# Dokumushikun/jittor-clip-fewshot

Hardware: AMD Instinct MI355X
Metric: images/sec ViT-B/32 fwd+LoRA-bwd bs=256 (higher is better)
Workload: dtype f32; 1 GPU; cfg-2: ViT-B/32 + rank-4 LoRA(q,k,v; 12 text + 12 vision blocks; shipped lora_weights.pkl) + 4 text-prompt tokens; run_lora train step = text tower fwd+bwd on 403 captions + image tower fwd+bwd + 100*cos CE + AdamW; global_batch=256, images_per_rank=256, captions=403, tower_streams=2, text_positions=77, parallelism=dp1

## Files before the change

include/clipfs.h:

```cpp
#ifndef CLIPFS_H
#define CLIPFS_H

#include <stddef.h>
#include <stdint.h>

#ifdef __cplusplus
extern "C" {
#endif

#define CLIPFS_OK 0
#define CLIPFS_EINVAL 1
#define CLIPFS_HIPERR_BASE 1000

#define CLIPFS_ABI_VERSION 2
int clipfs_abi_version(void);
const char* clipfs_source_stamp(void);
const char* clipfs_gemm_source_stamp(void);
const char* clipfs_last_error(void);

typedef struct clipfs_gemm_args {
  size_t struct_size;
  const float* A;
  const float* B;
  float* C;
// ... 17 lines not shown
  float* workspace;
  size_t workspace_floats;
  const void* A_f16;
  void* C_f16;
  int aux_f16;
  int* counters;
  size_t counters_ints;
} clipfs_gemm_args;
int clipfs_gemm_nt(const clipfs_gemm_args* args, void* stream);
int clipfs_split_bf16(const float* src, void* planes, size_t n, void* stream);
int clipfs_convert_f16(const float* src, void* dst, size_t n, void* stream);
int clipfs_gemm_splits(int M, int N, int K);
size_t clipfs_gemm_workspace_floats(int M, int N, int K);
size_t clipfs_gemm_counter_ints(int M, int N, int K);
int clipfs_gemm_timing(int enable);
int clipfs_gemm_timing_collect(double* total_ms, double* total_flops, int* launches);
double clipfs_gemm_timing_last_bytes(void);

int clipfs_layernorm_fwd(const float* x, int ldx, const float* gamma, const float* beta, float* y,
                         float* mean, float* rstd, int rows, int width, float eps, void* stream);
int clipfs_layernorm_bwd(const float* dy, const float* x, int ldx, const float* gamma, const float* mean,
                         const float* rstd, const float* dres, float* dx, int lddx, int rows, int width,
                         void* stream);
int clipfs_layernorm_bwd_rows(const float* dy, const float* x, int ldx, const float* gamma, const float* mean,
                              const float* rstd, const int32_t* xmap, const float* dres, float* dx, int lddx, int rows,
                              int width, void* stream);
int clipfs_layernorm_fwd_f16(const float* x, int ldx, const float* gamma, const float* beta, float* y, void* y16,
                             float* mean, float* rstd, int rows, int width, float eps, void* stream);
int clipfs_layernorm_bwd_f16(const float* dy, const float* x, int ldx, const float* gamma, const float* mean,
                             const float* rstd, const float* dres, float* dx, void* dx16, int lddx, int rows, int width,
                             void* stream);
int clipfs_layernorm_fwd_lora_ok(int width, int r, int nseg);
int clipfs_layernorm_fwd_lora(const float* x, int ldx, const float* gamma, const float* beta, float* y, void* y16,
                              float* mean, float* rstd, int rows, int width, float eps, const float* A, float* t, int r,
                              int nseg, unsigned seg_mask, float p, uint64_t seed, uint32_t stream_base, uint32_t drow0,
                              void* keep_bits, void* stream);
int clipfs_layernorm_fwd_lora_map(const float* x, int ldx, const float* gamma, const float* beta, float* y, void* y16,
                                  float* mean, float* rstd, int rows, int width, float eps, const float* A, float* t, int r,
                                  int nseg, unsigned seg_mask, float p, uint64_t seed, uint32_t stream_base, uint32_t drow0,
                                  const int32_t* drow_map, void* keep_bits, void* stream);

int clipfs_attention_fwd(const float* qkv, float* out, float* lse, int batch, int seq, int heads, int causal,
                         void* stream);
int clipfs_attention_bwd(const float* qkv, const float* dout, const float* out, const float* lse, float* dqkv,
                         float* work, int batch, int seq, int heads, int causal, void* stream);
size_t clipfs_attention_lse_floats(int batch, int seq, int heads);
int clipfs_attention_bwd_packed_ok(int seq, int causal);
int clipfs_attention_bwd_packed(const float* qkv, const float* dout, const float* out, const float* lse, float* dqkv,
                                const int32_t* off, int batch, int seq, int heads, void* stream);
int clipfs_attention_fwd_packed(const float* qkv, float* out, float* lse, const int32_t* off, int batch, int seq, int heads,
                                void* stream);
int clipfs_attention_bwd_packed_io(const float* qkv, const float* dout, const float* out, const float* lse, float* dqkv,
                                   const int32_t* off, int batch, int seq, int heads, void* stream);
int clipfs_attention_f16_fwd(const void* qkv, int qkv_f16, float* out, void* out16, float* lse, int batch, int seq,
                             int heads, int causal, void* stream);
int clipfs_attention_f16_bwd(const void* qkv, int qkv_f16, const void* dout, int dout_f16, const float* out,
                             const float* lse, float* dqkv, void* dqkv16, float* work, int batch, int seq, int heads,
                             int causal, void* stream);

int clipfs_lora_down(const float* x, const float* A, float* t, int rows, int width, int r, int nseg,
                     unsigned seg_mask, float p, uint64_t seed, uint32_t stream_base, uint32_t drow0,
                     void* keep_bits, void* stream);
int clipfs_lora_keep_bits_ok(int width, int segw, int r, int nseg);
size_t clipfs_lora_bwd_work_floats(int rows, int width, int r, int nseg);
int clipfs_lora_bwd(const float* dy, const float* x, const float* t, const float* A, const float* B,
                    float* dt, float* dA, float* dB, float* dx, int rows, int width, int segw, int r,
                    int nseg, unsigned seg_mask, float scale, float p, uint64_t seed, uint32_t stream_base,
                    uint32_t drow0, const void* keep_bits, float* work, void* stream);
int clipfs_lora_bwd_f16dy_ok(int width, int segw, int r, int nseg);
int clipfs_lora_bwd_f16dy(const void* dy16, const float* x, const float* t, const float* A, const float* B,
                          float* dt, float* dA, float* dB, float* dx, int rows, int width, int segw, int r,
                          int nseg, unsigned seg_mask, float scale, float p, uint64_t seed, uint32_t stream_base,
                          uint32_t drow0, const void* keep_bits, float* work, void* stream);

int clipfs_vit_fill_special(float* x, const float* class_emb, const float* pos, const float* vpt, int batch,
                            int tokens, int n_patch, int n_vpt, int width, void* stream);
int clipfs_text_embed(const int64_t* ids, const float* table, const float* pos, const float* ctx, int n_ctx,
                      float* x, int n, int seq, int width, void* stream);
int clipfs_token_rows_grad(const float* dx, float* dtok, int n, int seq, int width, int n_tok, int first,
                           void* stream);
int clipfs_matmul_small(const float* A, const float* B, float* C, int M, int N, int K, long sam, long sak,
                        long sbk, long sbn, float alpha, void* stream);
int clipfs_gather_eot(const float* x, const int64_t* ids, float* out, int32_t* idx_out, int n, int seq,
                      int width, void* stream);
int clipfs_scatter_rows(const float* dy, const int32_t* idx, float* dx, int n, int seq, int width, void* stream);
int clipfs_gather_seq_rows(const float* src, size_t ld, const int32_t* idx, float* out, int n, int seq, int width,
                           void* stream);
int clipfs_add_seq_rows(const float* src, const int32_t* idx, float* dx, int n, int seq, int width, void* stream);
int clipfs_put_seq_rows(const float* src, const int32_t* idx, float* dst, size_t ld, int n, int seq, int width,
                        void* stream);
int clipfs_eot_index(const int64_t* ids, int32_t* idx, int n, int seq, void* stream);
int clipfs_gather_rows_map(const float* src, size_t ld, const int32_t* map, float* out, int n, int width, void* stream);
int clipfs_put_rows_map(const float* src, const int32_t* map, float* dst, size_t ld, int n, int width, void* stream);
int clipfs_gather_seq_rows_f16(const void* src_f16, size_t ld, const int32_t* idx, float* out, int n, int seq, int width,
                               void* stream);
int clipfs_put_seq_rows_f16(const float* src, const int32_t* idx, void* dst_f16, size_t ld, int n, int seq, int width,
                            void* stream);

void* clipfs_bpe_create(const char* merges, size_t n_bytes, int n_merges);
void clipfs_bpe_destroy(void* handle);
long clipfs_bpe_encode(const void* handle, const uint8_t* words, const int32_t* offsets, int n_words, int32_t* ids,
                       int32_t* counts, long cap);

int clipfs_nchw_to_nhwc(const float* x, float* y, int N, int C, int H, int W, void* stream);
int clipfs_im2col_nhwc(const float* x, float* col, int N, int H, int W, int C, int kh, int kw, int stride, int pad,
                       int Kp, void* stream);
int clipfs_maxpool3x3s2_nhwc(const float* x, float* y, int N, int H, int W, int C, void* stream);
int clipfs_global_avgpool_nhwc(const float* x, float* y, int N, int HW, int C, void* stream);

int clipfs_l2norm_fwd(const float* x, float* y, float* inv_norm, int rows, int width, void* stream);
int clipfs_l2norm_bwd(const float* dy, const float* y, const float* inv_norm, float* dx, int rows, int width,
                      void* stream);
int clipfs_class_mean_fwd(const float* emb, float* out, int classes, int templates, int width, void* stream);
int clipfs_class_mean_bwd(const float* emb, const float* dout, float* demb, int classes, int templates, int width,
                          void* stream);
int clipfs_cross_entropy(const float* logits, const int64_t* target, float* dlogits, float* loss_rows,
                         float* loss_sum, int32_t* correct, int rows, int classes, float grad_scale,
                         void* stream);
int clipfs_topk(const float* logits, int32_t* labels, int rows, int classes, int k, void* stream);
int clipfs_channel_affine(const float* x, const float* scale1, const float* bias1, float* y, int rows,
                          int width, void* stream);
int clipfs_logit_normalize(const float* z, float* out, float* work, int rows, int classes, void* stream);
int clipfs_logit_normalize_bwd(const float* z, const float* dzn, float* dz, int rows, int classes, void* stream);
int clipfs_colsum(const float* x, const float* y, float* out, int rows, int cols, void* stream);
size_t clipfs_bias_grad_work_floats(int rows, int cols);
int clipfs_bias_grad(const float* x, size_t ldx, int rows, int cols, int seg_width, float* out0, float* out1,
                     float* out2, float* work, void* stream);
int clipfs_l1_loss(const float* a, const float* b, size_t n, float* loss, float* da, float grad_scale, void* stream);
int clipfs_kl_logits(const float* logits, const float* target_logits, float* loss_rows, float* dlogits, int rows,
                     int classes, float grad_scale, void* stream);

int clipfs_adamw(float* p, const float* g, float* m, float* v, size_t n, int step, float lr, float beta1,
                 float beta2, float eps, float weight_decay, float grad_scale, void* stream);

size_t clipfs_mta_work_floats(int n_img, int views, int width, int classes);
// ... 1 lines not shown
               int n_img, int views, int width, int classes, void* stream);

int clipfs_tta_views(const uint8_t* image, int height, int width, const int32_t* recs, int n_views, int out_size,
                     const float* mean, const float* stdv, float* out, void* stream);

int clipfs_crop_batch(const uint8_t* pool, size_t pool_bytes, const int64_t* src, const int64_t* src_dev, int n_src,
                      const int32_t* recs, const int32_t* recs_dev, int n, int out_size, const float* mean,
                      const float* stdv, float* out_norm, float* out_raw, void* stream);

typedef struct clipfs_block {
  const float *ln1_g, *ln1_b, *ln2_g, *ln2_b;
  const float *w_qkv, *b_qkv, *w_qkv_t;
  const float *w_o, *b_o, *w_o_t;
  const float *w_fc, *b_fc, *w_fc_t;
  const float *w_pr, *b_pr, *w_pr_t;
  const float *lora_a_qkv, *lora_b_qkv, *lora_a_o, *lora_b_o;
  float *g_lora_a_qkv, *g_lora_b_qkv, *g_lora_a_o, *g_lora_b_o;
  unsigned lora_mask;
  const void *w_qkv_p, *w_o_p, *w_fc_p, *w_pr_p, *w_qkv_t_p, *w_o_t_p, *w_fc_t_p, *w_pr_t_p;
  float *g_ln1_b, *g_ln2_b, *g_b_q, *g_b_k, *g_b_v, *g_b_o, *g_b_fc, *g_b_pr;
  const float* prompt;
  float* g_prompt;
  int prompt_first, prompt_rows;
} clipfs_block;

typedef struct clipfs_tower {
  size_t struct_size;
  size_t block_size;
  int width, heads, layers, seq, causal;
  int lora_r;
  float lora_scale, lora_dropout;
  uint64_t dropout_seed;
  uint32_t dropout_stream0;
  uint32_t dropout_row0;
  const clipfs_block* blocks;
  int weight_format;
  int* gemm_counters;
  size_t gemm_counters_ints;
  int grad_lo;
} clipfs_tower;

int clipfs_prompt_put(const float* prompt, float* x, const int32_t* off, int batch, int seq, int first, int n, int width,
                      void* stream);
int clipfs_prompt_harvest(float* dx, void* dx16, const int32_t* off, int batch, int seq, int first, int n, int width,
                          float* g, void* stream);

size_t clipfs_tower_saved_floats(const clipfs_tower* t, int batch);
size_t clipfs_tower_scratch_floats(const clipfs_tower* t, int batch);
size_t clipfs_tower_counter_ints(const clipfs_tower* t, int batch);
int clipfs_tower_fwd(const clipfs_tower* t, float* x, int batch, float* saved, float* scratch, void* stream);
int clipfs_tower_fwd_rows(const clipfs_tower* t, float* x, const int32_t* rows, int batch, float* saved, float* scratch,
                          void* stream);
int clipfs_tower_rows_mode(const clipfs_tower* t);
int clipfs_tower_bwd(const clipfs_tower* t, float* dx, int batch, const float* saved, float* scratch,
                     int stop_at_input, void* stream);
int clipfs_tower_bwd_sparse(const clipfs_tower* t, const float* dxs, const int32_t* rows, float* dx, int batch,
                            const float* saved, float* scratch, int stop_at_input, void* stream);
int clipfs_tower_pack_mode(const clipfs_tower* t, int batch, int R);
int clipfs_tower_bwd_packed(const clipfs_tower* t, const float* dxs, const int32_t* rows, const int32_t* plan, int R,
                            float* dx, int batch, const float* saved, float* scratch, int stop_at_input, void* stream);
int clipfs_tower_pack_fwd_mode(const clipfs_tower* t, int batch, int R);
int clipfs_tower_fwd_packed(const clipfs_tower* t, float* x, const int32_t* rows, const int32_t* plan, int R, int batch,
                            float* saved, float* scratch, void* stream);
int clipfs_tower_bwd_packed_saved(const clipfs_tower* t, const float* dxs, const int32_t* rows, const int32_t* plan, int R,
                                  float* dx, int batch, const float* saved, float* scratch, int stop_at_input, void* stream);

#ifdef __cplusplus
}
#endif
#endif
```

jittor-clip-fewshot_amd/clipfs/_lib.py:

```python
from __future__ import annotations

import ctypes as C
import os

ABI_VERSION = 2

_HERE = os.path.dirname(os.path.abspath(__file__))
_TAG = os.environ.get("CLIPFS_LIB_TAG", "")
LIB_PATH = os.path.join(_HERE, f"libclipfs_hip_{_TAG}.so" if _TAG else "libclipfs_hip.so")

c_f32p = C.c_void_p
c_stream = C.c_void_p


class ClipfsError(RuntimeError):
    pass


class GemmArgs(C.Structure):
    _fields_ = [
        ("struct_size", C.c_size_t),
        ("A", C.c_void_p), ("B", C.c_void_p), ("C", C.c_void_p),
        ("M", C.c_int), ("N", C.c_int), ("K", C.c_int),
        ("lda", C.c_int), ("ldb", C.c_int), ("ldc", C.c_int),
# ... 24 lines not shown
                                  "prompt", "g_prompt")] + [("prompt_first", C.c_int), ("prompt_rows", C.c_int)]


class Tower(C.Structure):
    _fields_ = [
        ("struct_size", C.c_size_t), ("block_size", C.c_size_t),
        ("width", C.c_int), ("heads", C.c_int), ("layers", C.c_int), ("seq", C.c_int), ("causal", C.c_int),
        ("lora_r", C.c_int), ("lora_scale", C.c_float), ("lora_dropout", C.c_float),
        ("dropout_seed", C.c_uint64), ("dropout_stream0", C.c_uint32), ("dropout_row0", C.c_uint32),
        ("blocks", C.POINTER(Block)), ("weight_format", C.c_int),
        ("gemm_counters", C.c_void_p), ("gemm_counters_ints", C.c_size_t),
        ("grad_lo", C.c_int),
    ]


_i, _f, _p, _sz = C.c_int, C.c_float, C.c_void_p, C.c_size_t
_u, _u64, _u32 = C.c_uint, C.c_uint64, C.c_uint32

SIGNATURES = {
    "clipfs_abi_version": (_i, []),
    "clipfs_last_error": (C.c_char_p, []),
    "clipfs_source_stamp": (C.c_char_p, []),
    "clipfs_gemm_source_stamp": (C.c_char_p, []),
    "clipfs_gemm_nt": (_i, [C.POINTER(GemmArgs), _p]),
    "clipfs_split_bf16": (_i, [_p, _p, _sz, _p]),
    "clipfs_convert_f16": (_i, [_p, _p, _sz, _p]),
    "clipfs_gemm_splits": (_i, [_i, _i, _i]),
    "clipfs_gemm_workspace_floats": (_sz, [_i, _i, _i]),
    "clipfs_gemm_counter_ints": (_sz, [_i, _i, _i]),
    "clipfs_gemm_timing": (_i, [_i]),
    "clipfs_gemm_timing_collect": (_i, [C.POINTER(C.c_double), C.POINTER(C.c_double), C.POINTER(C.c_int)]),
    "clipfs_gemm_timing_last_bytes": (C.c_double, []),
    "clipfs_layernorm_fwd": (_i, [_p, _i, _p, _p, _p, _p, _p, _i, _i, _f, _p]),
    "clipfs_layernorm_bwd": (_i, [_p, _p, _i, _p, _p, _p, _p, _p, _i, _i, _i, _p]),
    "clipfs_layernorm_fwd_f16": (_i, [_p, _i, _p, _p, _p, _p, _p, _p, _i, _i, _f, _p]),
    "clipfs_layernorm_fwd_lora_ok": (_i, [_i, _i, _i]),
    "clipfs_layernorm_fwd_lora": (_i, [_p, _i, _p, _p, _p, _p, _p, _p, _i, _i, _f, _p, _p, _i, _i, _u, _f, _u64, _u32, _u32, _p, _p]),
    "clipfs_layernorm_bwd_f16": (_i, [_p, _p, _i, _p, _p, _p, _p, _p, _p, _i, _i, _i, _p]),
    "clipfs_attention_fwd": (_i, [_p, _p, _p, _i, _i, _i, _i, _p]),
    "clipfs_attention_bwd": (_i, [_p, _p, _p, _p, _p, _p, _i, _i, _i, _i, _p]),
    "clipfs_attention_lse_floats": (_sz, [_i, _i, _i]),
    "clipfs_attention_f16_fwd": (_i, [_p, _i, _p, _p, _p, _i, _i, _i, _i, _p]),
    "clipfs_attention_f16_bwd": (_i, [_p, _i, _p, _i, _p, _p, _p, _p, _p, _i, _i, _i, _i, _p]),
    "clipfs_lora_keep_bits_ok": (_i, [_i, _i, _i, _i]),
    "clipfs_lora_down": (_i, [_p, _p, _p, _i, _i, _i, _i, _u, _f, _u64, _u32, _u32, _p, _p]),
    "clipfs_lora_bwd_work_floats": (_sz, [_i, _i, _i, _i]),
    "clipfs_lora_bwd": (_i, [_p, _p, _p, _p, _p, _p, _p, _p, _p, _i, _i, _i, _i, _i, _u, _f, _f, _u64, _u32, _u32, _p, _p, _p]),
    "clipfs_lora_bwd_f16dy_ok": (_i, [_i, _i, _i, _i]),
    "clipfs_lora_bwd_f16dy": (_i, [_p, _p, _p, _p, _p, _p, _p, _p, _p, _i, _i, _i, _i, _i, _u, _f, _f, _u64, _u32, _u32, _p, _p, _p]),
    "clipfs_vit_fill_special": (_i, [_p, _p, _p, _p, _i, _i, _i, _i, _i, _p]),
    "clipfs_text_embed": (_i, [_p, _p, _p, _p, _i, _p, _i, _i, _i, _p]),
    "clipfs_token_rows_grad": (_i, [_p, _p, _i, _i, _i, _i, _i, _p]),
    "clipfs_matmul_small": (_i, [_p, _p, _p, _i, _i, _i, C.c_long, C.c_long, C.c_long, C.c_long, _f, _p]),
    "clipfs_gather_eot": (_i, [_p, _p, _p, _p, _i, _i, _i, _p]),
    "clipfs_scatter_rows": (_i, [_p, _p, _p, _i, _i, _i, _p]),
    "clipfs_gather_seq_rows": (_i, [_p, _sz, _p, _p, _i, _i, _i, _p]),
    "clipfs_add_seq_rows": (_i, [_p, _p, _p, _i, _i, _i, _p]),
    "clipfs_put_seq_rows": (_i, [_p, _p, _p, _sz, _i, _i, _i, _p]),
    "clipfs_eot_index": (_i, [_p, _p, _i, _i, _p]),
    "clipfs_gather_seq_rows_f16": (_i, [_p, _sz, _p, _p, _i, _i, _i, _p]),
    "clipfs_put_seq_rows_f16": (_i, [_p, _p, _p, _sz, _i, _i, _i, _p]),
    "clipfs_l2norm_fwd": (_i, [_p, _p, _p, _i, _i, _p]),
    "clipfs_l2norm_bwd": (_i, [_p, _p, _p, _p, _i, _i, _p]),
    "clipfs_class_mean_fwd": (_i, [_p, _p, _i, _i, _i, _p]),
    "clipfs_class_mean_bwd": (_i, [_p, _p, _p, _i, _i, _i, _p]),
    "clipfs_cross_entropy": (_i, [_p, _p, _p, _p, _p, _p, _i, _i, _f, _p]),
    "clipfs_topk": (_i, [_p, _p, _i, _i, _i, _p]),
    "clipfs_channel_affine": (_i, [_p, _p, _p, _p, _i, _i, _p]),
    "clipfs_logit_normalize": (_i, [_p, _p, _p, _i, _i, _p]),
    "clipfs_logit_normalize_bwd": (_i, [_p, _p, _p, _i, _i, _p]),
    "clipfs_colsum": (_i, [_p, _p, _p, _i, _i, _p]),
    "clipfs_bias_grad_work_floats": (_sz, [_i, _i]),
    "clipfs_bias_grad": (_i, [_p, _sz, _i, _i, _i, _p, _p, _p, _p, _p]),
    "clipfs_l1_loss": (_i, [_p, _p, _sz, _p, _p, _f, _p]),
    "clipfs_kl_logits": (_i, [_p, _p, _p, _p, _i, _i, _f, _p]),
    "clipfs_adamw": (_i, [_p, _p, _p, _p, _sz, _i, _f, _f, _f, _f, _f, _f, _p]),
    "clipfs_mta_work_floats": (_sz, [_i, _i, _i, _i]),
    "clipfs_mta": (_i, [_p, _p, _p, _p, _p, _i, _i, _i, _i, _p]),
    "clipfs_tta_views": (_i, [_p, _i, _i, _p, _i, _i, _p, _p, _p, _p]),
    "clipfs_crop_batch": (_i, [_p, _sz, _p, _p, _i, _p, _p, _i, _i, _p, _p, _p, _p, _p]),
    "clipfs_bpe_create": (C.c_void_p, [C.c_char_p, _sz, _i]),
    "clipfs_bpe_destroy": (None, [C.c_void_p]),
    "clipfs_bpe_encode": (C.c_long, [C.c_void_p, _p, _p, _i, _p, _p, C.c_long]),
    "clipfs_nchw_to_nhwc": (_i, [_p, _p, _i, _i, _i, _i, _p]),
    "clipfs_im2col_nhwc": (_i, [_p, _p, _i, _i, _i, _i, _i, _i, _i, _i, _i, _p]),
    "clipfs_maxpool3x3s2_nhwc": (_i, [_p, _p, _i, _i, _i, _i, _p]),
    "clipfs_global_avgpool_nhwc": (_i, [_p, _p, _i, _i, _i, _p]),
    "clipfs_prompt_put": (_i, [_p, _p, _p, _i, _i, _i, _i, _i, _p]),
    "clipfs_prompt_harvest": (_i, [_p, _p, _p, _i, _i, _i, _i, _i, _p, _p]),
    "clipfs_tower_saved_floats": (_sz, [C.POINTER(Tower), _i]),
    "clipfs_tower_scratch_floats": (_sz, [C.POINTER(Tower), _i]),
    "clipfs_tower_counter_ints": (_sz, [C.POINTER(Tower), _i]),
    "clipfs_tower_fwd": (_i, [C.POINTER(Tower), _p, _i, _p, _p, _p]),
    "clipfs_tower_fwd_rows": (_i, [C.POINTER(Tower), _p, _p, _i, _p, _p, _p]),
    "clipfs_tower_rows_mode": (_i, [C.POINTER(Tower)]),
    "clipfs_tower_bwd": (_i, [C.POINTER(Tower), _p, _i, _p, _p, _i, _p]),
    "clipfs_tower_bwd_sparse": (_i, [C.POINTER(Tower), _p, _p, _p, _i, _p, _p, _i, _p]),
    "clipfs_attention_bwd_packed_ok": (_i, [_i, _i]),
    "clipfs_attention_bwd_packed": (_i, [_p, _p, _p, _p, _p, _p, _i, _i, _i, _p]),
    "clipfs_gather_rows_map": (_i, [_p, _sz, _p, _p, _i, _i, _p]),
    "clipfs_put_rows_map": (_i, [_p, _p, _p, _sz, _i, _i, _p]),
    "clipfs_layernorm_bwd_rows": (_i, [_p, _p, _i, _p, _p, _p, _p, _p, _p, _i, _i, _i, _p]),
    "clipfs_tower_pack_mode": (_i, [C.POINTER(Tower), _i, _i]),
    "clipfs_tower_bwd_packed": (_i, [C.POINTER(Tower), _p, _p, _p, _i, _p, _i, _p, _p, _i, _p]),
    "clipfs_layernorm_fwd_lora_map": (_i, [_p, _i, _p, _p, _p, _p, _p, _p, _i, _i, _f, _p, _p, _i, _i, _u, _f, _u64, _u32, _u32, _p,
                                           _p, _p]),
    "clipfs_attention_fwd_packed": (_i, [_p, _p, _p, _p, _i, _i, _i, _p]),
    "clipfs_attention_bwd_packed_io": (_i, [_p, _p, _p, _p, _p, _p, _i, _i, _i, _p]),
    "clipfs_tower_pack_fwd_mode": (_i, [C.POINTER(Tower), _i, _i]),
    "clipfs_tower_fwd_packed": (_i, [C.POINTER(Tower), _p, _p, _p, _i, _i, _p, _p, _p]),
    "clipfs_tower_bwd_packed_saved": (_i, [C.POINTER(Tower), _p, _p, _p, _i, _p, _i, _p, _p, _i, _p]),
}

def new_gemm_args() -> GemmArgs:
    g = GemmArgs()
    g.struct_size = C.sizeof(GemmArgs)
    return g


def new_tower() -> Tower:
    t = Tower()
    t.struct_size = C.sizeof(Tower)
    t.block_size = C.sizeof(Block)
    return t


_lib = None


def load() -> C.CDLL:
    global _lib
    if _lib is not None:
        return _lib
    if not os.path.isfile(LIB_PATH):
        raise ClipfsError(
            f"{LIB_PATH} not found: the HIP engine is not built.  Run "
            "`python jittor-clip-fewshot_amd/build.py` (needs hipcc).  There is no CPU fallback.")
    try:
        import torch
    except Exception:
        pass
    lib = C.CDLL(LIB_PATH, mode=C.RTLD_GLOBAL if hasattr(C, "RTLD_GLOBAL") else 0)
    for name, (res, args) in SIGNATURES.items():
        fn = getattr(lib, name)
        fn.restype = res
        fn.argtypes = args
    if lib.clipfs_abi_version() != ABI_VERSION:
        raise ClipfsError(f"libclipfs_hip.so ABI version {lib.clipfs_abi_version()} != {ABI_VERSION} of this binding: "
                          "rebuild with `python jittor-clip-fewshot_amd/build.py --force`")
    _lib = lib
    return lib


def check(rc: int, what: str = "") -> None:
    if rc != 0:
        msg = load().clipfs_last_error().decode("utf-8", "replace")
        raise ClipfsError(f"{what or 'clipfs call'} failed (rc={rc}): {msg}")
```

jittor-clip-fewshot_amd/clipfs/engine.py:

```python
from __future__ import annotations

import ctypes as C
from typing import Dict, List, Optional, Tuple

import torch

from . import _lib, ops
from ._lib import Block, Tower, check


def _ptr(t: Optional[torch.Tensor]) -> Optional[int]:
    return None if t is None else t.data_ptr()


def _bias_slot(p: Optional[torch.nn.Parameter]) -> Optional[torch.Tensor]:
    if p is None or not p.requires_grad:
        return None
    return getattr(p, "grad_slot", None)


def _lora_trains(a, where: str) -> bool:
    flags = {p.requires_grad for p, _ in a.trainable_pairs()}
    if len(flags) > 1:
        raise ValueError(f"{where}: some of its LoRA adapters are frozen and others trainable; freeze or train the "
                         "q / k / v / o adapters of a block together")
    return flags == {True}


def _blk_biases(blk) -> List[torch.nn.Parameter]:
    a = blk.attn
    if getattr(a, "is_lora_mha", False):
        out = [a.q_proj.bias, a.k_proj.bias, a.v_proj.bias, a.proj.bias]
    else:
        out = [a.in_proj_bias, a.out_proj.bias]
    return out + [blk.ln_1.bias, blk.ln_2.bias, blk.mlp.c_fc.bias, blk.mlp.c_proj.bias]


def _mix_seed(base: int, step: int) -> int:
    z = (base * 0x9E3779B97F4A7C15 + step * 0xBF58476D1CE4E5B9 + 0x94D049BB133111EB) & 0xFFFFFFFFFFFFFFFF
    z ^= z >> 30
    z = (z * 0xBF58476D1CE4E5B9) & 0xFFFFFFFFFFFFFFFF
    z ^= z >> 27
    z = (z * 0x94D049BB133111EB) & 0xFFFFFFFFFFFFFFFF
    z ^= z >> 31
    return z or 1


class _TowerRT:

    def __init__(self, transformer, seq: int, stream0: int, name: str = "tower"):
        self.mod = transformer
        self.name = name
        self.seq = seq
        self.width = transformer.width
        self.heads = transformer.heads
        self.layers = transformer.layers
        self.causal = bool(transformer.causal)
        self.stream0 = stream0
        self._bufs: Dict[Tuple[str, int], torch.Tensor] = {}
        self._wt: Dict[int, Dict[str, torch.Tensor]] = {}
        self._planes: Dict[Tuple[int, str, str], torch.Tensor] = {}
        self.precision = "fp32"
        self.lora_r = 0
        self.lora_scale = 0.0
        self.lora_dropout = 0.0

    def _transposed(self, i: int, blk) -> Dict[str, torch.Tensor]:
        wt = self._wt.get(i)
        if wt is None:
            a = blk.attn
            w_qkv = a.qkv_weight if getattr(a, "is_lora_mha", False) else a.in_proj_weight
            w_o = a.proj.weight if getattr(a, "is_lora_mha", False) else a.out_proj.weight
            wt = {"qkv": w_qkv.data.t().contiguous(), "o": w_o.data.t().contiguous(),
                  "fc": blk.mlp.c_fc.weight.data.t().contiguous(), "pr": blk.mlp.c_proj.weight.data.t().contiguous()}
            self._wt[i] = wt
        return wt

    def _plane(self, i: int, name: str, w: torch.Tensor) -> torch.Tensor:
        key = (i, name, self.precision)
        pl = self._planes.get(key)
        if pl is None:
            pl = ops.split_bf16(w.contiguous()) if self.precision == "bf16x3" else ops.to_f16(w.contiguous())
            self._planes[key] = pl
        return pl

    def _block_trains(self, i: int, blk) -> bool:
        a = blk.attn
        if getattr(a, "is_lora_mha", False) and a.r > 0 and _lora_trains(a, f"{self.name} block {i}"):
            return True
        if _bias_slot(getattr(blk, "VPT_shallow", None)) is not None:
            return True
        return any(_bias_slot(p) is not None for p in _blk_biases(blk))

    def grad_floor(self, needs_input_grad: bool, head_trains: bool = False) -> Optional[int]:
        if needs_input_grad:
            return 0
        for i, blk in enumerate(self.mod.resblocks):
            if self._block_trains(i, blk):
                return i
        return self.layers - 1 if head_trains else None

    def descriptor(self, train: bool, seed: int, seq: Optional[int] = None, row0: int = 0, grad_lo: int = 0) -> Tower:
        blocks = (Block * self.layers)()
        r, scale, p = 0, 0.0, 0.0
        n_pr = getattr(self.mod, "prompt_rows", 0)
        first = (seq or self.seq) - n_pr if getattr(self.mod, "prompt_tail", False) else 1
        for i, blk in enumerate(self.mod.resblocks):
            a = blk.attn
            b = blocks[i]
            vp = getattr(blk, "VPT_shallow", None)
            if vp is not None:
                g = _bias_slot(vp)
                ok = (vp.dim() == 2 and tuple(vp.shape) == (n_pr, self.width) and vp.dtype == torch.float32
                      and vp.is_contiguous() and vp.device == self.mod.resblocks[0].ln_1.weight.device and first >= 1)
                if g is not None:
                    ok = ok and g.shape == vp.shape and g.dtype == torch.float32 and g.is_contiguous() and g.device == vp.device
                if not ok:
                    raise ValueError(f"{self.name} block {i}: deep prompt {tuple(vp.shape)} (slot "
# ... 21 lines not shown
                gq, gk, gv = (None, None, None) if g is None else (g[:d], g[d:2 * d], g[2 * d:])
                go = _bias_slot(a.out_proj.bias)
            b.g_b_q, b.g_b_k, b.g_b_v, b.g_b_o = _ptr(gq), _ptr(gk), _ptr(gv), _ptr(go)
            b.g_ln1_b, b.g_ln2_b = _ptr(_bias_slot(blk.ln_1.bias)), _ptr(_bias_slot(blk.ln_2.bias))
            b.g_b_fc, b.g_b_pr = _ptr(_bias_slot(blk.mlp.c_fc.bias)), _ptr(_bias_slot(blk.mlp.c_proj.bias))
            if train:
                wt = self._transposed(i, blk)
                b.w_qkv_t, b.w_o_t, b.w_fc_t, b.w_pr_t = _ptr(wt["qkv"]), _ptr(wt["o"]), _ptr(wt["fc"]), _ptr(wt["pr"])
            if self.precision != "fp32":
                b.w_qkv_p = _ptr(self._plane(i, "qkv", w_qkv.data))
                b.w_o_p = _ptr(self._plane(i, "o", w_o.data))
                b.w_fc_p = _ptr(self._plane(i, "fc", blk.mlp.c_fc.weight.data))
                b.w_pr_p = _ptr(self._plane(i, "pr", blk.mlp.c_proj.weight.data))
                if train:
                    b.w_qkv_t_p = _ptr(self._plane(i, "qkv_t", wt["qkv"]))
                    b.w_o_t_p = _ptr(self._plane(i, "o_t", wt["o"]))
                    b.w_fc_t_p = _ptr(self._plane(i, "fc_t", wt["fc"]))
                    b.w_pr_t_p = _ptr(self._plane(i, "pr_t", wt["pr"]))
            b.lora_mask = 0
            if lora and a.r > 0:
                if r and (a.r != r or abs(a.scaling - scale) > 0 or abs(a.dropout_rate - p) > 0):
                    raise ValueError("all LoRA layers of one tower must share r / alpha / dropout")
                r, scale, p = a.r, float(a.scaling), float(a.dropout_rate)
                b.lora_mask = a.lora_mask
                trains = _lora_trains(a, f"{self.name} block {i}")
                b.lora_a_qkv, b.lora_b_qkv = _ptr(a.lora_A_qkv), _ptr(a.lora_B_qkv)
                if trains:
                    b.g_lora_a_qkv, b.g_lora_b_qkv = _ptr(a.grad_A_qkv), _ptr(a.grad_B_qkv)
                if a.lora_mask & 8:
                    b.lora_a_o, b.lora_b_o = _ptr(a.lora_A_o), _ptr(a.lora_B_o)
                    if trains:
                        b.g_lora_a_o, b.g_lora_b_o = _ptr(a.grad_A_o), _ptr(a.grad_B_o)
        t = _lib.new_tower()
        t.width, t.heads, t.layers, t.seq, t.causal = (self.width, self.heads, self.layers, seq or self.seq,
                                                       int(self.causal))
        t.lora_r, t.lora_scale, t.lora_dropout = r, scale, p
        t.dropout_seed = seed if p > 0 else 0
        t.dropout_stream0 = self.stream0
        t.dropout_row0 = row0 * (seq or self.seq)
        t.weight_format = {"fp32": 0, "bf16x3": 1, "fp16": 2}[self.precision]
        t.grad_lo = grad_lo
        t.blocks = C.cast(blocks, C.POINTER(Block))
        t._blocks_keepalive = blocks
        self.lora_r, self.lora_scale, self.lora_dropout = r, scale, p
        return t

    def lora_dropout_rate(self) -> float:
        return max((float(b.attn.dropout_rate) for b in self.mod.resblocks
                    if getattr(b.attn, "is_lora_mha", False) and b.attn.r > 0), default=0.0)

    def has_lora(self) -> bool:
        return any(getattr(b.attn, "is_lora_mha", False) and b.attn.r > 0 for b in self.mod.resblocks)

    def buffer(self, kind: str, n_floats: int, device) -> torch.Tensor:
        key = (kind, n_floats)
        buf = self._bufs.get(key)
        if buf is None:
            for k in [k for k in self._bufs if k[0] == kind]:
                del self._bufs[k]
            buf = torch.empty(max(n_floats, 4), device=device, dtype=torch.float32)
            self._bufs[key] = buf
        return buf

    def _attach_counters(self, t: Tower, batch: int, device) -> None:
        n = _lib.load().clipfs_tower_counter_ints(C.byref(t), batch)
        if n == 0:
            return
        buf = self._bufs.get(("counters", 0))
        if buf is None or buf.numel() < n:
            buf = torch.zeros(n, device=device, dtype=torch.int32)
            self._bufs[("counters", 0)] = buf
        t.gemm_counters, t.gemm_counters_ints = buf.data_ptr(), buf.numel()

    def forward(self, x: torch.Tensor, batch: int, train: bool, seed: int, seq: Optional[int] = None,
                own_saved: bool = False, row0: int = 0, rows: Optional[torch.Tensor] = None, grad_lo: int = 0,
                pack: Optional[Tuple[torch.Tensor, int]] = None, desc: Optional[Tower] = None):
        lib = _lib.load()
        t = desc if desc is not None else self.descriptor(train, seed, seq, row0, grad_lo if train else 0)
        self._attach_counters(t, batch, x.device)
        scratch = self.buffer("scratch", lib.clipfs_tower_scratch_floats(C.byref(t), batch), x.device)
        saved = None
        if train:
            n = lib.clipfs_tower_saved_floats(C.byref(t), batch)
            saved = torch.empty(max(n, 4), device=x.device, dtype=torch.float32) if own_saved else \
                self.buffer("saved", n, x.device)
        if rows is not None:
            assert rows.dtype == torch.int32 and rows.is_cuda and rows.numel() >= batch
        if pack is not None:
            assert rows is not None
            plan, R = pack
            check(lib.clipfs_tower_fwd_packed(C.byref(t), x.data_ptr(), rows.data_ptr(), plan.data_ptr(), R, batch, _ptr(saved),
                                              scratch.data_ptr(), torch.cuda.current_stream().cuda_stream), "tower_fwd_packed")
        elif rows is not None:
            check(lib.clipfs_tower_fwd_rows(C.byref(t), x.data_ptr(), rows.data_ptr(), batch, _ptr(saved), scratch.data_ptr(),
                                            torch.cuda.current_stream().cuda_stream), "tower_fwd_rows")
        else:
            check(lib.clipfs_tower_fwd(C.byref(t), x.data_ptr(), batch, _ptr(saved), scratch.data_ptr(),
                                       torch.cuda.current_stream().cuda_stream), "tower_fwd")
        return saved

    def backward(self, dx: torch.Tensor, batch: int, saved: torch.Tensor, seed: int, stop_at_input: bool,
                 seq: Optional[int] = None, row0: int = 0, grad_lo: int = 0):
        lib = _lib.load()
        t = self.descriptor(True, seed, seq, row0, grad_lo)
        self._attach_counters(t, batch, dx.device)
        scratch = self.buffer("scratch", lib.clipfs_tower_scratch_floats(C.byref(t), batch), dx.device)
        check(lib.clipfs_tower_bwd(C.byref(t), dx.data_ptr(), batch, saved.data_ptr(), scratch.data_ptr(),
                                   int(stop_at_input), torch.cuda.current_stream().cuda_stream), "tower_bwd")


    def backward_sparse(self, dxs: torch.Tensor, rows: torch.Tensor, batch: int, saved: torch.Tensor, seed: int,
                        stop_at_input: bool, seq: Optional[int] = None, row0: int = 0, grad_lo: int = 0) -> torch.Tensor:
        lib = _lib.load()
        t = self.descriptor(True, seed, seq, row0, grad_lo)
        self._attach_counters(t, batch, dxs.device)
        scratch = self.buffer("scratch", lib.clipfs_tower_scratch_floats(C.byref(t), batch), dxs.device)
        dx = torch.empty(batch * (seq or self.seq), self.width, device=dxs.device, dtype=torch.float32)
        check(lib.clipfs_tower_bwd_sparse(C.byref(t), dxs.data_ptr(), rows.data_ptr(), dx.data_ptr(), batch, saved.data_ptr(),
                                          scratch.data_ptr(), int(stop_at_input), torch.cuda.current_stream().cuda_stream),
              "tower_bwd_sparse")
        return dx

    def backward_packed(self, dxs: torch.Tensor, rows: torch.Tensor, plan: torch.Tensor, R: int, batch: int,
                        saved: torch.Tensor, seed: int, stop_at_input: bool, seq: Optional[int] = None, row0: int = 0,
                        grad_lo: int = 0, saved_packed: bool = False) -> torch.Tensor:
        lib = _lib.load()
        t = self.descriptor(True, seed, seq, row0, grad_lo)
        self._attach_counters(t, batch, dxs.device)
        scratch = self.buffer("scratch", lib.clipfs_tower_scratch_floats(C.byref(t), batch), dxs.device)
        dx = torch.empty(batch * (seq or self.seq), self.width, device=dxs.device, dtype=torch.float32)
        fn = lib.clipfs_tower_bwd_packed_saved if saved_packed else lib.clipfs_tower_bwd_packed
        check(fn(C.byref(t), dxs.data_ptr(), rows.data_ptr(), plan.data_ptr(), R, dx.data_ptr(), batch, saved.data_ptr(),
                 scratch.data_ptr(), int(stop_at_input), torch.cuda.current_stream().cuda_stream),
              "tower_bwd_packed_saved" if saved_packed else "tower_bwd_packed")
        return dx

    def pack_mode(self, batch: int, R: int, seed: int, seq: Optional[int] = None, grad_lo: int = 0,
                  train: bool = True) -> bool:
        t = self.descriptor(train, seed, seq, 0, grad_lo)
        return bool(_lib.load().clipfs_tower_pack_mode(C.byref(t), batch, R))

    @staticmethod
    def pack_modes(desc: Tower, batch: int, R: int) -> Tuple[bool, bool]:
        lib = _lib.load()
        return bool(lib.clipfs_tower_pack_mode(C.byref(desc), batch, R)), bool(lib.clipfs_tower_pack_fwd_mode(C.byref(desc), batch, R))

    def pack_fwd_mode(self, batch: int, R: int, seed: int, seq: Optional[int] = None, grad_lo: int = 0,
                      train: bool = True) -> bool:
        t = self.descriptor(train, seed, seq, 0, grad_lo)
        return bool(_lib.load().clipfs_tower_pack_fwd_mode(C.byref(t), batch, R))


class Engine:
    def __init__(self, model):
        self.model = model
        v = model.visual
        self.vis = _TowerRT(v.transformer, v.tokens, stream0=1000, name="vision")
        self.txt = _TowerRT(model.transformer, model.context_length, stream0=0, name="text")
        self.vproj_t = v.proj.data.t().contiguous()
        self.tproj_t = model.text_projection.data.t().contiguous()
        self.seed_base = 0x5EED
        self.step = 0
        self.trim_text = False
        self._trim_cache = {}
        self.sparse_backward = True
        self.prune_backward = True
        self.pack_text_backward = True
        self.pack_text_forward = True
        self._pack_cache = {}

    @property
    def precision(self) -> str:
        return self.vis.precision

    @precision.setter
    def precision(self, mode: str) -> None:
        if mode not in ("fp32", "bf16x3", "fp16"):
            raise ValueError("precision must be 'fp32', 'bf16x3' or 'fp16'")
        self.vis.precision = mode
        self.txt.precision = mode

    def image_plan(self) -> Optional[int]:
        if not self.prune_backward:
            return 0
        v = self.model.visual
        return self.vis.grad_floor(v.VPT is not None or _bias_slot(v.ln_pre.bias) is not None,
                                   _bias_slot(v.ln_post.bias) is not None)

    def text_plan(self, has_ctx: bool) -> Optional[int]:
        if not self.prune_backward:
            return 0
        return self.txt.grad_floor(has_ctx, _bias_slot(self.model.ln_final.bias) is not None)

    def next_seed(self) -> int:
        self.step += 1
        return _mix_seed(self.seed_base, self.step)

    def vit_forward(self, images: torch.Tensor, train: bool, seed: int = 0, own_saved: bool = False, row0: int = 0):
        lo = self.image_plan() if train else 0
        if lo is None:
            train = False
        m = self.model
        v = m.visual
        assert images.is_cuda and images.dtype == torch.float32, "images: fp32 device tensor [B,3,R,R]"
        images = images.contiguous()
        B = images.shape[0]
        if images.shape[1] != 3 or images.shape[2] != v.input_resolution or images.shape[3] != v.input_resolution:
            raise ValueError(f"expected images [B,3,{v.input_resolution},{v.input_resolution}], got {tuple(images.shape)}")
        L, d = v.tokens, v.width
        P = (v.input_resolution // v.patch_size) ** 2
        x0 = torch.empty(B * L, d, device=images.device, dtype=torch.float32)
        ops.patch_embed(images, v.conv1.weight.data, v.positional_embedding.data, x0, L)
        ops.vit_fill_special(x0, v.class_embedding.data, v.positional_embedding.data,
                             None if v.VPT is None else v.VPT.data, B, L, P)
        need_pre = train and v.VPT is not None
        if need_pre:
            x, mean0, rstd0 = ops.layernorm_fwd(x0, v.ln_pre.weight.data, v.ln_pre.bias.data, save_stats=True)
        else:
            x = ops.layernorm_fwd(x0, v.ln_pre.weight.data, v.ln_pre.bias.data)
            mean0 = rstd0 = None
        one_row = bool(self.sparse_backward)
        saved = self.vis.forward(x, B, train, seed, own_saved=own_saved, row0=row0,
# ... 354 lines not shown
```

jittor-clip-fewshot_amd/clipfs/ops.py:

```python
from __future__ import annotations

import ctypes as C
from typing import Optional

import torch

from . import _lib
from ._lib import GemmArgs, check


def _stream() -> int:
    return torch.cuda.current_stream().cuda_stream


def _p(t: Optional[torch.Tensor]) -> Optional[int]:
    if t is None:
        return None
    assert t.is_cuda, "clipfs ops need device tensors (there is no CPU path)"
    return t.data_ptr()


def _f32(t: torch.Tensor) -> torch.Tensor:
    assert t.dtype == torch.float32 and t.is_contiguous(), (t.dtype, t.is_contiguous())
    return t
# ... 201 lines not shown
def lora_bwd(dy, x, t, A, B, dA, dB, *, dx=None, scale, p=0.0, seed=0, stream_base=0, seg_mask=None, row0=0, keep_bits=None):
    rows, width = x.shape
    nseg = dy.shape[1] // width
    r = B.shape[1]
    if seg_mask is None:
        seg_mask = (1 << nseg) - 1
    lib = _lib.load()
    nwork = lib.clipfs_lora_bwd_work_floats(rows, width, r, nseg)
    work = torch.empty(nwork, device=x.device, dtype=torch.float32)
    dt = torch.empty(rows, nseg * r, device=x.device, dtype=torch.float32)
    if dy.dtype == torch.float16:
        assert dy.is_contiguous()
        check(lib.clipfs_lora_bwd_f16dy(_p(dy), _p(_f32(x)), _p(_f32(t)), _p(_f32(A)), _p(_f32(B)), _p(dt), _p(dA),
                                        _p(dB), _p(dx), rows, width, width, r, nseg, seg_mask, scale, p, seed, stream_base,
                                        row0, _p(keep_bits), _p(work), _stream()), "lora_bwd_f16dy")
        return dt
    check(lib.clipfs_lora_bwd(_p(_f32(dy)), _p(_f32(x)), _p(_f32(t)), _p(_f32(A)), _p(_f32(B)), _p(dt), _p(dA),
                              _p(dB), _p(dx), rows, width, width, r, nseg, seg_mask, scale, p, seed, stream_base,
                              row0, _p(keep_bits), _p(work), _stream()), "lora_bwd")
    return dt


def vit_fill_special(x, class_emb, pos, vpt, batch, tokens, n_patch):
    n_vpt = 0 if vpt is None else vpt.shape[0]
    check(_lib.load().clipfs_vit_fill_special(_p(x), _p(class_emb), _p(pos), _p(vpt), batch, tokens, n_patch, n_vpt,
                                              class_emb.numel(), _stream()), "vit_fill_special")


def text_embed(ids, table, pos, ctx=None):
    n, seq = ids.shape
    width = table.shape[1]
    assert ids.dtype == torch.int64 and ids.is_contiguous()
    x = torch.empty(n * seq, width, device=table.device, dtype=torch.float32)
    n_ctx = 0 if ctx is None else ctx.shape[0]
    check(_lib.load().clipfs_text_embed(_p(ids), _p(table), _p(pos), _p(ctx), n_ctx, _p(x), n, seq, width, _stream()),
          "text_embed")
    return x


def token_rows_grad(dx, dtok, n, seq, first):
    n_tok, width = dtok.shape
    check(_lib.load().clipfs_token_rows_grad(_p(dx), _p(dtok), n, seq, width, n_tok, first, _stream()),
          "token_rows_grad")


def matmul_small(a, b, M, N, K, sam, sak, sbk, sbn, alpha=1.0, out=None):
    if out is None:
        out = torch.empty(M, N, device=a.device, dtype=torch.float32)
    check(_lib.load().clipfs_matmul_small(_p(a), _p(b), _p(out), M, N, K, sam, sak, sbk, sbn, alpha, _stream()),
          "matmul_small")
    return out


def eot_index(ids: torch.Tensor) -> torch.Tensor:
    assert ids.is_cuda and ids.dtype == torch.int64 and ids.is_contiguous()
    n, seq = ids.shape
    idx = torch.empty(n, device=ids.device, dtype=torch.int32)
    check(_lib.load().clipfs_eot_index(_p(ids), _p(idx), n, seq, _stream()), "eot_index")
    return idx


def gather_eot(x, ids):
    n, seq = ids.shape
    width = x.shape[-1]
    out = torch.empty(n, width, device=x.device, dtype=torch.float32)
    idx = torch.empty(n, device=x.device, dtype=torch.int32)
    check(_lib.load().clipfs_gather_eot(_p(x), _p(ids), _p(out), _p(idx), n, seq, width, _stream()), "gather_eot")
    return out, idx


def scatter_rows(dy, idx, seq, out=None):
    n, width = dy.shape
    dx = out if out is not None else torch.empty(n * seq, width, device=dy.device, dtype=torch.float32)
    check(_lib.load().clipfs_scatter_rows(_p(_f32(dy)), _p(idx), _p(dx), n, seq, width, _stream()), "scatter_rows")
    return dx


def l2norm_fwd(x, save_inv=False):
    rows, width = x.shape
    y = torch.empty_like(x)
    inv = torch.empty(rows, device=x.device, dtype=torch.float32) if save_inv else None
    check(_lib.load().clipfs_l2norm_fwd(_p(_f32(x)), _p(y), _p(inv), rows, width, _stream()), "l2norm_fwd")
    return (y, inv) if save_inv else y


def l2norm_bwd(dy, y, inv):
    rows, width = y.shape
    dx = torch.empty_like(y)
    check(_lib.load().clipfs_l2norm_bwd(_p(_f32(dy)), _p(y), _p(inv), _p(dx), rows, width, _stream()), "l2norm_bwd")
    return dx


def class_mean_fwd(emb, classes, templates, out=None):
    width = emb.shape[1]
    if out is None:
        out = torch.empty(classes, width, device=emb.device, dtype=torch.float32)
    assert out.is_contiguous() and tuple(out.shape) == (classes, width)
    check(_lib.load().clipfs_class_mean_fwd(_p(_f32(emb)), _p(out), classes, templates, width, _stream()),
          "class_mean_fwd")
    return out


def class_mean_bwd(emb, dout, classes, templates):
    demb = torch.empty_like(emb)
    check(_lib.load().clipfs_class_mean_bwd(_p(_f32(emb)), _p(_f32(dout)), _p(demb), classes, templates, emb.shape[1],
                                            _stream()), "class_mean_bwd")
# ... 102 lines not shown
```

jittor-clip-fewshot_amd/csrc/attention.hip:

```cpp
#include "common.h"

#include <stdlib.h>

namespace clipfs {

constexpr int HD = 64;
constexpr int KSTRIDE = 68;

typedef float f32x4 __attribute__((ext_vector_type(4)));

__device__ __forceinline__ void stage_rows(const float* __restrict__ base, size_t ld, float* __restrict__ dst, int L,
                                           int tid) {
  for (int idx = tid; idx < L * (HD / 4); idx += (int)blockDim.x) {
    const int r = idx >> 4, c = idx & 15;
    *reinterpret_cast<f32x4*>(dst + r * KSTRIDE + 4 * c) = *reinterpret_cast<const f32x4*>(base + (size_t)r * ld + 4 * c);
  }
}

template <int KPL>
__device__ __forceinline__ void rows_to_regs(const float* __restrict__ s, int lane, int L, float (&reg)[KPL][HD]) {
#pragma unroll
  for (int kk = 0; kk < KPL; ++kk) {
    const int j = lane + 64 * kk;
    const bool ok = j < L;
// ... 525 lines not shown
  float* sP = sG + L * KSTRIDE;
  const int lane = threadIdx.x & 63;
  const int wave = __builtin_amdgcn_readfirstlane(threadIdx.x >> 6);
  const int b = blockIdx.x / H, h = blockIdx.x % H;
  const int d = H * HD;
  const size_t ld = (size_t)3 * d;
  const float* q0 = qkv + (size_t)b * L * ld + (size_t)h * HD;
  stage_rows_n(q0, ld, sQ, L);
  stage_rows_n(dout + (size_t)b * L * d + (size_t)h * HD, (size_t)d, sG, L);
  __syncthreads();
  float* myP = sP + wave * 64;
  float* myS = sP + 8 * 64 + wave * 64;
  const float* lse0 = lse + ((size_t)b * H + h) * L;
  const float* D0 = Dbuf + ((size_t)b * H + h) * L;
  for (int j = wave; j < L; j += 8) {
    f32x4 k[HD / 4], v[HD / 4];
#pragma unroll
    for (int c = 0; c < HD / 4; ++c) {
      k[c] = *reinterpret_cast<const f32x4*>(q0 + d + (size_t)j * ld + 4 * c);
      v[c] = *reinterpret_cast<const f32x4*>(q0 + 2 * d + (size_t)j * ld + 4 * c);
    }
    float av = 0.f, ak = 0.f;
    const int ibeg = causal ? j : 0;
    for (int i0 = ibeg & ~63; i0 < L; i0 += 64) {
      const int i = i0 + lane;
      float pj = 0.f, ds = 0.f;
      if (i < L && i >= ibeg) {
        pj = __expf(dot64_row(k, sQ + i * KSTRIDE) * 0.125f - lse0[i]);
        ds = pj * (dot64_row(v, sG + i * KSTRIDE) - D0[i]) * 0.125f;
      }
      myP[lane] = pj;
      myS[lane] = ds;
      __builtin_amdgcn_wave_barrier();
      const int n = min(64, L - i0);
      av = axpy_block_lds(myP, sG + i0 * KSTRIDE, lane, n, av);
      ak = axpy_block_lds(myS, sQ + i0 * KSTRIDE, lane, n, ak);
      __builtin_amdgcn_wave_barrier();
    }
    dqkv[((size_t)b * L + j) * ld + 2 * d + h * HD + lane] = av;
    dqkv[((size_t)b * L + j) * ld + d + h * HD + lane] = ak;
  }
}

bool attention_mfma_enabled();
int attention_mfma_fwd(const float* qkv, float* out, float* lse, int batch, int seq, int heads, int causal, hipStream_t st);
int attention_mfma_bwd(const float* qkv, const float* dout, const float* out, const float* lse, float* dqkv, float* work,
                       int batch, int seq, int heads, int causal, hipStream_t st);
constexpr int ATTN_MFMA_MAX = 288;
bool attention16_enabled(int seq);
int attention16_bwd_packed(const float* qkv, const float* dout, const float* out, const float* lse, float* dqkv,
                           const int32_t* off, int batch, int seq, int heads, bool pin, hipStream_t st);
int attention16_fwd_packed(const float* qkv, float* out, float* lse, const int32_t* off, int batch, int seq, int heads,
                           hipStream_t st);

static int check_attn(const char* what, int batch, int seq, int heads, int max_seq) {
  CLIPFS_REQUIRE(batch > 0 && heads > 0 && seq > 0 && seq <= max_seq, "%s: batch %d seq %d heads %d unsupported (seq <= %d)",
                 what, batch, seq, heads, max_seq);
  return CLIPFS_OK;
}

static int padded_lp(int seq) {
  int lp = (seq + 3) & ~3;
  if (((lp >> 2) & 1) == 0) lp += 4;
  return lp;
}

}

using namespace clipfs;

constexpr int ATTN_FAST_MAX = 96;
constexpr int ATTN_MAX_SEQ = 4096;
constexpr int ATTN_LDS_MAX = 288;

extern "C" int clipfs_attention_fwd(const float* qkv, float* out, float* lse, int batch, int seq, int heads, int causal,
                                    void* stream) {
  CLIPFS_CHECK(check_attn("attention_fwd", batch, seq, heads, ATTN_MAX_SEQ));
  CLIPFS_REQUIRE(qkv && out && aligned16(qkv), "attention_fwd: null or misaligned pointer");
  hipStream_t st = (hipStream_t)stream;
  if (attention_mfma_enabled() && seq <= ATTN_MFMA_MAX && aligned16(out))
    return attention_mfma_fwd(qkv, out, lse, batch, seq, heads, causal, st);
  if ((seq > 128 || (seq > ATTN_FAST_MAX && lse)) && seq <= ATTN_LDS_MAX) {
    const size_t lds = ((size_t)2 * seq * KSTRIDE + 8 * 64) * sizeof(float);
    static bool attr = false;
    if (!attr) {
      (void)hipFuncSetAttribute(reinterpret_cast<const void*>(&attention_lds_fwd_kernel),
                                hipFuncAttributeMaxDynamicSharedMemorySize, 160 * 1024);
      attr = true;
    }
    hipLaunchKernelGGL(attention_lds_fwd_kernel, dim3(batch * heads), dim3(512), lds, st, qkv, out, lse, seq, heads, causal);
    return launch_status();
  }
  if (seq > 128 || (seq > ATTN_FAST_MAX && lse)) {
    hipLaunchKernelGGL(attention_generic_fwd_kernel, dim3(batch * heads, (seq + 3) / 4), dim3(256), 0, st, qkv, out, lse,
                       seq, heads, causal);
    return launch_status();
  }
  static const int thr_cfg = getenv("CLIPFS_ATTN_FWD_THREADS") ? atoi(getenv("CLIPFS_ATTN_FWD_THREADS")) : 0;
  const dim3 grid(batch * heads), block(thr_cfg ? thr_cfg : 256);
  const size_t lds1 = ((size_t)seq * KSTRIDE + 16 * 64) * sizeof(float);
  const size_t lds2 = ((size_t)seq * KSTRIDE + 16 * 128) * sizeof(float);
  if (seq <= 64)
    hipLaunchKernelGGL((attention_fwd_kernel<64>), grid, block, lds1, st, qkv, out, seq, heads, causal);
  else if (seq <= 80)
    hipLaunchKernelGGL((attention_fwd_kernel<80>), grid, block, lds2, st, qkv, out, seq, heads, causal);
  else if (seq <= 96)
// ... 46 lines not shown
  const dim3 grid(batch * heads), block(thr_cfg ? thr_cfg : (seq > 64 ? 512 : 256));
  static bool attr = false;
  if (!attr) {
    (void)hipFuncSetAttribute(reinterpret_cast<const void*>(&attention_bwd_kernel<64>),
                              hipFuncAttributeMaxDynamicSharedMemorySize, 160 * 1024);
    (void)hipFuncSetAttribute(reinterpret_cast<const void*>(&attention_bwd_kernel<80>),
                              hipFuncAttributeMaxDynamicSharedMemorySize, 160 * 1024);
    (void)hipFuncSetAttribute(reinterpret_cast<const void*>(&attention_bwd_kernel<96>),
                              hipFuncAttributeMaxDynamicSharedMemorySize, 160 * 1024);
    attr = true;
  }
  if (seq <= 64)
    hipLaunchKernelGGL((attention_bwd_kernel<64>), grid, block, lds, st, qkv, dout, dqkv, seq, heads, causal, lp);
  else if (seq <= 80)
    hipLaunchKernelGGL((attention_bwd_kernel<80>), grid, block, lds, st, qkv, dout, dqkv, seq, heads, causal, lp);
  else
    hipLaunchKernelGGL((attention_bwd_kernel<96>), grid, block, lds, st, qkv, dout, dqkv, seq, heads, causal, lp);
  return launch_status();
}

extern "C" int clipfs_attention_bwd_packed_ok(int seq, int causal) {
  return (causal && seq > 0 && seq <= ATTN_MFMA_MAX && attention_mfma_enabled() && attention16_enabled(seq)) ? 1 : 0;
}

extern "C" int clipfs_attention_bwd_packed(const float* qkv, const float* dout, const float* out, const float* lse,
                                           float* dqkv, const int32_t* off, int batch, int seq, int heads, void* stream) {
  CLIPFS_CHECK(check_attn("attention_bwd_packed", batch, seq, heads, ATTN_MAX_SEQ));
  CLIPFS_REQUIRE(clipfs_attention_bwd_packed_ok(seq, 1), "attention_bwd_packed: seq %d has no packed kernel", seq);
  CLIPFS_REQUIRE(qkv && dout && out && lse && dqkv && off, "attention_bwd_packed: null pointer");
  CLIPFS_REQUIRE(aligned16(qkv) && aligned16(dout) && aligned16(out) && aligned16(dqkv),
                 "attention_bwd_packed: misaligned pointer");
  return attention16_bwd_packed(qkv, dout, out, lse, dqkv, off, batch, seq, heads, false, (hipStream_t)stream);
}

extern "C" int clipfs_attention_fwd_packed(const float* qkv, float* out, float* lse, const int32_t* off, int batch, int seq,
                                           int heads, void* stream) {
  CLIPFS_CHECK(check_attn("attention_fwd_packed", batch, seq, heads, ATTN_MAX_SEQ));
  CLIPFS_REQUIRE(clipfs_attention_bwd_packed_ok(seq, 1), "attention_fwd_packed: seq %d has no packed kernel", seq);
  CLIPFS_REQUIRE(qkv && out && off, "attention_fwd_packed: null pointer");
  CLIPFS_REQUIRE(aligned16(qkv) && aligned16(out), "attention_fwd_packed: misaligned pointer");
  return attention16_fwd_packed(qkv, out, lse, off, batch, seq, heads, (hipStream_t)stream);
}

extern "C" int clipfs_attention_bwd_packed_io(const float* qkv, const float* dout, const float* out, const float* lse,
                                              float* dqkv, const int32_t* off, int batch, int seq, int heads, void* stream) {
  CLIPFS_CHECK(check_attn("attention_bwd_packed_io", batch, seq, heads, ATTN_MAX_SEQ));
  CLIPFS_REQUIRE(clipfs_attention_bwd_packed_ok(seq, 1), "attention_bwd_packed_io: seq %d has no packed kernel", seq);
  CLIPFS_REQUIRE(qkv && dout && out && lse && dqkv && off, "attention_bwd_packed_io: null pointer");
  CLIPFS_REQUIRE(aligned16(qkv) && aligned16(dout) && aligned16(out) && aligned16(dqkv),
                 "attention_bwd_packed_io: misaligned pointer");
  return attention16_bwd_packed(qkv, dout, out, lse, dqkv, off, batch, seq, heads, true, (hipStream_t)stream);
}

extern "C" size_t clipfs_attention_lse_floats(int batch, int seq, int heads) {
  if (attention_mfma_enabled() && seq <= ATTN_MFMA_MAX) return (size_t)batch * heads * seq;
  return seq > ATTN_FAST_MAX ? (size_t)batch * heads * seq : 0;
}
```

jittor-clip-fewshot_amd/csrc/attention_mfma16.hip:

```cpp
#include "common.h"

#include <stdlib.h>

namespace clipfs {

typedef float f32x4 __attribute__((ext_vector_type(4)));

constexpr int A16_HD = 64;
constexpr float A16_LOG2E = 1.4426950408889634f;
constexpr int A16_MAX_TILES = 6;

__device__ __forceinline__ f32x4 mfma16(float a, float b, f32x4 c) {
  return __builtin_amdgcn_mfma_f32_16x16x4f32(a, b, c, 0, 0, 0);
}

template <int NT>
__device__ __forceinline__ void a16_fetch(const float* __restrict__ src, size_t ld, int L, f32x4 (&v)[4]) {
  constexpr int Lp = 16 * NT;
#pragma unroll
  for (int k = 0; k < 4; ++k) {
    const int idx = (int)threadIdx.x + k * 64 * NT;
    const int c = idx / Lp, tok = idx - c * Lp;
    v[k] = *reinterpret_cast<const f32x4*>(src + (size_t)min(tok, L - 1) * ld + 4 * c);
  }
// ... 18 lines not shown
#pragma unroll
    for (int e = 0; e < 4; ++e) w[4 * j + e] = v[e];
  }
}

template <int NA, int TP>
__device__ __forceinline__ void a16_scores(const float* tr, int lane, const float (&own)[16], f32x4 (&acc)[A16_MAX_TILES]) {
  const float* p = tr + (16 * (lane >> 4)) * TP + (lane & 15);
#pragma unroll
  for (int t = 0; t < NA; ++t) acc[t] = f32x4{0.f, 0.f, 0.f, 0.f};
#pragma unroll
  for (int s = 0; s < 16; ++s)
#pragma unroll
    for (int t = 0; t < NA; ++t) acc[t] = mfma16(p[s * TP + 16 * t], own[s], acc[t]);
}

template <int TP>
__device__ __forceinline__ void a16_accum(const float* tr, int lane, int t, const f32x4& w, f32x4 (&o)[4]) {
  const float* p = tr + (lane & 15) * TP + 16 * t + 4 * (lane >> 4);
  f32x4 a[4];
#pragma unroll
  for (int ft = 0; ft < 4; ++ft) a[ft] = *reinterpret_cast<const f32x4*>(p + 16 * ft * TP);
#pragma unroll
  for (int r = 0; r < 4; ++r)
#pragma unroll
    for (int ft = 0; ft < 4; ++ft) o[ft] = mfma16(a[ft][r], w[r], o[ft]);
}

__device__ __forceinline__ void a16_store(float* __restrict__ dst, const f32x4 (&o)[4], float scale, int lane) {
  float* p = dst + 4 * (lane >> 4);
#pragma unroll
  for (int ft = 0; ft < 4; ++ft) *reinterpret_cast<f32x4*>(p + 16 * ft) = o[ft] * scale;
}

__device__ __forceinline__ float a16_allreduce_max(float v) {
  v = fmaxf(v, __shfl_xor(v, 16, 64));
  return fmaxf(v, __shfl_xor(v, 32, 64));
}
__device__ __forceinline__ float a16_allreduce_sum(float v) {
  v += __shfl_xor(v, 16, 64);
  return v + __shfl_xor(v, 32, 64);
}

#define A16_SWITCH_SCORES(na, IMG, OWN, ACC)                                   \
  switch (na) {                                                                \
    case 1: a16_scores<1, TP>(IMG, lane, OWN, ACC); break;               \
    case 2: a16_scores<(NT >= 2 ? 2 : 1), TP>(IMG, lane, OWN, ACC); break; \
    case 3: a16_scores<(NT >= 3 ? 3 : 1), TP>(IMG, lane, OWN, ACC); break; \
    case 4: a16_scores<(NT >= 4 ? 4 : 1), TP>(IMG, lane, OWN, ACC); break; \
    case 5: a16_scores<(NT >= 5 ? 5 : 1), TP>(IMG, lane, OWN, ACC); break; \
    default: a16_scores<(NT >= 6 ? 6 : 1), TP>(IMG, lane, OWN, ACC); break; \
  }

template <int NT, bool PACKED = false>
__global__ __launch_bounds__(64 * NT) void attention16_fwd_kernel(const float* __restrict__ qkv, float* __restrict__ out,
                                                                  float* __restrict__ lse, int L, int H, int causal,
                                                                  const int32_t* __restrict__ off) {
  extern __shared__ __attribute__((aligned(16))) float a16_smem[];
  constexpr int TP = 16 * NT + 8;
  float* sKt = a16_smem;
  float* sVt = sKt + 64 * TP;
  const int lane = threadIdx.x & 63;
  const int qt = __builtin_amdgcn_readfirstlane(threadIdx.x >> 6);
  const int d = H * A16_HD;
  const size_t ld = (size_t)3 * d;
  const int g = lane >> 4;
  const int q_tok = 16 * qt + (lane & 15);
  const float c = 0.125f * A16_LOG2E;
  const int item = blockIdx.x;
  const int b = item / H, h = item % H;
  const size_t prow = PACKED ? (size_t)off[b] : (size_t)b * L;
  const int Lb = PACKED ? (int)(off[b + 1] - prow) : L;
  if (PACKED && (Lb <= 0 || Lb > L)) return;
  const int klim = causal ? q_tok : Lb - 1;
  const int na = causal ? qt + 1 : NT;
  const float* hq = qkv + prow * ld + (size_t)h * A16_HD;
  f32x4 kst[4], vst[4];
  a16_fetch<NT>(hq + d, ld, Lb, kst);
  a16_fetch<NT>(hq + 2 * d, ld, Lb, vst);
  float qf[16];
  a16_load_own(hq, ld, min(q_tok, Lb - 1), lane, qf);
  a16_put<NT>(sKt, kst, Lb);
  a16_put<NT>(sVt, vst, Lb);
  __syncthreads();
  if (PACKED && 16 * qt >= Lb) return;
  f32x4 s[A16_MAX_TILES];
  A16_SWITCH_SCORES(na, sKt, qf, s)
  float m = -INFINITY;
#pragma unroll
  for (int t = 0; t < NT; ++t)
    if (t < na) {
#pragma unroll
      for (int r = 0; r < 4; ++r) {
        const int key = 16 * t + 4 * g + r;
        s[t][r] = (key < Lb && key <= klim) ? s[t][r] * c : -INFINITY;
        m = fmaxf(m, s[t][r]);
      }
    }
  m = a16_allreduce_max(m);
  float l = 0.f;
#pragma unroll
  for (int t = 0; t < NT; ++t)
    if (t < na) {
#pragma unroll
      for (int r = 0; r < 4; ++r) {
        s[t][r] = __builtin_amdgcn_exp2f(s[t][r] - m);
        l += s[t][r];
      }
    }
  l = a16_allreduce_sum(l);
  f32x4 o[4];
#pragma unroll
  for (int ft = 0; ft < 4; ++ft) o[ft] = f32x4{0.f, 0.f, 0.f, 0.f};
#pragma unroll
  for (int t = 0; t < NT; ++t)
    if (t < na) a16_accum<TP>(sVt, lane, t, s[t], o);
  if (q_tok < Lb) {
    a16_store(out + (prow + q_tok) * d + h * A16_HD, o, 1.f / l, lane);
    if (lse && g == 0) lse[((size_t)b * H + h) * L + q_tok] = (m + log2f(l)) * (1.f / A16_LOG2E);
  }
}

template <int NT, bool PACKED, bool PIN>
__device__ __forceinline__ void attention16_bwd_q_body(const float* __restrict__ qkv, const float* __restrict__ dout,
                                                       const float* __restrict__ out, const float* __restrict__ lse,
                                                       float* __restrict__ dqkv, int L, int H, int causal, int item,
                                                       const int32_t* __restrict__ off, float* a16_smem) {
  constexpr int TP = 16 * NT + 8;
  float* sKt = a16_smem;
  float* sVt = sKt + 64 * TP;
  const int lane = threadIdx.x & 63;
  const int qt = __builtin_amdgcn_readfirstlane(threadIdx.x >> 6);
  const int d = H * A16_HD;
  const size_t ld = (size_t)3 * d;
  const int g = lane >> 4;
  const int b = item / H, h = item % H;
  const size_t prow = PACKED ? (size_t)off[b] : (size_t)b * L;
  const size_t irow = PIN ? prow : (size_t)b * L;
  const int Lb = PACKED ? (int)(off[b + 1] - prow) : L;
  const int q_tok = 16 * qt + (lane & 15), q_cl = min(q_tok, Lb - 1);
  const float c = 0.125f * A16_LOG2E;
  const int klim = causal ? q_tok : Lb - 1;
  const int na = causal ? qt + 1 : (Lb + 15) / 16;
  const float* hq = qkv + irow * ld + (size_t)h * A16_HD;
  f32x4 kst[4], vst[4];
  a16_fetch<NT>(hq + d, ld, Lb, kst);
  a16_fetch<NT>(hq + 2 * d, ld, Lb, vst);
  float qf[16], gf[16];
  a16_load_own(hq, ld, q_cl, lane, qf);
  a16_load_own(dout + prow * d + (size_t)h * A16_HD, (size_t)d, q_cl, lane, gf);
  float Di = 0.f;
  {
    const float* op = out + (irow + q_cl) * d + h * A16_HD + 16 * g;
#pragma unroll
    for (int j = 0; j < 4; ++j) {
      const f32x4 ov = *reinterpret_cast<const f32x4*>(op + 4 * j);
#pragma unroll
      for (int e = 0; e < 4; ++e) Di = fmaf(gf[4 * j + e], ov[e], Di);
    }
  }
  const float lse2 = lse[((size_t)b * H + h) * L + q_cl] * A16_LOG2E;
  a16_put<NT>(sKt, kst, Lb);
  a16_put<NT>(sVt, vst, Lb);
  Di = a16_allreduce_sum(Di);
  __syncthreads();
  if (PACKED && 16 * qt >= Lb) return;
  f32x4 s[A16_MAX_TILES], dp[A16_MAX_TILES];
  A16_SWITCH_SCORES(na, sKt, qf, s)
  A16_SWITCH_SCORES(na, sVt, gf, dp)
  f32x4 acc[4];
#pragma unroll
  for (int ft = 0; ft < 4; ++ft) acc[ft] = f32x4{0.f, 0.f, 0.f, 0.f};
#pragma unroll
  for (int t = 0; t < NT; ++t)
    if (t < na) {
      f32x4 ds;
#pragma unroll
      for (int r = 0; r < 4; ++r) {
        const int key = 16 * t + 4 * g + r;
        const float p = (key < Lb && key <= klim) ? __builtin_amdgcn_exp2f(s[t][r] * c - lse2) : 0.f;
        ds[r] = p * (dp[t][r] - Di) * 0.125f;
      }
      a16_accum<TP>(sKt, lane, t, ds, acc);
    }
  if (q_tok < Lb) a16_store(dqkv + (prow + q_tok) * ld + h * A16_HD, acc, 1.f, lane);
}

template <int NT, bool PACKED, bool PIN>
__device__ __forceinline__ void attention16_bwd_kv_body(const float* __restrict__ qkv, const float* __restrict__ dout,
                                                        const float* __restrict__ out, const float* __restrict__ lse,
                                                        float* __restrict__ dqkv, int L, int H, int causal, int item,
                                                        const int32_t* __restrict__ off, float* a16_smem) {
  constexpr int Lp = 16 * NT, TP = Lp + 8;
  float* sQt = a16_smem;
  float* sGt = sQt + 64 * TP;
  float* sLse = sGt + 64 * TP;
  float* sD = sLse + Lp;
  float* sPart = sD + Lp;
  const int lane = threadIdx.x & 63;
  const int kt = __builtin_amdgcn_readfirstlane(threadIdx.x >> 6);
  const int d = H * A16_HD;
  const size_t ld = (size_t)3 * d;
  const int g = lane >> 4;
  const int b = item / H, h = item % H;
  const size_t prow = PACKED ? (size_t)off[b] : (size_t)b * L;
  const size_t irow = PIN ? prow : (size_t)b * L;
  const int Lb = PACKED ? (int)(off[b + 1] - prow) : L;
  const int k_tok = 16 * kt + (lane & 15), k_cl = min(k_tok, Lb - 1);
  const float c = 0.125f * A16_LOG2E;
  const int t_first = causal ? kt : 0;
  const int na = (PACKED ? (Lb + 15) / 16 : NT) - t_first;
  const float* sQ1 = sQt + 16 * t_first;
  const float* sG1 = sGt + 16 * t_first;
  const float* hq = qkv + irow * ld + (size_t)h * A16_HD;
  const int vtok = min((int)threadIdx.x, Lb - 1);
  f32x4 qst[4], gst[4], ost[4];
  a16_fetch<NT>(hq, ld, Lb, qst);
  a16_fetch<NT>(dout + prow * d + (size_t)h * A16_HD, (size_t)d, Lb, gst);
  a16_fetch<NT>(out + irow * d + (size_t)h * A16_HD, (size_t)d, Lb, ost);
  float kf[16], vf[16];
  a16_load_own(hq + d, ld, k_cl, lane, kf);
  a16_load_own(hq + 2 * d, ld, k_cl, lane, vf);
  const float lse_i = lse[(size_t)item * L + vtok];
  a16_put<NT>(sQt, qst, Lb);
  a16_put<NT>(sGt, gst, Lb);
#pragma unroll
  for (int k = 0; k < 4; ++k) {
    const int idx = (int)threadIdx.x + k * 64 * NT;
    const int c = idx / Lp, tok = idx - c * Lp;
    sPart[c * Lp + tok] = fmaf(gst[k][3], ost[k][3], fmaf(gst[k][2], ost[k][2], fmaf(gst[k][1], ost[k][1], gst[k][0] * ost[k][0])));
  }
  __syncthreads();
  if ((int)threadIdx.x < Lp) {
    float d_i = 0.f;
#pragma unroll
    for (int c = 0; c < 16; ++c) d_i += sPart[c * Lp + threadIdx.x];
    sLse[threadIdx.x] = (int)threadIdx.x < Lb ? lse_i * A16_LOG2E : 0.f;
    sD[threadIdx.x] = (int)threadIdx.x < Lb ? d_i : 0.f;
  }
  __syncthreads();
  if (PACKED && na <= 0) return;
  f32x4 s[A16_MAX_TILES], dp[A16_MAX_TILES];
  A16_SWITCH_SCORES(na, sQ1, kf, s)
  A16_SWITCH_SCORES(na, sG1, vf, dp)
  f32x4 av[4], ak[4];
#pragma unroll
  for (int ft = 0; ft < 4; ++ft) {
    av[ft] = f32x4{0.f, 0.f, 0.f, 0.f};
    ak[ft] = f32x4{0.f, 0.f, 0.f, 0.f};
  }
#pragma unroll
  for (int u = 0; u < NT; ++u)
    if (u < na) {
      const int t = t_first + u;
      const f32x4 l4 = *reinterpret_cast<const f32x4*>(sLse + 16 * t + 4 * g);
      const f32x4 d4 = *reinterpret_cast<const f32x4*>(sD + 16 * t + 4 * g);
      f32x4 p, ds;
#pragma unroll
      for (int r = 0; r < 4; ++r) {
        const int qi = 16 * t + 4 * g + r;
        p[r] = (qi < Lb && (!causal || qi >= k_tok)) ? __builtin_amdgcn_exp2f(s[u][r] * c - l4[r]) : 0.f;
        ds[r] = p[r] * (dp[u][r] - d4[r]) * 0.125f;
      }
      a16_accum<TP>(sGt, lane, t, p, av);
      a16_accum<TP>(sQt, lane, t, ds, ak);
    }
  if (k_tok < Lb) {
    float* kp = dqkv + (prow + k_tok) * ld + d + h * A16_HD;
    a16_store(kp, ak, 1.f, lane);
    a16_store(kp + d, av, 1.f, lane);
  }
}

template <int NT, bool PACKED = false, bool PIN = false>
__global__ __launch_bounds__(64 * NT) void attention16_bwd_kernel(const float* __restrict__ qkv, const float* __restrict__ dout,
                                                                  const float* __restrict__ out, const float* __restrict__ lse,
                                                                  float* __restrict__ dqkv, int L, int H, int causal,
                                                                  const int32_t* __restrict__ off) {
  extern __shared__ __attribute__((aligned(16))) float a16_smem[];
  const int item = blockIdx.x >> 1;
  if (blockIdx.x & 1)
    attention16_bwd_kv_body<NT, PACKED, PIN>(qkv, dout, out, lse, dqkv, L, H, causal, item, off, a16_smem);
  else
    attention16_bwd_q_body<NT, PACKED, PIN>(qkv, dout, out, lse, dqkv, L, H, causal, item, off, a16_smem);
}


bool attention16_enabled(int seq) {
  static const int cfg = getenv("CLIPFS_ATTN16") ? atoi(getenv("CLIPFS_ATTN16")) : 1;
  return cfg != 0 && seq <= 16 * A16_MAX_TILES;
}

static size_t a16_lds(int nt, bool vectors) {
  return ((size_t)2 * 64 * (16 * nt + 8) + (vectors ? 18 * (size_t)16 * nt : 0)) * sizeof(float);
}

template <int NT, bool PACKED = false>
static int a16_fwd(const float* qkv, float* out, float* lse, int batch, int seq, int heads, int causal, hipStream_t st,
                   const int32_t* off = nullptr) {
  static bool attr = false;
  if (!attr && a16_lds(NT, false) > 48 * 1024) {
    (void)hipFuncSetAttribute(reinterpret_cast<const void*>(&attention16_fwd_kernel<NT, PACKED>),
                              hipFuncAttributeMaxDynamicSharedMemorySize, (int)a16_lds(NT, false));
    attr = true;
  }
  hipLaunchKernelGGL((attention16_fwd_kernel<NT, PACKED>), dim3(batch * heads), dim3(64 * NT), a16_lds(NT, false), st, qkv, out,
                     lse, seq, heads, causal, off);
  return launch_status();
}

template <int NT, bool PACKED = false, bool PIN = false>
static int a16_bwd(const float* qkv, const float* dout, const float* out, const float* lse, float* dqkv, float* work,
                   int batch, int seq, int heads, int causal, hipStream_t st, const int32_t* off = nullptr) {
  (void)work;
  static bool attr = false;
  if (!attr && a16_lds(NT, true) > 48 * 1024) {
    (void)hipFuncSetAttribute(reinterpret_cast<const void*>(&attention16_bwd_kernel<NT, PACKED, PIN>),
                              hipFuncAttributeMaxDynamicSharedMemorySize, (int)a16_lds(NT, true));
    attr = true;
  }
  hipLaunchKernelGGL((attention16_bwd_kernel<NT, PACKED, PIN>), dim3(2 * batch * heads), dim3(64 * NT), a16_lds(NT, true), st,
                     qkv, dout, out, lse, dqkv, seq, heads, causal, off);
  return launch_status();
}

int attention16_fwd(const float* qkv, float* out, float* lse, int batch, int seq, int heads, int causal, hipStream_t st) {
  switch ((seq + 15) / 16) {
    case 1: return a16_fwd<1>(qkv, out, lse, batch, seq, heads, causal, st);
    case 2: return a16_fwd<2>(qkv, out, lse, batch, seq, heads, causal, st);
    case 3: return a16_fwd<3>(qkv, out, lse, batch, seq, heads, causal, st);
    case 4: return a16_fwd<4>(qkv, out, lse, batch, seq, heads, causal, st);
    case 5: return a16_fwd<5>(qkv, out, lse, batch, seq, heads, causal, st);
    default: return a16_fwd<6>(qkv, out, lse, batch, seq, heads, causal, st);
  }
}

int attention16_bwd(const float* qkv, const float* dout, const float* out, const float* lse, float* dqkv, float* work,
                    int batch, int seq, int heads, int causal, hipStream_t st) {
  switch ((seq + 15) / 16) {
    case 1: return a16_bwd<1>(qkv, dout, out, lse, dqkv, work, batch, seq, heads, causal, st);
    case 2: return a16_bwd<2>(qkv, dout, out, lse, dqkv, work, batch, seq, heads, causal, st);
    case 3: return a16_bwd<3>(qkv, dout, out, lse, dqkv, work, batch, seq, heads, causal, st);
    case 4: return a16_bwd<4>(qkv, dout, out, lse, dqkv, work, batch, seq, heads, causal, st);
    case 5: return a16_bwd<5>(qkv, dout, out, lse, dqkv, work, batch, seq, heads, causal, st);
    default: return a16_bwd<6>(qkv, dout, out, lse, dqkv, work, batch, seq, heads, causal, st);
  }
}

int attention16_bwd_packed(const float* qkv, const float* dout, const float* out, const float* lse, float* dqkv,
                           const int32_t* off, int batch, int seq, int heads, bool pin, hipStream_t st) {
#define A16_BWD_PACKED(nt)                                                                              \
  return pin ? a16_bwd<nt, true, true>(qkv, dout, out, lse, dqkv, nullptr, batch, seq, heads, 1, st, off) \
             : a16_bwd<nt, true, false>(qkv, dout, out, lse, dqkv, nullptr, batch, seq, heads, 1, st, off)
  switch ((seq + 15) / 16) {
    case 1: A16_BWD_PACKED(1);
    case 2: A16_BWD_PACKED(2);
    case 3: A16_BWD_PACKED(3);
    case 4: A16_BWD_PACKED(4);
    case 5: A16_BWD_PACKED(5);
    default: A16_BWD_PACKED(6);
  }
#undef A16_BWD_PACKED
}

int attention16_fwd_packed(const float* qkv, float* out, float* lse, const int32_t* off, int batch, int seq, int heads,
                           hipStream_t st) {
  switch ((seq + 15) / 16) {
    case 1: return a16_fwd<1, true>(qkv, out, lse, batch, seq, heads, 1, st, off);
    case 2: return a16_fwd<2, true>(qkv, out, lse, batch, seq, heads, 1, st, off);
    case 3: return a16_fwd<3, true>(qkv, out, lse, batch, seq, heads, 1, st, off);
    case 4: return a16_fwd<4, true>(qkv, out, lse, batch, seq, heads, 1, st, off);
    case 5: return a16_fwd<5, true>(qkv, out, lse, batch, seq, heads, 1, st, off);
    default: return a16_fwd<6, true>(qkv, out, lse, batch, seq, heads, 1, st, off);
  }
}

}
```

jittor-clip-fewshot_amd/csrc/elem.hip:

```cpp
#include "common.h"

namespace clipfs {

__global__ __launch_bounds__(256) void vit_fill_special_kernel(float* __restrict__ x, const float* __restrict__ cls,
                                                               const float* __restrict__ pos,
                                                               const float* __restrict__ vpt, int batch, int tokens,
                                                               int n_patch, int n_vpt, int width) {
  const int per_img = (1 + n_vpt) * width;
  const size_t total = (size_t)batch * per_img;
  for (size_t i = (size_t)blockIdx.x * 256 + threadIdx.x; i < total; i += (size_t)gridDim.x * 256) {
    const int b = (int)(i / per_img), rem = (int)(i % per_img);
    const int r = rem / width, c = rem % width;
    if (r == 0)
      x[((size_t)b * tokens) * width + c] = cls[c] + pos[c];
    else
      x[((size_t)b * tokens + n_patch + r) * width + c] = vpt[(size_t)(r - 1) * width + c];
  }
}

__global__ __launch_bounds__(256) void text_embed_kernel(const int64_t* __restrict__ ids, const float* __restrict__ table,
                                                         const float* __restrict__ pos, const float* __restrict__ ctx,
                                                         int n_ctx, float* __restrict__ x, int n, int seq, int width) {
  const int nch = width >> 2;
  const size_t total = (size_t)n * seq * nch;
// ... 426 lines not shown
  }
  const float var = block_total(q) / (float)(n - 1);
  const bool clamped = var < 1e-6f;
  const float sd = sqrtf(fmaxf(var, 1e-6f));
  float g = 0.f;
  for (int r = wave; r < rows; r += 16) {
    float rs = 0.f;
    for (int c = lane; c < classes; c += 64) rs += z[(size_t)r * classes + c];
    const float rm = wave_sum(rs) / (float)classes;
    for (int c = lane; c < classes; c += 64) g = fmaf(dzn[(size_t)r * classes + c], z[(size_t)r * classes + c] - rm, g);
  }
  g = block_total(g);
  const float coef = clamped ? 0.f : g / (sd * sd * sd * (float)(n - 1));
  for (int r = wave; r < rows; r += 16) {
    float ds = 0.f;
    for (int c = lane; c < classes; c += 64) ds += dzn[(size_t)r * classes + c];
    const float dm = wave_sum(ds) / (float)classes;
    for (int c = lane; c < classes; c += 64) {
      const size_t i = (size_t)r * classes + c;
      dz[i] = (dzn[i] - dm) / sd - coef * (z[i] - mean);
    }
  }
}

__global__ __launch_bounds__(256) void colsum_kernel(const float* __restrict__ x, const float* __restrict__ y,
                                                     float* __restrict__ out, int rows, int cols) {
  const int c = blockIdx.x * 256 + threadIdx.x;
  if (c >= cols) return;
  float acc = 0.f;
  for (int r = 0; r < rows; ++r) {
    const float v = x[(size_t)r * cols + c];
    acc = y ? fmaf(v, y[(size_t)r * cols + c], acc) : acc + v;
  }
  out[c] = acc;
}

__global__ __launch_bounds__(256) void adamw_kernel(float* __restrict__ p, const float* __restrict__ g,
                                                    float* __restrict__ m, float* __restrict__ v, size_t n, float lr,
                                                    float b1, float b2, float eps, float wd, float inv_sqrt_bc2,
                                                    float step_size, float grad_scale) {
  const size_t i = (size_t)blockIdx.x * 256 + threadIdx.x;
  if (i >= n) return;
  const float gi = g[i] * grad_scale;
  float pi = p[i] * (1.f - lr * wd);
  const float mi = b1 * m[i] + (1.f - b1) * gi;
  const float vi = b2 * v[i] + (1.f - b2) * gi * gi;
  const float denom = sqrtf(vi) * inv_sqrt_bc2 + eps;
  pi -= step_size * mi / denom;
  p[i] = pi;
  m[i] = mi;
  v[i] = vi;
}

__global__ __launch_bounds__(256) void matmul_small_kernel(const float* __restrict__ A, const float* __restrict__ B,
                                                           float* __restrict__ C, int M, int N, int K, long sam, long sak,
                                                           long sbk, long sbn, float alpha) {
  const size_t i = (size_t)blockIdx.x * 256 + threadIdx.x;
  if (i >= (size_t)M * N) return;
  const int m = (int)(i / N), n = (int)(i % N);
  float acc = 0.f;
  for (int k = 0; k < K; ++k) acc = fmaf(A[m * sam + k * sak], B[k * sbk + n * sbn], acc);
  C[i] = alpha * acc;
}

static inline unsigned grid_for(size_t total) {
  size_t b = (total + 255) / 256;
  return (unsigned)(b < 1 ? 1 : (b > 8192 ? 8192 : b));
}


__global__ __launch_bounds__(1024) void l1_loss_kernel(const float* __restrict__ a, const float* __restrict__ b, size_t n,
                                                       float* __restrict__ loss, float* __restrict__ da, float gscale) {
  __shared__ float red[16];
  const int lane = threadIdx.x & 63, wave = threadIdx.x >> 6;
  const float g = gscale / (float)n;
  float acc = 0.f;
  for (size_t i = threadIdx.x; i < n; i += 1024) {
    const float d = a[i] - b[i];
    acc += fabsf(d);
    if (da) da[i] = d > 0.f ? g : (d < 0.f ? -g : 0.f);
  }
  acc = wave_sum(acc);
  if (lane == 0) red[wave] = acc;
  __syncthreads();
  if (threadIdx.x == 0) {
    float t = 0.f;
#pragma unroll
    for (int w = 0; w < 16; ++w) t += red[w];
    loss[0] = t / (float)n;
  }
}

__global__ __launch_bounds__(256) void kl_logits_kernel(const float* __restrict__ x, const float* __restrict__ t,
                                                        float* __restrict__ loss_rows, float* __restrict__ dx, int rows,
                                                        int cols, float gscale) {
  const int lane = threadIdx.x & 63;
  const int row = blockIdx.x * 4 + (threadIdx.x >> 6);
  if (row >= rows) return;
  const float* xr = x + (size_t)row * cols;
  const float* tr = t + (size_t)row * cols;
  float mx = -INFINITY, mt = -INFINITY;
  for (int j = lane; j < cols; j += 64) {
    mx = fmaxf(mx, xr[j]);
    mt = fmaxf(mt, tr[j]);
  }
  mx = wave_max(mx);
  mt = wave_max(mt);
  float sx = 0.f, st = 0.f;
  for (int j = lane; j < cols; j += 64) {
    sx += __expf(xr[j] - mx);
    st += __expf(tr[j] - mt);
  }
  sx = wave_sum(sx);
  st = wave_sum(st);
  const float lx = mx + __logf(sx), lt = mt + __logf(st);
  float acc = 0.f;
  for (int j = lane; j < cols; j += 64) {
    const float a = xr[j] - lx, b = tr[j] - lt;
    const float q = __expf(b);
    acc += q * (b - a);
    if (dx) dx[(size_t)row * cols + j] = (__expf(a) - q) * gscale;
  }
  acc = wave_sum(acc);
  if (lane == 0) loss_rows[row] = acc;
}

}

using namespace clipfs;

extern "C" int clipfs_vit_fill_special(float* x, const float* class_emb, const float* pos, const float* vpt, int batch,
                                       int tokens, int n_patch, int n_vpt, int width, void* stream) {
  CLIPFS_REQUIRE(x && class_emb && pos && (n_vpt == 0 || vpt), "vit_fill_special: null pointer");
  CLIPFS_REQUIRE(batch > 0 && width > 0 && n_vpt >= 0 && tokens == 1 + n_patch + n_vpt, "vit_fill_special: tokens %d != 1 + %d + %d", tokens, n_patch, n_vpt);
  const size_t total = (size_t)batch * (1 + n_vpt) * width;
  hipLaunchKernelGGL(vit_fill_special_kernel, dim3(grid_for(total)), dim3(256), 0, (hipStream_t)stream, x, class_emb, pos,
                     vpt, batch, tokens, n_patch, n_vpt, width);
  return launch_status();
}

extern "C" int clipfs_text_embed(const int64_t* ids, const float* table, const float* pos, const float* ctx, int n_ctx,
                                 float* x, int n, int seq, int width, void* stream) {
  CLIPFS_REQUIRE(ids && table && pos && x, "text_embed: null pointer");
  CLIPFS_REQUIRE(n > 0 && seq > 0 && width > 0 && (width & 3) == 0 && (!ctx || (n_ctx > 0 && n_ctx < seq)), "text_embed: bad dims");
  CLIPFS_REQUIRE(aligned16(table) && aligned16(pos) && aligned16(x) && (!ctx || aligned16(ctx)), "text_embed: misaligned pointer");
  const size_t total = (size_t)n * seq * (width / 4);
  hipLaunchKernelGGL(text_embed_kernel, dim3(grid_for(total)), dim3(256), 0, (hipStream_t)stream, ids, table, pos, ctx,
                     n_ctx, x, n, seq, width);
  return launch_status();
}

extern "C" int clipfs_token_rows_grad(const float* dx, float* dctx, int n, int seq, int width, int n_ctx, int first,
                                      void* stream) {
  CLIPFS_REQUIRE(dx && dctx && n > 0 && n_ctx > 0 && first >= 0 && first + n_ctx <= seq && width > 0, "token_rows_grad: bad args");
  hipLaunchKernelGGL(text_ctx_grad_kernel, dim3((n_ctx * width + 255) / 256), dim3(256), 0, (hipStream_t)stream, dx, dctx,
                     n, seq, width, n_ctx, first);
  return launch_status();
}

extern "C" int clipfs_matmul_small(const float* A, const float* B, float* C, int M, int N, int K, long sam, long sak,
                                   long sbk, long sbn, float alpha, void* stream) {
  CLIPFS_REQUIRE(A && B && C && M > 0 && N > 0 && K > 0, "matmul_small: bad args");
  const size_t total = (size_t)M * N;
  hipLaunchKernelGGL(matmul_small_kernel, dim3((unsigned)((total + 255) / 256)), dim3(256), 0, (hipStream_t)stream, A, B, C,
                     M, N, K, sam, sak, sbk, sbn, alpha);
  return launch_status();
}

extern "C" int clipfs_gather_eot(const float* x, const int64_t* ids, float* out, int32_t* idx_out, int n, int seq,
                                 int width, void* stream) {
  CLIPFS_REQUIRE(x && ids && out && n > 0 && seq > 0 && width > 0, "gather_eot: bad args");
  hipLaunchKernelGGL(gather_eot_kernel, dim3(n), dim3(64), 0, (hipStream_t)stream, x, ids, out, idx_out, seq, width);
  return launch_status();
}

extern "C" int clipfs_scatter_rows(const float* dy, const int32_t* idx, float* dx, int n, int seq, int width,
                                   void* stream) {
  CLIPFS_REQUIRE(dy && idx && dx && n > 0 && seq > 0 && width > 0, "scatter_rows: bad args");
  const size_t total = (size_t)n * seq * width;
  hipLaunchKernelGGL(scatter_rows_kernel, dim3(grid_for(total)), dim3(256), 0, (hipStream_t)stream, dy, idx, dx, n, seq,
                     width);
  return launch_status();
}

extern "C" int clipfs_gather_seq_rows(const float* src, size_t ld, const int32_t* idx, float* out, int n, int seq, int width,
                                      void* stream) {
  CLIPFS_REQUIRE(src && idx && out && n > 0 && seq > 0 && width > 0 && ld >= (size_t)width, "gather_seq_rows: bad args");
  hipLaunchKernelGGL(gather_seq_rows_kernel, dim3(grid_for((size_t)n * width)), dim3(256), 0, (hipStream_t)stream, src, ld,
                     idx, out, n, seq, width);
  return launch_status();
}

extern "C" int clipfs_add_seq_rows(const float* src, const int32_t* idx, float* dx, int n, int seq, int width, void* stream) {
  CLIPFS_REQUIRE(src && idx && dx && n > 0 && seq > 0 && width > 0, "add_seq_rows: bad args");
  hipLaunchKernelGGL(add_seq_rows_kernel, dim3(grid_for((size_t)n * width)), dim3(256), 0, (hipStream_t)stream, src, idx, dx,
                     n, seq, width);
  return launch_status();
}

extern "C" int clipfs_put_seq_rows(const float* src, const int32_t* idx, float* dst, size_t ld, int n, int seq, int width,
                                   void* stream) {
  CLIPFS_REQUIRE(src && idx && dst && n > 0 && seq > 0 && width > 0 && ld >= (size_t)width, "put_seq_rows: bad args");
  hipLaunchKernelGGL(put_seq_rows_kernel, dim3(grid_for((size_t)n * width)), dim3(256), 0, (hipStream_t)stream, src, idx, dst,
                     ld, n, seq, width);
  return launch_status();
}

static inline bool rows_map_vec(const void* a, const void* b, size_t ld, int width) {
  return (width % 4) == 0 && (ld % 4) == 0 && aligned16(a) && aligned16(b);
}

extern "C" int clipfs_gather_rows_map(const float* src, size_t ld, const int32_t* map, float* out, int n, int width,
                                      void* stream) {
  CLIPFS_REQUIRE(src && map && out && n > 0 && width > 0 && ld >= (size_t)width, "gather_rows_map: bad args");
  if (rows_map_vec(src, out, ld, width))
    hipLaunchKernelGGL(gather_rows_map_kernel<4>, dim3(grid_for((size_t)n * width / 4)), dim3(256), 0, (hipStream_t)stream,
                       src, ld, map, out, n, width);
  else
// ... 125 lines not shown
```

jittor-clip-fewshot_amd/csrc/tower.hip:

```cpp
#include "common.h"

#include <stdlib.h>

namespace clipfs {

static inline size_t al4(size_t n) { return (n + 3) & ~(size_t)3; }

static inline bool f16_attention(const clipfs_tower* t) { return t->weight_format == 2 && t->seq <= 288; }
static inline bool qkv_f16(const clipfs_tower* t) {
  return f16_attention(t) && (t->width % 128) == 0 && t->lora_r <= 64;
}

struct SavedLayout {
  size_t x_in, stat1, h1, t_qkv, qkv, att, lse, t_o, x_mid, stat2, u, keep, total;
};

static inline bool keep_bits_slot(const clipfs_tower* t) {
  return t->lora_r > 0 && t->lora_dropout > 0.f && clipfs_lora_keep_bits_ok(t->width, t->width, t->lora_r, 3);
}
static inline bool keep_bits_saved(const clipfs_tower* t) { return keep_bits_slot(t) && t->dropout_seed != 0; }

static SavedLayout saved_layout_rows(const clipfs_tower* t, size_t M, size_t batch) {
  const size_t d = t->width, r = t->lora_r > 0 ? t->lora_r : 0;
  SavedLayout L;
// ... 143 lines not shown
  clipfs_gemm_args a = {};
  a.struct_size = sizeof(a);
  a.B_planes = Bp;
  a.b_format = cx.b_format;
  a.workspace = cx.ws;
  a.workspace_floats = cx.ws_floats;
  a.counters = cx.counters;
  a.counters_ints = cx.counters_ints;
  a.A = A; a.B = B; a.C = C; a.M = M; a.N = N; a.K = K;
  a.lda = K; a.ldb = K; a.ldc = N; a.alpha = 1.f;
  a.bias = bias; a.residual = res; a.ldres = N;
  a.act = act; a.aux_out = aux_out; a.aux_in = aux_in;
  a.lora_t = lt; a.lora_b = lb; a.lora_r = r; a.lora_nseg = nseg; a.lora_seg_width = segw; a.lora_scale = lscale;
  if (cx.b_format == 2 && Bp && cx.a16 && (K % 32) == 0 && (!lt || (segw % 128 == 0 && r <= 64))) {
    if (chain & CHAIN_IN16) {
      a.A_f16 = cx.c16;
    } else if (a16_ready) {
      a.A_f16 = a16_ready;
    } else {
      CLIPFS_CHECK(clipfs_convert_f16(A, cx.a16, (size_t)M * K, st));
      a.A_f16 = cx.a16;
    }
    if (chain & CHAIN_OUT16) {
      a.C_f16 = cx.c16;
      a.C = nullptr;
    }
    a.aux_f16 = 1;
    if (c16_only) {
      a.C_f16 = c16_only;
      a.C = nullptr;
    }
  } else {
    CLIPFS_REQUIRE(!c16_only, "tower: the f16 x f16 GEMM is required for an f16-only result");
  }
  return clipfs_gemm_nt(&a, st);
}

static int put_prompt(const clipfs_block& b, float* x, const int32_t* off, int batch, int seq, int d, hipStream_t st) {
  if (!b.prompt) return CLIPFS_OK;
  return clipfs_prompt_put(b.prompt, x, off, batch, seq, b.prompt_first, b.prompt_rows, d, st);
}
static int harvest_prompt(const clipfs_block& b, float* dx, void* dx16, const int32_t* off, int batch, int seq, int d,
                          hipStream_t st) {
  if (!b.prompt) return CLIPFS_OK;
  return clipfs_prompt_harvest(dx, dx16, off, batch, seq, b.prompt_first, b.prompt_rows, d, b.g_prompt, st);
}

static int bias_sum(const float* x, int rows, int cols, int segw, float* o0, float* o1, float* o2, float* work,
                    hipStream_t st) {
  if (!o0 && !o1 && !o2) return CLIPFS_OK;
  return clipfs_bias_grad(x, (size_t)cols, rows, cols, segw, o0, o1, o2, work, st);
}

}

using namespace clipfs;

extern "C" size_t clipfs_tower_saved_floats(const clipfs_tower* t, int batch) {
  if (!t || batch <= 0 || t->struct_size != sizeof(clipfs_tower)) return 0;
  if (t->grad_lo < 0 || t->grad_lo >= t->layers) return 0;
  return saved_layout(t, (size_t)batch * t->seq).total * (size_t)(t->layers - t->grad_lo);
}

extern "C" size_t clipfs_tower_scratch_floats(const clipfs_tower* t, int batch) {
  if (!t || batch <= 0 || t->struct_size != sizeof(clipfs_tower)) return 0;
  return scratch_layout(t, (size_t)batch * t->seq).total;
}

extern "C" size_t clipfs_tower_counter_ints(const clipfs_tower* t, int batch) {
  if (!t || batch <= 0 || t->struct_size != sizeof(clipfs_tower)) return 0;
  return scratch_layout(t, (size_t)batch * t->seq).counter_ints;
}

static bool last_block_rows_ok(const clipfs_tower* t) {
  static const bool force_dense = getenv("CLIPFS_DENSE_BWD") && atoi(getenv("CLIPFS_DENSE_BWD")) != 0;
  const clipfs_block& b = t->blocks[t->layers - 1];
  const bool lora_o = b.lora_a_o && (b.lora_mask & 8u);
  return !(force_dense || lora_o || t->seq < 8);
}

static int tower_fwd_impl(const clipfs_tower* t, float* x, const int32_t* rows, int batch, float* saved, float* scratch,
                          void* stream) {
  CLIPFS_CHECK(check_tower(t, batch));
  CLIPFS_REQUIRE(x && scratch, "tower_fwd: null buffer");
  hipStream_t st = (hipStream_t)stream;
  const int M = batch * t->seq, d = t->width, r = t->lora_r;
  const SavedLayout SL = saved_layout(t, (size_t)M);
  const ScratchLayout SC = scratch_layout(t, (size_t)M);
  const bool train = saved != nullptr;
  const TowerCtx cx = make_ctx(t, scratch, SC);
  CLIPFS_REQUIRE(!t->gemm_counters || t->gemm_counters_ints >= SC.counter_ints,
                 "tower: gemm_counters holds %zu ints, %zu needed", t->gemm_counters_ints, SC.counter_ints);
  const uint64_t seed = t->dropout_seed;
  const int lo = t->grad_lo;
  for (int l = 0; l < t->layers; ++l) {
    const clipfs_block& b = t->blocks[l];
    const bool keep_l = train && l >= lo;
    if (train && l == lo) {
      hipError_t e = hipMemcpyAsync(saved + SL.x_in, x, (size_t)M * d * sizeof(float), hipMemcpyDeviceToDevice, st);
      CLIPFS_REQUIRE(e == hipSuccess, "tower_fwd: memcpy failed: %s", hipGetErrorString(e));
    }
    float* sv = keep_l ? saved + (size_t)(l - lo) * SL.total : nullptr;
    const float* x_in = keep_l ? sv + SL.x_in : x;
    float* h1 = keep_l ? sv + SL.h1 : scratch + SC.h;
    float* qkv = keep_l ? sv + SL.qkv : scratch + SC.b3;
    float* att = keep_l ? sv + SL.att : scratch + SC.b1;
    float* x_mid = keep_l ? sv + SL.x_mid : x;
    float* t_qkv = keep_l ? sv + SL.t_qkv : scratch + SC.dt;
    float* t_o = keep_l ? sv + SL.t_o : scratch + SC.dt + al4((size_t)M * 3 * r);
    float* x_next = keep_l ? (l + 1 < t->layers ? saved + (size_t)(l + 1 - lo) * SL.total + SL.x_in : x) : x;
    float* lse = keep_l ? sv + SL.lse : (train ? scratch + SC.big : nullptr);
    const unsigned qkv_mask = b.lora_a_qkv ? (b.lora_mask & 7u) : 0u;
    const bool lora_o = b.lora_a_o && (b.lora_mask & 8u);
    const uint32_t ds = t->dropout_stream0 + 4u * (uint32_t)l;
    CLIPFS_CHECK(put_prompt(b, const_cast<float*>(x_in), nullptr, batch, t->seq, d, st));

    void* h16 = cx.a16;
    void* dqkv16 = cx.a16 ? (void*)((char*)cx.a16 + (size_t)M * d * 2) : nullptr;
    (void)dqkv16;
    void* keep = (keep_l && qkv_mask && keep_bits_saved(t)) ? (void*)(sv + SL.keep) : nullptr;
    if (qkv_mask && clipfs_layernorm_fwd_lora_ok(d, r, 3)) {
      CLIPFS_CHECK(clipfs_layernorm_fwd_lora(x_in, d, b.ln1_g, b.ln1_b, h1, h16, keep_l ? sv + SL.stat1 : nullptr,
                                             keep_l ? sv + SL.stat1 + M : nullptr, M, d, 1e-5f, b.lora_a_qkv, t_qkv, r, 3, qkv_mask,
                                             t->lora_dropout, seed, ds, t->dropout_row0, keep, st));
    } else {
      if (h16)
        CLIPFS_CHECK(clipfs_layernorm_fwd_f16(x_in, d, b.ln1_g, b.ln1_b, h1, h16, keep_l ? sv + SL.stat1 : nullptr,
                                              keep_l ? sv + SL.stat1 + M : nullptr, M, d, 1e-5f, st));
      else
        CLIPFS_CHECK(clipfs_layernorm_fwd(x_in, d, b.ln1_g, b.ln1_b, h1, keep_l ? sv + SL.stat1 : nullptr,
                                          keep_l ? sv + SL.stat1 + M : nullptr, M, d, 1e-5f, st));
      if (qkv_mask)
        CLIPFS_CHECK(clipfs_lora_down(h1, b.lora_a_qkv, t_qkv, M, d, r, 3, qkv_mask, t->lora_dropout, seed, ds, t->dropout_row0,
                                      keep, st));
    }
    const bool q16 = qkv_f16(t);
    CLIPFS_CHECK(gemm(cx, h1, b.w_qkv, b.w_qkv_p, qkv, M, 3 * d, d, b.b_qkv, nullptr, 0, nullptr, nullptr, qkv_mask ? t_qkv : nullptr,
                      b.lora_b_qkv, r, 3, d, t->lora_scale, st, CHAIN_NONE, h16, q16 ? (void*)qkv : nullptr));
    const void* att16 = nullptr;
    if (f16_attention(t)) {
      CLIPFS_CHECK(clipfs_attention_f16_fwd(qkv, q16, att, h16, lse, batch, t->seq, t->heads, t->causal, st));
      att16 = h16;
    } else
      CLIPFS_CHECK(clipfs_attention_fwd(qkv, att, lse, batch, t->seq, t->heads, t->causal, st));
    if (rows && l == t->layers - 1) {
      const int seq = t->seq, Ms = batch;
      float* att_s = scratch + SC.big;
      float* xin_s = att_s + (size_t)Ms * d;
      float* xmid_s = xin_s + (size_t)Ms * d;
      float* h2_s = xmid_s + (size_t)Ms * d;
      float* xout_s = h2_s + (size_t)Ms * d;
      float* g_s = xout_s + (size_t)Ms * d;
      float* u_s = g_s + (size_t)Ms * 4 * d;
      float* mean_s = u_s + (size_t)Ms * 4 * d;
      float* rstd_s = mean_s + al4((size_t)Ms);
      CLIPFS_CHECK(clipfs_gather_seq_rows(att, (size_t)d, rows, att_s, Ms, seq, d, st));
      CLIPFS_CHECK(clipfs_gather_seq_rows(x_in, (size_t)d, rows, xin_s, Ms, seq, d, st));
      const bool f16m = t->weight_format == 2;
      CLIPFS_CHECK(gemm(cx, att_s, b.w_o, f16m ? nullptr : b.w_o_p, xmid_s, Ms, d, d, b.b_o, xin_s, 0, nullptr, nullptr, nullptr, nullptr,
                        0, 0, 0, 0.f, st));
      CLIPFS_CHECK(clipfs_layernorm_fwd(xmid_s, d, b.ln2_g, b.ln2_b, h2_s, keep_l ? mean_s : nullptr, keep_l ? rstd_s : nullptr, Ms,
                                        d, 1e-5f, st));
      CLIPFS_CHECK(gemm(cx, h2_s, b.w_fc, f16m ? nullptr : b.w_fc_p, g_s, Ms, 4 * d, d, b.b_fc, nullptr, 1, keep_l ? u_s : nullptr,
                        nullptr, nullptr, nullptr, 0, 0, 0, 0.f, st));
      CLIPFS_CHECK(gemm(cx, g_s, b.w_pr, f16m ? nullptr : b.w_pr_p, xout_s, Ms, d, 4 * d, b.b_pr, xmid_s, 0, nullptr, nullptr, nullptr,
                        nullptr, 0, 0, 0, 0.f, st));
      CLIPFS_CHECK(clipfs_put_seq_rows(xout_s, rows, x, (size_t)d, Ms, seq, d, st));
      if (keep_l) {
        CLIPFS_CHECK(clipfs_put_seq_rows(xmid_s, rows, sv + SL.x_mid, (size_t)d, Ms, seq, d, st));
        if (f16m)
          CLIPFS_CHECK(clipfs_put_seq_rows_f16(u_s, rows, sv + SL.u, (size_t)4 * d, Ms, seq, 4 * d, st));
        else
          CLIPFS_CHECK(clipfs_put_seq_rows(u_s, rows, sv + SL.u, (size_t)4 * d, Ms, seq, 4 * d, st));
        CLIPFS_CHECK(clipfs_put_seq_rows(mean_s, rows, sv + SL.stat2, 1, Ms, seq, 1, st));
        CLIPFS_CHECK(clipfs_put_seq_rows(rstd_s, rows, sv + SL.stat2 + M, 1, Ms, seq, 1, st));
      }
      break;
    }
    if (lora_o)
      CLIPFS_CHECK(clipfs_lora_down(att, b.lora_a_o, t_o, M, d, r, 1, 1u, t->lora_dropout, seed, ds + 3, t->dropout_row0, nullptr, st));
    CLIPFS_CHECK(gemm(cx, att, b.w_o, b.w_o_p, x_mid, M, d, d, b.b_o, x_in, 0, nullptr, nullptr, lora_o ? t_o : nullptr, b.lora_b_o, r,
                      1, d, t->lora_scale, st, CHAIN_NONE, att16));
    float* h2 = scratch + SC.h;
    if (h16)
      CLIPFS_CHECK(clipfs_layernorm_fwd_f16(x_mid, d, b.ln2_g, b.ln2_b, nullptr, h16, keep_l ? sv + SL.stat2 : nullptr,
                                            keep_l ? sv + SL.stat2 + M : nullptr, M, d, 1e-5f, st));
    else
      CLIPFS_CHECK(clipfs_layernorm_fwd(x_mid, d, b.ln2_g, b.ln2_b, h2, keep_l ? sv + SL.stat2 : nullptr,
                                        keep_l ? sv + SL.stat2 + M : nullptr, M, d, 1e-5f, st));
    float* gbuf = scratch + SC.big;
    CLIPFS_CHECK(gemm(cx, h2, b.w_fc, b.w_fc_p, gbuf, M, 4 * d, d, b.b_fc, nullptr, 1, keep_l ? sv + SL.u : nullptr, nullptr, nullptr,
                      nullptr, 0, 0, 0, 0.f, st, CHAIN_OUT16, h16));
    CLIPFS_CHECK(gemm(cx, gbuf, b.w_pr, b.w_pr_p, x_next, M, d, 4 * d, b.b_pr, x_mid, 0, nullptr, nullptr, nullptr, nullptr, 0, 0, 0,
                      0.f, st, CHAIN_IN16));
  }
  return CLIPFS_OK;
}

extern "C" int clipfs_tower_fwd(const clipfs_tower* t, float* x, int batch, float* saved, float* scratch, void* stream) {
  return tower_fwd_impl(t, x, nullptr, batch, saved, scratch, stream);
}

extern "C" int clipfs_tower_fwd_rows(const clipfs_tower* t, float* x, const int32_t* rows, int batch, float* saved,
                                     float* scratch, void* stream) {
  CLIPFS_REQUIRE(t && rows, "tower_fwd_rows: null argument");
  CLIPFS_CHECK(check_tower(t, batch));
  return tower_fwd_impl(t, x, last_block_rows_ok(t) ? rows : nullptr, batch, saved, scratch, stream);
}

extern "C" int clipfs_tower_rows_mode(const clipfs_tower* t) {
  return (t && t->blocks && t->layers > 0 && last_block_rows_ok(t)) ? 1 : 0;
}

static int lora_bwd_block(const clipfs_tower* t, bool dy16, const float* dy, const void* dy16p, const float* x,
                          const float* tt, const float* A, const float* B, float* dt, float* gA, float* gB, float* dx,
                          int M, int nseg, unsigned mask, uint32_t ds, const void* keep, float* work, hipStream_t st, int l) {
  CLIPFS_REQUIRE((gA == nullptr) == (gB == nullptr), "tower_bwd: block %d has only one of the LoRA gradient slots", l);
  if (!gA && !dx) return CLIPFS_OK;
  const int d = t->width, r = t->lora_r;
  if (dy16)
    return clipfs_lora_bwd_f16dy(dy16p, x, tt, A, B, dt, gA, gB, dx, M, d, d, r, nseg, mask, t->lora_scale, t->lora_dropout,
                                 t->dropout_seed, ds, t->dropout_row0, keep, work, st);
  return clipfs_lora_bwd(dy, x, tt, A, B, dt, gA, gB, dx, M, d, d, r, nseg, mask, t->lora_scale, t->lora_dropout,
                         t->dropout_seed, ds, t->dropout_row0, keep, work, st);
}

static int tower_bwd_range(const clipfs_tower* t, float* dx, int batch, const float* saved, float* scratch,
                           int stop_at_input, hipStream_t st, int l_hi) {
  const int M = batch * t->seq, d = t->width, r = t->lora_r;
  const SavedLayout SL = saved_layout(t, (size_t)M);
  const ScratchLayout SC = scratch_layout(t, (size_t)M);
  const TowerCtx cx = make_ctx(t, scratch, SC);
  void* h16 = cx.a16;
  void* dqkv16 = cx.a16 ? (void*)((char*)cx.a16 + (size_t)M * d * 2) : nullptr;
  if (h16) CLIPFS_CHECK(clipfs_convert_f16(dx, h16, (size_t)M * d, st));
  const int lo = t->grad_lo;
  for (int l = l_hi; l >= lo; --l) {
    const clipfs_block& b = t->blocks[l];
    const float* sv = saved + (size_t)(l - lo) * SL.total;
    CLIPFS_REQUIRE(b.w_pr_t && b.w_fc_t && b.w_o_t && b.w_qkv_t, "tower_bwd: block %d lacks transposed weights", l);
    CLIPFS_REQUIRE(t->weight_format != 2 || (b.w_pr_t_p && b.w_fc_t_p && b.w_o_t_p && b.w_qkv_t_p),
                   "tower_bwd: block %d lacks f16 copies of the transposed weights", l);
    const unsigned qkv_mask = b.lora_a_qkv ? (b.lora_mask & 7u) : 0u;
    const bool lora_o = b.lora_a_o && (b.lora_mask & 8u);
    const uint32_t ds = t->dropout_stream0 + 4u * (uint32_t)l;
    float* du = scratch + SC.big;
    float* dh = scratch + SC.h;
    float* datt = scratch + SC.b1;
    float* dqkv = scratch + SC.b3;
    float* dt = scratch + SC.dt;
    float* work = scratch + SC.work;
    float* bwork = scratch + SC.bwork;
    CLIPFS_CHECK(bias_sum(dx, M, d, d, b.g_b_pr, nullptr, nullptr, bwork, st));
    CLIPFS_CHECK(gemm(cx, dx, b.w_pr_t, b.w_pr_t_p, du, M, 4 * d, d, nullptr, nullptr, 2, nullptr, sv + SL.u, nullptr, nullptr, 0, 0, 0,
                      0.f, st, CHAIN_OUT16, h16));
    CLIPFS_CHECK(bias_sum(du, M, 4 * d, 4 * d, b.g_b_fc, nullptr, nullptr, bwork, st));
    CLIPFS_CHECK(gemm(cx, du, b.w_fc_t, b.w_fc_t_p, dh, M, d, 4 * d, nullptr, nullptr, 0, nullptr, nullptr, nullptr, nullptr, 0, 0, 0, 0.f,
                      st, CHAIN_IN16));
    CLIPFS_CHECK(bias_sum(dh, M, d, d, b.g_ln2_b, nullptr, nullptr, bwork, st));
    if (h16)
      CLIPFS_CHECK(clipfs_layernorm_bwd_f16(dh, sv + SL.x_mid, d, b.ln2_g, sv + SL.stat2, sv + SL.stat2 + M, dx, dx, h16, d,
                                            M, d, st));
    else
      CLIPFS_CHECK(clipfs_layernorm_bwd(dh, sv + SL.x_mid, d, b.ln2_g, sv + SL.stat2, sv + SL.stat2 + M, dx, dx, d, M, d,
// ... 43 lines not shown
                                int stop_at_input, void* stream) {
  CLIPFS_CHECK(check_tower(t, batch));
  CLIPFS_REQUIRE(t->grad_lo == 0 || stop_at_input,
                 "tower_bwd: grad_lo %d > 0 needs stop_at_input (the input gradient runs through every block)", t->grad_lo);
  CLIPFS_REQUIRE(dx && saved && scratch, "tower_bwd: null buffer");
  const ScratchLayout SC = scratch_layout(t, (size_t)batch * t->seq);
  CLIPFS_REQUIRE(!t->gemm_counters || t->gemm_counters_ints >= SC.counter_ints,
                 "tower: gemm_counters holds %zu ints, %zu needed", t->gemm_counters_ints, SC.counter_ints);
  return tower_bwd_range(t, dx, batch, saved, scratch, stop_at_input, (hipStream_t)stream, t->layers - 1);
}

struct PackPlan {
  const int32_t* off;
  const int32_t* eotp;
  const int32_t* map;
  int R;
};

static bool pack_dropout_ok(const clipfs_tower* t) {
  const bool drop = t->lora_r > 0 && t->lora_dropout > 0.f && t->dropout_seed != 0;
  if (!drop) return true;
  for (int l = t->grad_lo; l < t->layers; ++l) {
    const clipfs_block& b = t->blocks[l];
    if (b.lora_a_o && (b.lora_mask & 8u)) return false;
    if (b.lora_a_qkv && (b.lora_mask & 7u) && !keep_bits_saved(t)) return false;
  }
  return true;
}

constexpr int kPackMinRows = 2048;

static bool pack_ok(const clipfs_tower* t, int batch, int R) {
  const int M = batch * t->seq, d = t->width, r = t->lora_r;
  if (M < kPackMinRows) return false;
  if (!t->causal || t->weight_format == 2 || !last_block_rows_ok(t)) return false;
  if (!clipfs_attention_bwd_packed_ok(t->seq, 1)) return false;
  if (R < batch || 2 * (size_t)R > (size_t)M || (d % 8) != 0) return false;
  if (!pack_dropout_ok(t)) return false;
  const ScratchLayout SC = scratch_layout(t, (size_t)M);
  if (r > 0) {
    const size_t need = al4(clipfs_lora_bwd_work_floats(R, d, r, 3));
    if (need > SC.gemm_ws - SC.work) return false;
  }
  if (tower_has_bias_slots(t)) {
    const int widths[3] = {d, 3 * d, 4 * d};
    for (int i = 0; i < 3; ++i)
      if (clipfs_bias_grad_work_floats(R, widths[i]) > SC.total - SC.bwork) return false;
  }
  return true;
}

static int tower_bwd_packed_range(const clipfs_tower* t, float* dx, int batch, const PackPlan& P, const float* saved,
                                  float* scratch, int stop_at_input, hipStream_t st, int l_hi, bool attn_only_top,
                                  bool saved_packed) {
  const int M = batch * t->seq, d = t->width, r = t->lora_r, R = P.R;
  const SavedLayout SL = saved_packed ? saved_layout_packed(t, (size_t)R, (size_t)batch) : saved_layout(t, (size_t)M);
  const int srows = saved_packed ? R : M;
  const ScratchLayout SC = scratch_layout(t, (size_t)M);
  const TowerCtx cx = make_ctx(t, scratch, SC);
  const size_t Rd = (size_t)R * d;
  float* datt_p = scratch + SC.b1;
  float* dx_p = datt_p + al4(Rd);
  float* dh_p = scratch + SC.h;
  float* du_p = scratch + SC.big;
  float* u_p = du_p + 4 * Rd;
  float* dqkv_p = scratch + SC.b3;
  float* h1_p = scratch + SC.big;
  float* tq_p = h1_p + al4(Rd);
  float* keep_p = tq_p + al4((size_t)R * 3 * r);
  float* att_p = keep_p + al4((size_t)R * d / 8);
  float* to_p = att_p + al4(Rd);
  float* dt = scratch + SC.dt;
  float* work = scratch + SC.work;
  float* bwork = scratch + SC.bwork;
  const int lo = t->grad_lo;
  for (int l = l_hi; l >= lo; --l) {
    const clipfs_block& b = t->blocks[l];
    const float* sv = saved + (size_t)(l - lo) * SL.total;
    CLIPFS_REQUIRE(b.w_pr_t && b.w_fc_t && b.w_o_t && b.w_qkv_t, "tower_bwd: block %d lacks transposed weights", l);
    const unsigned qkv_mask = b.lora_a_qkv ? (b.lora_mask & 7u) : 0u;
    const bool lora_o = b.lora_a_o && (b.lora_mask & 8u);
    const uint32_t ds = t->dropout_stream0 + 4u * (uint32_t)l;
    if (!(attn_only_top && l == l_hi)) {
      CLIPFS_CHECK(bias_sum(dx_p, R, d, d, b.g_b_pr, nullptr, nullptr, bwork, st));
      if (!saved_packed) CLIPFS_CHECK(clipfs_gather_rows_map(sv + SL.u, (size_t)4 * d, P.map, u_p, R, 4 * d, st));
      CLIPFS_CHECK(gemm(cx, dx_p, b.w_pr_t, b.w_pr_t_p, du_p, R, 4 * d, d, nullptr, nullptr, 2, nullptr,
                        saved_packed ? sv + SL.u : u_p, nullptr, nullptr, 0, 0, 0, 0.f, st));
      CLIPFS_CHECK(bias_sum(du_p, R, 4 * d, 4 * d, b.g_b_fc, nullptr, nullptr, bwork, st));
      CLIPFS_CHECK(gemm(cx, du_p, b.w_fc_t, b.w_fc_t_p, dh_p, R, d, 4 * d, nullptr, nullptr, 0, nullptr, nullptr, nullptr, nullptr, 0,
                        0, 0, 0.f, st));
      CLIPFS_CHECK(bias_sum(dh_p, R, d, d, b.g_ln2_b, nullptr, nullptr, bwork, st));
      if (saved_packed)
        CLIPFS_CHECK(clipfs_layernorm_bwd(dh_p, sv + SL.x_mid, d, b.ln2_g, sv + SL.stat2, sv + SL.stat2 + srows, dx_p, dx_p, d,
                                          R, d, st));
      else
        CLIPFS_CHECK(clipfs_layernorm_bwd_rows(dh_p, sv + SL.x_mid, d, b.ln2_g, sv + SL.stat2, sv + SL.stat2 + srows, P.map,
                                               dx_p, dx_p, d, R, d, st));
      CLIPFS_CHECK(bias_sum(dx_p, R, d, d, b.g_b_o, nullptr, nullptr, bwork, st));
      CLIPFS_CHECK(gemm(cx, dx_p, b.w_o_t, b.w_o_t_p, datt_p, R, d, d, nullptr, nullptr, 0, nullptr, nullptr, nullptr, nullptr, 0, 0,
                        0, 0.f, st));
      if (lora_o) {
        if (!saved_packed) {
          CLIPFS_CHECK(clipfs_gather_rows_map(sv + SL.att, (size_t)d, P.map, att_p, R, d, st));
          CLIPFS_CHECK(clipfs_gather_rows_map(sv + SL.t_o, (size_t)r, P.map, to_p, R, r, st));
        }
        CLIPFS_CHECK(lora_bwd_block(t, false, dx_p, nullptr, saved_packed ? sv + SL.att : att_p, saved_packed ? sv + SL.t_o : to_p,
                                    b.lora_a_o, b.lora_b_o, dt, b.g_lora_a_o, b.g_lora_b_o, datt_p, R, 1, 1u, ds + 3, nullptr,
                                    work, st, l));
      }
    }
    if (saved_packed)
      CLIPFS_CHECK(clipfs_attention_bwd_packed_io(sv + SL.qkv, datt_p, sv + SL.att, sv + SL.lse, dqkv_p, P.off, batch, t->seq,
                                                  t->heads, st));
    else
      CLIPFS_CHECK(clipfs_attention_bwd_packed(sv + SL.qkv, datt_p, sv + SL.att, sv + SL.lse, dqkv_p, P.off, batch, t->seq,
                                               t->heads, st));
    CLIPFS_CHECK(bias_sum(dqkv_p, R, 3 * d, d, b.g_b_q, b.g_b_k, b.g_b_v, bwork, st));
    const bool need_dx = !(l == lo && stop_at_input) || b.g_prompt;
    const bool need_dh = need_dx || b.g_ln1_b;
    if (need_dh)
      CLIPFS_CHECK(gemm(cx, dqkv_p, b.w_qkv_t, b.w_qkv_t_p, dh_p, R, d, 3 * d, nullptr, nullptr, 0, nullptr, nullptr, nullptr, nullptr,
                        0, 0, 0, 0.f, st));
    if (qkv_mask && (b.g_lora_a_qkv || need_dh)) {
      const bool keep = keep_bits_saved(t);
      if (!saved_packed) {
        CLIPFS_CHECK(clipfs_gather_rows_map(sv + SL.h1, (size_t)d, P.map, h1_p, R, d, st));
        CLIPFS_CHECK(clipfs_gather_rows_map(sv + SL.t_qkv, (size_t)3 * r, P.map, tq_p, R, 3 * r, st));
        if (keep)
          CLIPFS_CHECK(clipfs_gather_rows_map(sv + SL.keep, (size_t)d / 8, P.map, keep_p, R, d / 8, st));
      }
      CLIPFS_CHECK(lora_bwd_block(t, false, dqkv_p, nullptr, saved_packed ? sv + SL.h1 : h1_p, saved_packed ? sv + SL.t_qkv : tq_p,
                                  b.lora_a_qkv, b.lora_b_qkv, dt, b.g_lora_a_qkv, b.g_lora_b_qkv, need_dh ? dh_p : nullptr, R, 3,
                                  qkv_mask, ds, keep ? (saved_packed ? (const void*)(sv + SL.keep) : (const void*)keep_p) : nullptr,
                                  work, st, l));
    }
    CLIPFS_CHECK(bias_sum(dh_p, R, d, d, b.g_ln1_b, nullptr, nullptr, bwork, st));
    if (need_dx) {
      if (saved_packed)
        CLIPFS_CHECK(clipfs_layernorm_bwd(dh_p, sv + SL.x_in, d, b.ln1_g, sv + SL.stat1, sv + SL.stat1 + srows, dx_p, dx_p, d, R,
                                          d, st));
      else
        CLIPFS_CHECK(clipfs_layernorm_bwd_rows(dh_p, sv + SL.x_in, d, b.ln1_g, sv + SL.stat1, sv + SL.stat1 + srows, P.map,
                                               dx_p, dx_p, d, R, d, st));
      CLIPFS_CHECK(harvest_prompt(b, dx_p, nullptr, P.off, batch, t->seq, d, st));
    }
  }
  if (stop_at_input) return CLIPFS_OK;
  hipError_t e = hipMemsetAsync(dx, 0, (size_t)M * d * sizeof(float), st);
  CLIPFS_REQUIRE(e == hipSuccess, "tower_bwd_packed: memset failed: %s", hipGetErrorString(e));
  return clipfs_put_rows_map(dx_p, P.map, dx, (size_t)d, R, d, st);
}

static int tower_bwd_sparse_impl(const clipfs_tower* t, const float* dxs, const int32_t* rows, float* dx, int batch,
                                 const float* saved, float* scratch, int stop_at_input, hipStream_t st, const PackPlan* P,
                                 bool saved_packed = false) {
  const int seq = t->seq, M = batch * seq, d = t->width, r = t->lora_r, Ms = batch;
  const SavedLayout SL = saved_packed ? saved_layout_packed(t, (size_t)P->R, (size_t)batch) : saved_layout(t, (size_t)M);
  const ScratchLayout SC = scratch_layout(t, (size_t)M);
  CLIPFS_REQUIRE(!t->gemm_counters || t->gemm_counters_ints >= SC.counter_ints,
                 "tower: gemm_counters holds %zu ints, %zu needed", t->gemm_counters_ints, SC.counter_ints);
  const int l = t->layers - 1;
  const clipfs_block& b = t->blocks[l];
  if (!last_block_rows_ok(t)) {
    CLIPFS_CHECK(clipfs_scatter_rows(dxs, rows, dx, batch, seq, d, st));
    return tower_bwd_range(t, dx, batch, saved, scratch, stop_at_input, st, l);
  }
  CLIPFS_REQUIRE(b.w_pr_t && b.w_fc_t && b.w_o_t && b.w_qkv_t, "tower_bwd: block %d lacks transposed weights", l);
  const TowerCtx cx = make_ctx(t, scratch, SC);
  const float* sv = saved + (size_t)(l - t->grad_lo) * SL.total;
  float* u_s = scratch + SC.big;
  float* du_s = u_s + (size_t)Ms * 4 * d;
  float* xmid_s = du_s + (size_t)Ms * 4 * d;
  float* dh_s = xmid_s + (size_t)Ms * d;
  float* dxm_s = dh_s + (size_t)Ms * d;
  float* datt_s = dxm_s + (size_t)Ms * d;
  float* mean_s = datt_s + (size_t)Ms * d;
  float* rstd_s = mean_s + al4((size_t)Ms);
  float* bwork = scratch + SC.bwork;
  CLIPFS_CHECK(bias_sum(dxs, Ms, d, d, b.g_b_pr, nullptr, nullptr, bwork, st));
  const bool f16m = t->weight_format == 2;
  if (saved_packed) {
    CLIPFS_CHECK(clipfs_gather_rows_map(sv + SL.u, (size_t)4 * d, P->eotp, u_s, Ms, 4 * d, st));
    CLIPFS_CHECK(clipfs_gather_rows_map(sv + SL.x_mid, (size_t)d, P->eotp, xmid_s, Ms, d, st));
    CLIPFS_CHECK(clipfs_gather_rows_map(sv + SL.stat2, 1, P->eotp, mean_s, Ms, 1, st));
    CLIPFS_CHECK(clipfs_gather_rows_map(sv + SL.stat2 + P->R, 1, P->eotp, rstd_s, Ms, 1, st));
  } else {
    if (f16m)
      CLIPFS_CHECK(clipfs_gather_seq_rows_f16(sv + SL.u, (size_t)4 * d, rows, u_s, Ms, seq, 4 * d, st));
    else
      CLIPFS_CHECK(clipfs_gather_seq_rows(sv + SL.u, (size_t)4 * d, rows, u_s, Ms, seq, 4 * d, st));
    CLIPFS_CHECK(clipfs_gather_seq_rows(sv + SL.x_mid, (size_t)d, rows, xmid_s, Ms, seq, d, st));
    CLIPFS_CHECK(clipfs_gather_seq_rows(sv + SL.stat2, 1, rows, mean_s, Ms, seq, 1, st));
    CLIPFS_CHECK(clipfs_gather_seq_rows(sv + SL.stat2 + M, 1, rows, rstd_s, Ms, seq, 1, st));
  }
  CLIPFS_CHECK(gemm(cx, dxs, b.w_pr_t, f16m ? nullptr : b.w_pr_t_p, du_s, Ms, 4 * d, d, nullptr, nullptr, 2, nullptr, u_s, nullptr, nullptr,
                    0, 0, 0, 0.f, st));
  CLIPFS_CHECK(bias_sum(du_s, Ms, 4 * d, 4 * d, b.g_b_fc, nullptr, nullptr, bwork, st));
  CLIPFS_CHECK(gemm(cx, du_s, b.w_fc_t, f16m ? nullptr : b.w_fc_t_p, dh_s, Ms, d, 4 * d, nullptr, nullptr, 0, nullptr, nullptr, nullptr,
                    nullptr, 0, 0, 0, 0.f, st));
  CLIPFS_CHECK(bias_sum(dh_s, Ms, d, d, b.g_ln2_b, nullptr, nullptr, bwork, st));
  CLIPFS_CHECK(clipfs_layernorm_bwd(dh_s, xmid_s, d, b.ln2_g, mean_s, rstd_s, dxs, dxm_s, d, Ms, d, st));
  CLIPFS_CHECK(bias_sum(dxm_s, Ms, d, d, b.g_b_o, nullptr, nullptr, bwork, st));
  CLIPFS_CHECK(gemm(cx, dxm_s, b.w_o_t, f16m ? nullptr : b.w_o_t_p, datt_s, Ms, d, d, nullptr, nullptr, 0, nullptr, nullptr, nullptr,
                    nullptr, 0, 0, 0, 0.f, st));
  if (P) {
    float* datt_p = scratch + SC.b1;
    const size_t Rd = (size_t)P->R * d;
    hipError_t e = hipMemsetAsync(datt_p, 0, (al4(Rd) + Rd) * sizeof(float), st);
    CLIPFS_REQUIRE(e == hipSuccess, "tower_bwd_packed: memset failed: %s", hipGetErrorString(e));
    CLIPFS_CHECK(clipfs_put_rows_map(datt_s, P->eotp, datt_p, (size_t)d, Ms, d, st));
    CLIPFS_CHECK(clipfs_put_rows_map(dxm_s, P->eotp, datt_p + al4(Rd), (size_t)d, Ms, d, st));
    return tower_bwd_packed_range(t, dx, batch, *P, saved, scratch, stop_at_input, st, l, true, saved_packed);
  }
  float* dh = scratch + SC.h;
  float* datt = scratch + SC.b1;
  float* dqkv = scratch + SC.b3;
  float* dt = scratch + SC.dt;
  float* work = scratch + SC.work;
  CLIPFS_CHECK(clipfs_scatter_rows(datt_s, rows, datt, batch, seq, d, st));
  const unsigned qkv_mask = b.lora_a_qkv ? (b.lora_mask & 7u) : 0u;
  const void* dqkv16_ready = nullptr;
  void* dqkv16 = (f16_attention(t) && cx.a16) ? (void*)((char*)cx.a16 + (size_t)M * d * 2) : nullptr;
  const bool dy16 = dqkv16 && (!qkv_mask || clipfs_lora_bwd_f16dy_ok(d, d, r, 3));
  if (f16_attention(t)) {
    CLIPFS_CHECK(clipfs_attention_f16_bwd(sv + SL.qkv, qkv_f16(t), datt, 0, sv + SL.att, sv + SL.lse, dy16 ? nullptr : dqkv, dqkv16,
                                          dh, batch, seq, t->heads, t->causal, st));
    dqkv16_ready = dqkv16;
  } else
    CLIPFS_CHECK(clipfs_attention_bwd(sv + SL.qkv, datt, sv + SL.att, sv + SL.lse, dqkv, dh, batch, seq, t->heads, t->causal, st));
  CLIPFS_CHECK(bias_sum(dqkv, M, 3 * d, d, b.g_b_q, b.g_b_k, b.g_b_v, bwork, st));
  const uint32_t ds = t->dropout_stream0 + 4u * (uint32_t)l;
  const bool need_dx = !(l == t->grad_lo && stop_at_input) || b.g_prompt;
  const bool need_dh = need_dx || b.g_ln1_b;
  if (need_dh)
    CLIPFS_CHECK(gemm(cx, dqkv, b.w_qkv_t, b.w_qkv_t_p, dh, M, d, 3 * d, nullptr, nullptr, 0, nullptr, nullptr, nullptr, nullptr, 0, 0,
                      0, 0.f, st, CHAIN_NONE, dqkv16_ready));
  if (qkv_mask)
    CLIPFS_CHECK(lora_bwd_block(t, dy16, dqkv, dqkv16, sv + SL.h1, sv + SL.t_qkv, b.lora_a_qkv, b.lora_b_qkv, dt,
                                b.g_lora_a_qkv, b.g_lora_b_qkv, need_dh ? dh : nullptr, M, 3, qkv_mask, ds,
                                keep_bits_saved(t) ? (const void*)(sv + SL.keep) : nullptr, work, st, l));
  CLIPFS_CHECK(bias_sum(dh, M, d, d, b.g_ln1_b, nullptr, nullptr, bwork, st));
  if (!need_dx) return CLIPFS_OK;
  CLIPFS_CHECK(clipfs_layernorm_bwd(dh, sv + SL.x_in, d, b.ln1_g, sv + SL.stat1, sv + SL.stat1 + M, nullptr, dx, d, M, d, st));
  CLIPFS_CHECK(clipfs_add_seq_rows(dxm_s, rows, dx, batch, seq, d, st));
  CLIPFS_CHECK(harvest_prompt(b, dx, nullptr, nullptr, batch, seq, d, st));
  return tower_bwd_range(t, dx, batch, saved, scratch, stop_at_input, st, l - 1);
}

extern "C" int clipfs_tower_bwd_sparse(const clipfs_tower* t, const float* dxs, const int32_t* rows, float* dx, int batch,
                                       const float* saved, float* scratch, int stop_at_input, void* stream) {
  CLIPFS_CHECK(check_tower(t, batch));
  CLIPFS_REQUIRE(t->grad_lo == 0 || stop_at_input,
                 "tower_bwd_sparse: grad_lo %d > 0 needs stop_at_input (the input gradient runs through every block)",
                 t->grad_lo);
  CLIPFS_REQUIRE(dxs && rows && dx && saved && scratch, "tower_bwd_sparse: null buffer");
  return tower_bwd_sparse_impl(t, dxs, rows, dx, batch, saved, scratch, stop_at_input, (hipStream_t)stream, nullptr);
}

extern "C" int clipfs_tower_pack_mode(const clipfs_tower* t, int batch, int R) {
  if (!t || !t->blocks || t->struct_size != sizeof(clipfs_tower) || t->block_size != sizeof(clipfs_block)) return 0;
  if (batch <= 0 || t->layers <= 0 || t->seq <= 0 || t->grad_lo < 0 || t->grad_lo >= t->layers) return 0;
  return pack_ok(t, batch, R) ? 1 : 0;
}

extern "C" int clipfs_tower_bwd_packed(const clipfs_tower* t, const float* dxs, const int32_t* rows, const int32_t* plan,
                                       int R, float* dx, int batch, const float* saved, float* scratch, int stop_at_input,
                                       void* stream) {
  CLIPFS_CHECK(check_tower(t, batch));
  CLIPFS_REQUIRE(t->grad_lo == 0 || stop_at_input,
                 "tower_bwd_packed: grad_lo %d > 0 needs stop_at_input (the input gradient runs through every block)",
                 t->grad_lo);
  CLIPFS_REQUIRE(dxs && rows && plan && dx && saved && scratch, "tower_bwd_packed: null buffer");
  CLIPFS_REQUIRE(R >= batch && (size_t)R <= (size_t)batch * t->seq, "tower_bwd_packed: R %d outside [batch %d, batch*seq %zu]",
                 R, batch, (size_t)batch * t->seq);
  hipStream_t st = (hipStream_t)stream;
  if (!pack_ok(t, batch, R))
    return tower_bwd_sparse_impl(t, dxs, rows, dx, batch, saved, scratch, stop_at_input, st, nullptr);
  const PackPlan P = {plan, plan + batch + 1, plan + 2 * (size_t)batch + 1, R};
  return tower_bwd_sparse_impl(t, dxs, rows, dx, batch, saved, scratch, stop_at_input, st, &P);
}

static bool pack_fwd_ok(const clipfs_tower* t, int batch, int R) {
  if (!pack_ok(t, batch, R) || t->weight_format != 0) return false;
  const int M = batch * t->seq, d = t->width, r = t->lora_r;
  const int shapes[4][2] = {{3 * d, d}, {d, d}, {4 * d, d}, {d, 4 * d}};
  for (int i = 0; i < 4; ++i)
    if (clipfs_gemm_workspace_floats(M, shapes[i][0], shapes[i][1]) != 0) return false;
// ... 9 lines not shown
static int tower_fwd_packed_impl(const clipfs_tower* t, float* x, const int32_t* rows, const PackPlan& P, int batch,
                                 float* saved, float* scratch, hipStream_t st) {
  const int seq = t->seq, M = batch * seq, d = t->width, r = t->lora_r, R = P.R;
  const size_t Rd = (size_t)R * d;
  const SavedLayout SL = saved_layout_packed(t, (size_t)R, (size_t)batch);
  const ScratchLayout SC = scratch_layout(t, (size_t)M);
  CLIPFS_REQUIRE(!t->gemm_counters || t->gemm_counters_ints >= SC.counter_ints,
                 "tower: gemm_counters holds %zu ints, %zu needed", t->gemm_counters_ints, SC.counter_ints);
  const TowerCtx cx = make_ctx(t, scratch, SC);
  TowerCtx cxp = cx;
  cxp.ws = nullptr;
  cxp.ws_floats = 0;
  cxp.counters = nullptr;
  cxp.counters_ints = 0;
  const bool train = saved != nullptr;
  const uint64_t seed = t->dropout_seed;
  const int lo = t->grad_lo;
  float* x_p = scratch + SC.b1 + al4(Rd);
  CLIPFS_CHECK(clipfs_gather_rows_map(x, (size_t)d, P.map, train && lo == 0 ? saved + SL.x_in : x_p, R, d, st));
  for (int l = 0; l < t->layers; ++l) {
    const clipfs_block& b = t->blocks[l];
    const bool keep_l = train && l >= lo;
    if (train && l == lo && lo > 0) {
      hipError_t e = hipMemcpyAsync(saved + SL.x_in, x_p, Rd * sizeof(float), hipMemcpyDeviceToDevice, st);
      CLIPFS_REQUIRE(e == hipSuccess, "tower_fwd_packed: memcpy failed: %s", hipGetErrorString(e));
    }
    float* sv = keep_l ? saved + (size_t)(l - lo) * SL.total : nullptr;
    const float* x_in = keep_l ? sv + SL.x_in : x_p;
    float* h1 = keep_l ? sv + SL.h1 : scratch + SC.h;
    float* qkv = keep_l ? sv + SL.qkv : scratch + SC.b3;
    float* att = keep_l ? sv + SL.att : scratch + SC.b1;
    float* x_mid = keep_l ? sv + SL.x_mid : x_p;
    float* t_qkv = keep_l ? sv + SL.t_qkv : scratch + SC.dt;
    float* t_o = keep_l ? sv + SL.t_o : scratch + SC.dt + al4((size_t)R * 3 * r);
    float* x_next = keep_l && l + 1 < t->layers ? saved + (size_t)(l + 1 - lo) * SL.total + SL.x_in : x_p;
    float* lse = keep_l ? sv + SL.lse : nullptr;
    const unsigned qkv_mask = b.lora_a_qkv ? (b.lora_mask & 7u) : 0u;
    const bool lora_o = b.lora_a_o && (b.lora_mask & 8u);
    const uint32_t ds = t->dropout_stream0 + 4u * (uint32_t)l;
    float* mean1 = keep_l ? sv + SL.stat1 : nullptr;
    float* rstd1 = keep_l ? sv + SL.stat1 + R : nullptr;
    CLIPFS_CHECK(put_prompt(b, const_cast<float*>(x_in), P.off, batch, seq, d, st));
    void* keep = (keep_l && qkv_mask && keep_bits_saved(t)) ? (void*)(sv + SL.keep) : nullptr;
    if (qkv_mask && clipfs_layernorm_fwd_lora_ok(d, r, 3)) {
      CLIPFS_CHECK(clipfs_layernorm_fwd_lora_map(x_in, d, b.ln1_g, b.ln1_b, h1, nullptr, mean1, rstd1, R, d, 1e-5f, b.lora_a_qkv,
                                                 t_qkv, r, 3, qkv_mask, t->lora_dropout, seed, ds, t->dropout_row0, P.map, keep,
                                                 st));
    } else {
      CLIPFS_CHECK(clipfs_layernorm_fwd(x_in, d, b.ln1_g, b.ln1_b, h1, mean1, rstd1, R, d, 1e-5f, st));
      if (qkv_mask)
        CLIPFS_CHECK(clipfs_lora_down(h1, b.lora_a_qkv, t_qkv, R, d, r, 3, qkv_mask, t->lora_dropout, seed, ds, t->dropout_row0,
                                      keep, st));
    }
    CLIPFS_CHECK(gemm(cxp, h1, b.w_qkv, b.w_qkv_p, qkv, R, 3 * d, d, b.b_qkv, nullptr, 0, nullptr, nullptr,
                      qkv_mask ? t_qkv : nullptr, b.lora_b_qkv, r, 3, d, t->lora_scale, st));
    CLIPFS_CHECK(clipfs_attention_fwd_packed(qkv, att, lse, P.off, batch, seq, t->heads, st));
    if (l == t->layers - 1) {
      const int Ms = batch;
      float* att_s = scratch + SC.big;
      float* xin_s = att_s + (size_t)Ms * d;
      float* xmid_s = xin_s + (size_t)Ms * d;
      float* h2_s = xmid_s + (size_t)Ms * d;
      float* xout_s = h2_s + (size_t)Ms * d;
      float* g_s = xout_s + (size_t)Ms * d;
      float* u_s = g_s + (size_t)Ms * 4 * d;
      float* mean_s = u_s + (size_t)Ms * 4 * d;
      float* rstd_s = mean_s + al4((size_t)Ms);
      CLIPFS_CHECK(clipfs_gather_rows_map(att, (size_t)d, P.eotp, att_s, Ms, d, st));
      CLIPFS_CHECK(clipfs_gather_rows_map(x_in, (size_t)d, P.eotp, xin_s, Ms, d, st));
      CLIPFS_CHECK(gemm(cx, att_s, b.w_o, b.w_o_p, xmid_s, Ms, d, d, b.b_o, xin_s, 0, nullptr, nullptr, nullptr, nullptr, 0, 0, 0,
                        0.f, st));
      CLIPFS_CHECK(clipfs_layernorm_fwd(xmid_s, d, b.ln2_g, b.ln2_b, h2_s, keep_l ? mean_s : nullptr, keep_l ? rstd_s : nullptr, Ms,
                                        d, 1e-5f, st));
      CLIPFS_CHECK(gemm(cx, h2_s, b.w_fc, b.w_fc_p, g_s, Ms, 4 * d, d, b.b_fc, nullptr, 1, keep_l ? u_s : nullptr, nullptr, nullptr,
                        nullptr, 0, 0, 0, 0.f, st));
      CLIPFS_CHECK(gemm(cx, g_s, b.w_pr, b.w_pr_p, xout_s, Ms, d, 4 * d, b.b_pr, xmid_s, 0, nullptr, nullptr, nullptr, nullptr, 0, 0,
                        0, 0.f, st));
      CLIPFS_CHECK(clipfs_put_seq_rows(xout_s, rows, x, (size_t)d, Ms, seq, d, st));
      if (keep_l) {
        CLIPFS_CHECK(clipfs_put_rows_map(xmid_s, P.eotp, sv + SL.x_mid, (size_t)d, Ms, d, st));
        CLIPFS_CHECK(clipfs_put_rows_map(u_s, P.eotp, sv + SL.u, (size_t)4 * d, Ms, 4 * d, st));
        CLIPFS_CHECK(clipfs_put_rows_map(mean_s, P.eotp, sv + SL.stat2, 1, Ms, 1, st));
        CLIPFS_CHECK(clipfs_put_rows_map(rstd_s, P.eotp, sv + SL.stat2 + R, 1, Ms, 1, st));
      }
      break;
    }
    if (lora_o)
      CLIPFS_CHECK(clipfs_lora_down(att, b.lora_a_o, t_o, R, d, r, 1, 1u, t->lora_dropout, seed, ds + 3, t->dropout_row0, nullptr,
                                    st));
    CLIPFS_CHECK(gemm(cxp, att, b.w_o, b.w_o_p, x_mid, R, d, d, b.b_o, x_in, 0, nullptr, nullptr, lora_o ? t_o : nullptr, b.lora_b_o,
                      r, 1, d, t->lora_scale, st));
    float* h2 = scratch + SC.h;
    CLIPFS_CHECK(clipfs_layernorm_fwd(x_mid, d, b.ln2_g, b.ln2_b, h2, keep_l ? sv + SL.stat2 : nullptr,
                                      keep_l ? sv + SL.stat2 + R : nullptr, R, d, 1e-5f, st));
    float* gbuf = scratch + SC.big;
    CLIPFS_CHECK(gemm(cxp, h2, b.w_fc, b.w_fc_p, gbuf, R, 4 * d, d, b.b_fc, nullptr, 1, keep_l ? sv + SL.u : nullptr, nullptr, nullptr,
                      nullptr, 0, 0, 0, 0.f, st));
    CLIPFS_CHECK(gemm(cxp, gbuf, b.w_pr, b.w_pr_p, x_next, R, d, 4 * d, b.b_pr, x_mid, 0, nullptr, nullptr, nullptr, nullptr, 0, 0, 0,
                      0.f, st));
  }
  return CLIPFS_OK;
}

extern "C" int clipfs_tower_pack_fwd_mode(const clipfs_tower* t, int batch, int R) {
  if (!t || !t->blocks || t->struct_size != sizeof(clipfs_tower) || t->block_size != sizeof(clipfs_block)) return 0;
  if (batch <= 0 || t->layers <= 0 || t->seq <= 0 || t->grad_lo < 0 || t->grad_lo >= t->layers) return 0;
  return pack_fwd_ok(t, batch, R) ? 1 : 0;
}

// ... 27 lines not shown
```

Measured before the change: 4867 images/s.

## Compute last-block attention only for the pooled query row in both towers

In the final transformer block only one token per sequence (EOT for text, class token for vision) feeds the output. The change adds one-query attention forward and backward kernels and row-selected QKV projection and dgrad paths. It uses them in the last layer so that Q and the attention output are produced only for the pooled row, while K and V are still computed for every row. The aim is to cut wasted QKV GEMM work and attention work in the top block, at the cost of extra kernels, more special cases, and a global mode toggle.

```diff
diff --git a/include/clipfs.h b/include/clipfs.h
--- a/include/clipfs.h
+++ b/include/clipfs.h
@@ -93,6 +93,12 @@
                                 void* stream);
 int clipfs_attention_bwd_packed_io(const float* qkv, const float* dout, const float* out, const float* lse, float* dqkv,
                                    const int32_t* off, int batch, int seq, int heads, void* stream);
+int clipfs_attention_one_ok(int seq);
+int clipfs_attention_fwd_one(const float* qkv, float* out, float* lse, const int32_t* rows, const int32_t* off, int batch,
+                             int seq, int heads, int causal, void* stream);
+int clipfs_attention_bwd_one(const float* qkv, const float* dout, const float* out, const float* lse, float* dqkv,
+                             const int32_t* rows, const int32_t* off, int packed_io, int batch, int seq, int heads,
+                             int causal, void* stream);
 int clipfs_attention_f16_fwd(const void* qkv, int qkv_f16, float* out, void* out16, float* lse, int batch, int seq,
                              int heads, int causal, void* stream);
 int clipfs_attention_f16_bwd(const void* qkv, int qkv_f16, const void* dout, int dout_f16, const float* out,
@@ -122,6 +128,8 @@
                            void* stream);
 int clipfs_matmul_small(const float* A, const float* B, float* C, int M, int N, int K, long sam, long sak,
                         long sbk, long sbn, float alpha, void* stream);
+int clipfs_matmul_small_ref(const float* A, const float* B, float* C, int M, int N, int K, long sam, long sak,
+                            long sbk, long sbn, float alpha, void* stream);
 int clipfs_gather_eot(const float* x, const int64_t* ids, float* out, int32_t* idx_out, int n, int seq,
                       int width, void* stream);
 int clipfs_scatter_rows(const float* dy, const int32_t* idx, float* dx, int n, int seq, int width, void* stream);
@@ -229,6 +237,8 @@
 int clipfs_tower_fwd_rows(const clipfs_tower* t, float* x, const int32_t* rows, int batch, float* saved, float* scratch,
                           void* stream);
 int clipfs_tower_rows_mode(const clipfs_tower* t);
+int clipfs_tower_one_query_mode(const clipfs_tower* t, int batch);
+int clipfs_tower_one_query(int enable);
 int clipfs_tower_bwd(const clipfs_tower* t, float* dx, int batch, const float* saved, float* scratch,
                      int stop_at_input, void* stream);
 int clipfs_tower_bwd_sparse(const clipfs_tower* t, const float* dxs, const int32_t* rows, float* dx, int batch,
diff --git a/jittor-clip-fewshot_amd/clipfs/_lib.py b/jittor-clip-fewshot_amd/clipfs/_lib.py
--- a/jittor-clip-fewshot_amd/clipfs/_lib.py
+++ b/jittor-clip-fewshot_amd/clipfs/_lib.py
@@ -100,6 +100,7 @@
     "clipfs_text_embed": (_i, [_p, _p, _p, _p, _i, _p, _i, _i, _i, _p]),
     "clipfs_token_rows_grad": (_i, [_p, _p, _i, _i, _i, _i, _i, _p]),
     "clipfs_matmul_small": (_i, [_p, _p, _p, _i, _i, _i, C.c_long, C.c_long, C.c_long, C.c_long, _f, _p]),
+    "clipfs_matmul_small_ref": (_i, [_p, _p, _p, _i, _i, _i, C.c_long, C.c_long, C.c_long, C.c_long, _f, _p]),
     "clipfs_gather_eot": (_i, [_p, _p, _p, _p, _i, _i, _i, _p]),
     "clipfs_scatter_rows": (_i, [_p, _p, _p, _i, _i, _i, _p]),
     "clipfs_gather_seq_rows": (_i, [_p, _sz, _p, _p, _i, _i, _i, _p]),
@@ -155,6 +156,11 @@
                                            _p, _p]),
     "clipfs_attention_fwd_packed": (_i, [_p, _p, _p, _p, _i, _i, _i, _p]),
     "clipfs_attention_bwd_packed_io": (_i, [_p, _p, _p, _p, _p, _p, _i, _i, _i, _p]),
+    "clipfs_attention_one_ok": (_i, [_i]),
+    "clipfs_attention_fwd_one": (_i, [_p, _p, _p, _p, _p, _i, _i, _i, _i, _p]),
+    "clipfs_attention_bwd_one": (_i, [_p, _p, _p, _p, _p, _p, _p, _i, _i, _i, _i, _i, _p]),
+    "clipfs_tower_one_query_mode": (_i, [C.POINTER(Tower), _i]),
+    "clipfs_tower_one_query": (_i, [_i]),
     "clipfs_tower_pack_fwd_mode": (_i, [C.POINTER(Tower), _i, _i]),
     "clipfs_tower_fwd_packed": (_i, [C.POINTER(Tower), _p, _p, _p, _i, _i, _p, _p, _p]),
     "clipfs_tower_bwd_packed_saved": (_i, [C.POINTER(Tower), _p, _p, _p, _i, _p, _i, _p, _p, _i, _p]),
diff --git a/jittor-clip-fewshot_amd/clipfs/engine.py b/jittor-clip-fewshot_amd/clipfs/engine.py
--- a/jittor-clip-fewshot_amd/clipfs/engine.py
+++ b/jittor-clip-fewshot_amd/clipfs/engine.py
@@ -64,6 +64,7 @@
         self.lora_r = 0
         self.lora_scale = 0.0
         self.lora_dropout = 0.0
+        self.one_query = True
 
     def _transposed(self, i: int, blk) -> Dict[str, torch.Tensor]:
         wt = self._wt.get(i)
@@ -191,6 +192,11 @@
     def has_lora(self) -> bool:
         return any(getattr(b.attn, "is_lora_mha", False) and b.attn.r > 0 for b in self.mod.resblocks)
 
+    def _lib_for_call(self):
+        lib = _lib.load()
+        lib.clipfs_tower_one_query(int(self.one_query))
+        return lib
+
     def buffer(self, kind: str, n_floats: int, device) -> torch.Tensor:
         key = (kind, n_floats)
         buf = self._bufs.get(key)
@@ -214,7 +220,7 @@
     def forward(self, x: torch.Tensor, batch: int, train: bool, seed: int, seq: Optional[int] = None,
                 own_saved: bool = False, row0: int = 0, rows: Optional[torch.Tensor] = None, grad_lo: int = 0,
                 pack: Optional[Tuple[torch.Tensor, int]] = None, desc: Optional[Tower] = None):
-        lib = _lib.load()
+        lib = self._lib_for_call()
         t = desc if desc is not None else self.descriptor(train, seed, seq, row0, grad_lo if train else 0)
         self._attach_counters(t, batch, x.device)
         scratch = self.buffer("scratch", lib.clipfs_tower_scratch_floats(C.byref(t), batch), x.device)
@@ -240,7 +246,7 @@
 
     def backward(self, dx: torch.Tensor, batch: int, saved: torch.Tensor, seed: int, stop_at_input: bool,
                  seq: Optional[int] = None, row0: int = 0, grad_lo: int = 0):
-        lib = _lib.load()
+        lib = self._lib_for_call()
         t = self.descriptor(True, seed, seq, row0, grad_lo)
         self._attach_counters(t, batch, dx.device)
         scratch = self.buffer("scratch", lib.clipfs_tower_scratch_floats(C.byref(t), batch), dx.device)
@@ -250,7 +256,7 @@
 
     def backward_sparse(self, dxs: torch.Tensor, rows: torch.Tensor, batch: int, saved: torch.Tensor, seed: int,
                         stop_at_input: bool, seq: Optional[int] = None, row0: int = 0, grad_lo: int = 0) -> torch.Tensor:
-        lib = _lib.load()
+        lib = self._lib_for_call()
         t = self.descriptor(True, seed, seq, row0, grad_lo)
         self._attach_counters(t, batch, dxs.device)
         scratch = self.buffer("scratch", lib.clipfs_tower_scratch_floats(C.byref(t), batch), dxs.device)
@@ -263,7 +269,7 @@
     def backward_packed(self, dxs: torch.Tensor, rows: torch.Tensor, plan: torch.Tensor, R: int, batch: int,
                         saved: torch.Tensor, seed: int, stop_at_input: bool, seq: Optional[int] = None, row0: int = 0,
                         grad_lo: int = 0, saved_packed: bool = False) -> torch.Tensor:
-        lib = _lib.load()
+        lib = self._lib_for_call()
         t = self.descriptor(True, seed, seq, row0, grad_lo)
         self._attach_counters(t, batch, dxs.device)
         scratch = self.buffer("scratch", lib.clipfs_tower_scratch_floats(C.byref(t), batch), dxs.device)
@@ -273,6 +279,10 @@
                  scratch.data_ptr(), int(stop_at_input), torch.cuda.current_stream().cuda_stream),
               "tower_bwd_packed_saved" if saved_packed else "tower_bwd_packed")
         return dx
+
+    def one_query_mode(self, batch: int, seed: int = 0, seq: Optional[int] = None, train: bool = True) -> bool:
+        t = self.descriptor(train, seed, seq, 0, 0)
+        return bool(self._lib_for_call().clipfs_tower_one_query_mode(C.byref(t), batch))
 
     def pack_mode(self, batch: int, R: int, seed: int, seq: Optional[int] = None, grad_lo: int = 0,
                   train: bool = True) -> bool:
@@ -307,6 +317,14 @@
         self.pack_text_backward = True
         self.pack_text_forward = True
         self._pack_cache = {}
+
+    @property
+    def one_query_last_block(self) -> bool:
+        return self.vis.one_query and self.txt.one_query
+
+    @one_query_last_block.setter
+    def one_query_last_block(self, on: bool) -> None:
+        self.vis.one_query = self.txt.one_query = bool(on)
 
     @property
     def precision(self) -> str:
diff --git a/jittor-clip-fewshot_amd/clipfs/ops.py b/jittor-clip-fewshot_amd/clipfs/ops.py
--- a/jittor-clip-fewshot_amd/clipfs/ops.py
+++ b/jittor-clip-fewshot_amd/clipfs/ops.py
@@ -277,6 +277,14 @@
     return out
 
 
+def matmul_small_ref(a, b, M, N, K, sam, sak, sbk, sbn, alpha=1.0, out=None):
+    if out is None:
+        out = torch.empty(M, N, device=a.device, dtype=torch.float32)
+    check(_lib.load().clipfs_matmul_small_ref(_p(a), _p(b), _p(out), M, N, K, sam, sak, sbk, sbn, alpha, _stream()),
+          "matmul_small_ref")
+    return out
+
+
 def eot_index(ids: torch.Tensor) -> torch.Tensor:
     assert ids.is_cuda and ids.dtype == torch.int64 and ids.is_contiguous()
     n, seq = ids.shape
diff --git a/jittor-clip-fewshot_amd/csrc/attention.hip b/jittor-clip-fewshot_amd/csrc/attention.hip
--- a/jittor-clip-fewshot_amd/csrc/attention.hip
+++ b/jittor-clip-fewshot_amd/csrc/attention.hip
@@ -601,6 +601,11 @@
                            const int32_t* off, int batch, int seq, int heads, bool pin, hipStream_t st);
 int attention16_fwd_packed(const float* qkv, float* out, float* lse, const int32_t* off, int batch, int seq, int heads,
                            hipStream_t st);
+int attention16_fwd_one(const float* qkv, float* out, float* lse, const int32_t* rows, const int32_t* off, int batch, int seq,
+                        int heads, int causal, hipStream_t st);
+int attention16_bwd_one(const float* qkv, const float* dout, const float* out, const float* lse, float* dqkv,
+                        const int32_t* rows, const int32_t* off, bool pin, int batch, int seq, int heads, int causal,
+                        hipStream_t st);
 
 static int check_attn(const char* what, int batch, int seq, int heads, int max_seq) {
   CLIPFS_REQUIRE(batch > 0 && heads > 0 && seq > 0 && seq <= max_seq, "%s: batch %d seq %d heads %d unsupported (seq <= %d)",
@@ -753,6 +758,31 @@
   return attention16_bwd_packed(qkv, dout, out, lse, dqkv, off, batch, seq, heads, true, (hipStream_t)stream);
 }
 
+extern "C" int clipfs_attention_one_ok(int seq) {
+  return (seq > 0 && seq <= ATTN_MFMA_MAX && attention_mfma_enabled() && attention16_enabled(seq)) ? 1 : 0;
+}
+
+extern "C" int clipfs_attention_fwd_one(const float* qkv, float* out, float* lse, const int32_t* rows, const int32_t* off,
+                                        int batch, int seq, int heads, int causal, void* stream) {
+  CLIPFS_CHECK(check_attn("attention_fwd_one", batch, seq, heads, ATTN_MAX_SEQ));
+  CLIPFS_REQUIRE(clipfs_attention_one_ok(seq), "attention_fwd_one: seq %d has no one-query kernel", seq);
+  CLIPFS_REQUIRE(qkv && out && (rows || off), "attention_fwd_one: null pointer");
+  CLIPFS_REQUIRE(aligned16(qkv) && aligned16(out), "attention_fwd_one: misaligned pointer");
+  return attention16_fwd_one(qkv, out, lse, rows, off, batch, seq, heads, causal, (hipStream_t)stream);
+}
+
+extern "C" int clipfs_attention_bwd_one(const float* qkv, const float* dout, const float* out, const float* lse, float* dqkv,
+                                        const int32_t* rows, const int32_t* off, int packed_io, int batch, int seq, int heads,
+                                        int causal, void* stream) {
+  CLIPFS_CHECK(check_attn("attention_bwd_one", batch, seq, heads, ATTN_MAX_SEQ));
+  CLIPFS_REQUIRE(clipfs_attention_one_ok(seq), "attention_bwd_one: seq %d has no one-query kernel", seq);
+  CLIPFS_REQUIRE(qkv && dout && out && lse && dqkv && (rows || off), "attention_bwd_one: null pointer");
+  CLIPFS_REQUIRE(off || !packed_io, "attention_bwd_one: packed q/k/v need the plan's offsets");
+  CLIPFS_REQUIRE(aligned16(qkv) && aligned16(dout) && aligned16(out) && aligned16(dqkv), "attention_bwd_one: misaligned pointer");
+  return attention16_bwd_one(qkv, dout, out, lse, dqkv, rows, off, packed_io != 0, batch, seq, heads, causal,
+                             (hipStream_t)stream);
+}
+
 extern "C" size_t clipfs_attention_lse_floats(int batch, int seq, int heads) {
   if (attention_mfma_enabled() && seq <= ATTN_MFMA_MAX) return (size_t)batch * heads * seq;
   return seq > ATTN_FAST_MAX ? (size_t)batch * heads * seq : 0;
diff --git a/jittor-clip-fewshot_amd/csrc/attention_mfma16.hip b/jittor-clip-fewshot_amd/csrc/attention_mfma16.hip
--- a/jittor-clip-fewshot_amd/csrc/attention_mfma16.hip
+++ b/jittor-clip-fewshot_amd/csrc/attention_mfma16.hip
@@ -94,10 +94,11 @@
     default: a16_scores<(NT >= 6 ? 6 : 1), TP>(IMG, lane, OWN, ACC); break; \
   }
 
-template <int NT, bool PACKED = false>
+template <int NT, bool PACKED = false, bool ONE = false>
 __global__ __launch_bounds__(64 * NT) void attention16_fwd_kernel(const float* __restrict__ qkv, float* __restrict__ out,
                                                                   float* __restrict__ lse, int L, int H, int causal,
-                                                                  const int32_t* __restrict__ off) {
+                                                                  const int32_t* __restrict__ off,
+                                                                  const int32_t* __restrict__ rows) {
   extern __shared__ __attribute__((aligned(16))) float a16_smem[];
   constexpr int TP = 16 * NT + 8;
   float* sKt = a16_smem;
@@ -114,6 +115,8 @@
   const size_t prow = PACKED ? (size_t)off[b] : (size_t)b * L;
   const int Lb = PACKED ? (int)(off[b + 1] - prow) : L;
   if (PACKED && (Lb <= 0 || Lb > L)) return;
+  const int qrow = ONE ? (PACKED ? Lb - 1 : (int)rows[b]) : 0;
+  if (ONE && (qrow < 0 || qrow >= Lb)) return;
   const int klim = causal ? q_tok : Lb - 1;
   const int na = causal ? qt + 1 : NT;
   const float* hq = qkv + prow * ld + (size_t)h * A16_HD;
@@ -121,11 +124,16 @@
   a16_fetch<NT>(hq + d, ld, Lb, kst);
   a16_fetch<NT>(hq + 2 * d, ld, Lb, vst);
   float qf[16];
-  a16_load_own(hq, ld, min(q_tok, Lb - 1), lane, qf);
+  a16_load_own(hq, ld, ONE ? qrow : min(q_tok, Lb - 1), lane, qf);
+  if (ONE && q_tok != qrow) {
+#pragma unroll
+    for (int j = 0; j < 16; ++j) qf[j] = 0.f;
+  }
   a16_put<NT>(sKt, kst, Lb);
   a16_put<NT>(sVt, vst, Lb);
   __syncthreads();
   if (PACKED && 16 * qt >= Lb) return;
+  if (ONE && qt != (qrow >> 4)) return;
   f32x4 s[A16_MAX_TILES];
   A16_SWITCH_SCORES(na, sKt, qf, s)
   float m = -INFINITY;
@@ -157,17 +165,18 @@
 #pragma unroll
   for (int t = 0; t < NT; ++t)
     if (t < na) a16_accum<TP>(sVt, lane, t, s[t], o);
-  if (q_tok < Lb) {
+  if (q_tok < Lb && (!ONE || q_tok == qrow)) {
     a16_store(out + (prow + q_tok) * d + h * A16_HD, o, 1.f / l, lane);
     if (lse && g == 0) lse[((size_t)b * H + h) * L + q_tok] = (m + log2f(l)) * (1.f / A16_LOG2E);
   }
 }
 
-template <int NT, bool PACKED, bool PIN>
+template <int NT, bool PACKED, bool PIN, bool ONE>
 __device__ __forceinline__ void attention16_bwd_q_body(const float* __restrict__ qkv, const float* __restrict__ dout,
                                                        const float* __restrict__ out, const float* __restrict__ lse,
                                                        float* __restrict__ dqkv, int L, int H, int causal, int item,
-                                                       const int32_t* __restrict__ off, float* a16_smem) {
+                                                       const int32_t* __restrict__ off, const int32_t* __restrict__ rows,
+                                                       float* a16_smem) {
   constexpr int TP = 16 * NT + 8;
   float* sKt = a16_smem;
   float* sVt = sKt + 64 * TP;
@@ -180,7 +189,9 @@
   const size_t prow = PACKED ? (size_t)off[b] : (size_t)b * L;
   const size_t irow = PIN ? prow : (size_t)b * L;
   const int Lb = PACKED ? (int)(off[b + 1] - prow) : L;
-  const int q_tok = 16 * qt + (lane & 15), q_cl = min(q_tok, Lb - 1);
+  const int qrow = ONE ? (PACKED ? Lb - 1 : (int)rows[b]) : 0;
+  if (ONE && (Lb <= 0 || Lb > L || qrow < 0 || qrow >= Lb)) return;
+  const int q_tok = 16 * qt + (lane & 15), q_cl = ONE ? qrow : min(q_tok, Lb - 1);
   const float c = 0.125f * A16_LOG2E;
   const int klim = causal ? q_tok : Lb - 1;
   const int na = causal ? qt + 1 : (Lb + 15) / 16;
@@ -190,7 +201,14 @@
   a16_fetch<NT>(hq + 2 * d, ld, Lb, vst);
   float qf[16], gf[16];
   a16_load_own(hq, ld, q_cl, lane, qf);
-  a16_load_own(dout + prow * d + (size_t)h * A16_HD, (size_t)d, q_cl, lane, gf);
+  if (ONE)
+    a16_load_own(dout + (size_t)b * d + (size_t)h * A16_HD, (size_t)d, 0, lane, gf);
+  else
+    a16_load_own(dout + prow * d + (size_t)h * A16_HD, (size_t)d, q_cl, lane, gf);
+  if (ONE && q_tok != qrow) {
+#pragma unroll
+    for (int j = 0; j < 16; ++j) qf[j] = gf[j] = 0.f;
+  }
   float Di = 0.f;
   {
     const float* op = out + (irow + q_cl) * d + h * A16_HD + 16 * g;
@@ -207,32 +225,39 @@
   Di = a16_allreduce_sum(Di);
   __syncthreads();
   if (PACKED && 16 * qt >= Lb) return;
-  f32x4 s[A16_MAX_TILES], dp[A16_MAX_TILES];
-  A16_SWITCH_SCORES(na, sKt, qf, s)
-  A16_SWITCH_SCORES(na, sVt, gf, dp)
   f32x4 acc[4];
 #pragma unroll
   for (int ft = 0; ft < 4; ++ft) acc[ft] = f32x4{0.f, 0.f, 0.f, 0.f};
-#pragma unroll
-  for (int t = 0; t < NT; ++t)
-    if (t < na) {
-      f32x4 ds;
-#pragma unroll
-      for (int r = 0; r < 4; ++r) {
-        const int key = 16 * t + 4 * g + r;
-        const float p = (key < Lb && key <= klim) ? __builtin_amdgcn_exp2f(s[t][r] * c - lse2) : 0.f;
-        ds[r] = p * (dp[t][r] - Di) * 0.125f;
+  if (!ONE || qt == (qrow >> 4)) {
+    f32x4 s[A16_MAX_TILES], dp[A16_MAX_TILES];
+    A16_SWITCH_SCORES(na, sKt, qf, s)
+    A16_SWITCH_SCORES(na, sVt, gf, dp)
+#pragma unroll
+    for (int t = 0; t < NT; ++t)
+      if (t < na) {
+        f32x4 ds;
+#pragma unroll
+        for (int r = 0; r < 4; ++r) {
+          const int key = 16 * t + 4 * g + r;
+          const float p = (key < Lb && key <= klim) ? __builtin_amdgcn_exp2f(s[t][r] * c - lse2) : 0.f;
+          ds[r] = p * (dp[t][r] - Di) * 0.125f;
+        }
+        a16_accum<TP>(sKt, lane, t, ds, acc);
       }
-      a16_accum<TP>(sKt, lane, t, ds, acc);
+    if (ONE && q_tok != qrow) {
+#pragma unroll
+      for (int ft = 0; ft < 4; ++ft) acc[ft] = f32x4{0.f, 0.f, 0.f, 0.f};
     }
+  }
   if (q_tok < Lb) a16_store(dqkv + (prow + q_tok) * ld + h * A16_HD, acc, 1.f, lane);
 }
 
-template <int NT, bool PACKED, bool PIN>
+template <int NT, bool PACKED, bool PIN, bool ONE>
 __device__ __forceinline__ void attention16_bwd_kv_body(const float* __restrict__ qkv, const float* __restrict__ dout,
                                                         const float* __restrict__ out, const float* __restrict__ lse,
                                                         float* __restrict__ dqkv, int L, int H, int causal, int item,
-                                                        const int32_t* __restrict__ off, float* a16_smem) {
+                                                        const int32_t* __restrict__ off, const int32_t* __restrict__ rows,
+                                                        float* a16_smem) {
   constexpr int Lp = 16 * NT, TP = Lp + 8;
   float* sQt = a16_smem;
   float* sGt = sQt + 64 * TP;
@@ -248,18 +273,36 @@
   const size_t prow = PACKED ? (size_t)off[b] : (size_t)b * L;
   const size_t irow = PIN ? prow : (size_t)b * L;
   const int Lb = PACKED ? (int)(off[b + 1] - prow) : L;
+  const int qrow = ONE ? (PACKED ? Lb - 1 : (int)rows[b]) : 0;
+  if (ONE && (Lb <= 0 || Lb > L || qrow < 0 || qrow >= Lb)) return;
   const int k_tok = 16 * kt + (lane & 15), k_cl = min(k_tok, Lb - 1);
   const float c = 0.125f * A16_LOG2E;
-  const int t_first = causal ? kt : 0;
-  const int na = (PACKED ? (Lb + 15) / 16 : NT) - t_first;
+  const int t_first = ONE ? (qrow >> 4) : (causal ? kt : 0);
+  const int na = ONE ? ((causal && kt > t_first) ? 0 : 1) : (PACKED ? (Lb + 15) / 16 : NT) - t_first;
   const float* sQ1 = sQt + 16 * t_first;
   const float* sG1 = sGt + 16 * t_first;
   const float* hq = qkv + irow * ld + (size_t)h * A16_HD;
-  const int vtok = min((int)threadIdx.x, Lb - 1);
+  const int vtok = ONE ? qrow : min((int)threadIdx.x, Lb - 1);
   f32x4 qst[4], gst[4], ost[4];
-  a16_fetch<NT>(hq, ld, Lb, qst);
-  a16_fetch<NT>(dout + prow * d + (size_t)h * A16_HD, (size_t)d, Lb, gst);
-  a16_fetch<NT>(out + irow * d + (size_t)h * A16_HD, (size_t)d, Lb, ost);
+  if (ONE) {
+    const float* q1 = hq + (size_t)qrow * ld;
+    const float* g1 = dout + (size_t)b * d + (size_t)h * A16_HD;
+    const float* o1 = out + (irow + qrow) * d + (size_t)h * A16_HD;
+#pragma unroll
+    for (int k = 0; k < 4; ++k) {
+      const int idx = (int)threadIdx.x + k * 64 * NT;
+      const int c4 = idx / Lp, tok = idx - c4 * Lp;
+      const f32x4 z = f32x4{0.f, 0.f, 0.f, 0.f};
+      const bool hit = tok == qrow;
+      qst[k] = hit ? *reinterpret_cast<const f32x4*>(q1 + 4 * c4) : z;
+      gst[k] = hit ? *reinterpret_cast<const f32x4*>(g1 + 4 * c4) : z;
+      ost[k] = hit ? *reinterpret_cast<const f32x4*>(o1 + 4 * c4) : z;
+    }
+  } else {
+    a16_fetch<NT>(hq, ld, Lb, qst);
+    a16_fetch<NT>(dout + prow * d + (size_t)h * A16_HD, (size_t)d, Lb, gst);
+    a16_fetch<NT>(out + irow * d + (size_t)h * A16_HD, (size_t)d, Lb, ost);
+  }
   float kf[16], vf[16];
   a16_load_own(hq + d, ld, k_cl, lane, kf);
   a16_load_own(hq + 2 * d, ld, k_cl, lane, vf);
@@ -277,14 +320,17 @@
     float d_i = 0.f;
 #pragma unroll
     for (int c = 0; c < 16; ++c) d_i += sPart[c * Lp + threadIdx.x];
-    sLse[threadIdx.x] = (int)threadIdx.x < Lb ? lse_i * A16_LOG2E : 0.f;
-    sD[threadIdx.x] = (int)threadIdx.x < Lb ? d_i : 0.f;
+    const bool live = ONE ? (int)threadIdx.x == qrow : (int)threadIdx.x < Lb;
+    sLse[threadIdx.x] = live ? lse_i * A16_LOG2E : 0.f;
+    sD[threadIdx.x] = live ? d_i : 0.f;
   }
   __syncthreads();
-  if (PACKED && na <= 0) return;
+  if (PACKED && (ONE ? 16 * kt >= Lb : na <= 0)) return;
   f32x4 s[A16_MAX_TILES], dp[A16_MAX_TILES];
-  A16_SWITCH_SCORES(na, sQ1, kf, s)
-  A16_SWITCH_SCORES(na, sG1, vf, dp)
+  if (!ONE || na > 0) {
+    A16_SWITCH_SCORES(na, sQ1, kf, s)
+    A16_SWITCH_SCORES(na, sG1, vf, dp)
+  }
   f32x4 av[4], ak[4];
 #pragma unroll
   for (int ft = 0; ft < 4; ++ft) {
@@ -292,7 +338,7 @@
     ak[ft] = f32x4{0.f, 0.f, 0.f, 0.f};
   }
 #pragma unroll
-  for (int u = 0; u < NT; ++u)
+  for (int u = 0; u < (ONE ? 1 : NT); ++u)
     if (u < na) {
       const int t = t_first + u;
       const f32x4 l4 = *reinterpret_cast<const f32x4*>(sLse + 16 * t + 4 * g);
@@ -314,17 +360,18 @@
   }
 }
 
-template <int NT, bool PACKED = false, bool PIN = false>
+template <int NT, bool PACKED = false, bool PIN = false, bool ONE = false>
 __global__ __launch_bounds__(64 * NT) void attention16_bwd_kernel(const float* __restrict__ qkv, const float* __restrict__ dout,
                                                                   const float* __restrict__ out, const float* __restrict__ lse,
                                                                   float* __restrict__ dqkv, int L, int H, int causal,
-                                                                  const int32_t* __restrict__ off) {
+                                                                  const int32_t* __restrict__ off,
+                                                                  const int32_t* __restrict__ rows) {
   extern __shared__ __attribute__((aligned(16))) float a16_smem[];
   const int item = blockIdx.x >> 1;
   if (blockIdx.x & 1)
-    attention16_bwd_kv_body<NT, PACKED, PIN>(qkv, dout, out, lse, dqkv, L, H, causal, item, off, a16_smem);
+    attention16_bwd_kv_body<NT, PACKED, PIN, ONE>(qkv, dout, out, lse, dqkv, L, H, causal, item, off, rows, a16_smem);
   else
-    attention16_bwd_q_body<NT, PACKED, PIN>(qkv, dout, out, lse, dqkv, L, H, causal, item, off, a16_smem);
+    attention16_bwd_q_body<NT, PACKED, PIN, ONE>(qkv, dout, out, lse, dqkv, L, H, causal, item, off, rows, a16_smem);
 }
 
 
@@ -337,32 +384,33 @@
   return ((size_t)2 * 64 * (16 * nt + 8) + (vectors ? 18 * (size_t)16 * nt : 0)) * sizeof(float);
 }
 
-template <int NT, bool PACKED = false>
+template <int NT, bool PACKED = false, bool ONE = false>
 static int a16_fwd(const float* qkv, float* out, float* lse, int batch, int seq, int heads, int causal, hipStream_t st,
-                   const int32_t* off = nullptr) {
+                   const int32_t* off = nullptr, const int32_t* rows = nullptr) {
   static bool attr = false;
   if (!attr && a16_lds(NT, false) > 48 * 1024) {
-    (void)hipFuncSetAttribute(reinterpret_cast<const void*>(&attention16_fwd_kernel<NT, PACKED>),
+    (void)hipFuncSetAttribute(reinterpret_cast<const void*>(&attention16_fwd_kernel<NT, PACKED, ONE>),
                               hipFuncAttributeMaxDynamicSharedMemorySize, (int)a16_lds(NT, false));
     attr = true;
   }
-  hipLaunchKernelGGL((attention16_fwd_kernel<NT, PACKED>), dim3(batch * heads), dim3(64 * NT), a16_lds(NT, false), st, qkv, out,
-                     lse, seq, heads, causal, off);
+  hipLaunchKernelGGL((attention16_fwd_kernel<NT, PACKED, ONE>), dim3(batch * heads), dim3(64 * NT), a16_lds(NT, false), st, qkv,
+                     out, lse, seq, heads, causal, off, rows);
   return launch_status();
 }
 
-template <int NT, bool PACKED = false, bool PIN = false>
+template <int NT, bool PACKED = false, bool PIN = false, bool ONE = false>
 static int a16_bwd(const float* qkv, const float* dout, const float* out, const float* lse, float* dqkv, float* work,
-                   int batch, int seq, int heads, int causal, hipStream_t st, const int32_t* off = nullptr) {
+                   int batch, int seq, int heads, int causal, hipStream_t st, const int32_t* off = nullptr,
+                   const int32_t* rows = nullptr) {
   (void)work;
   static bool attr = false;
   if (!attr && a16_lds(NT, true) > 48 * 1024) {
-    (void)hipFuncSetAttribute(reinterpret_cast<const void*>(&attention16_bwd_kernel<NT, PACKED, PIN>),
+    (void)hipFuncSetAttribute(reinterpret_cast<const void*>(&attention16_bwd_kernel<NT, PACKED, PIN, ONE>),
                               hipFuncAttributeMaxDynamicSharedMemorySize, (int)a16_lds(NT, true));
     attr = true;
   }
-  hipLaunchKernelGGL((attention16_bwd_kernel<NT, PACKED, PIN>), dim3(2 * batch * heads), dim3(64 * NT), a16_lds(NT, true), st,
-                     qkv, dout, out, lse, dqkv, seq, heads, causal, off);
+  hipLaunchKernelGGL((attention16_bwd_kernel<NT, PACKED, PIN, ONE>), dim3(2 * batch * heads), dim3(64 * NT), a16_lds(NT, true),
+                     st, qkv, dout, out, lse, dqkv, seq, heads, causal, off, rows);
   return launch_status();
 }
 
@@ -417,4 +465,38 @@
   }
 }
 
-}
+int attention16_fwd_one(const float* qkv, float* out, float* lse, const int32_t* rows, const int32_t* off, int batch, int seq,
+                        int heads, int causal, hipStream_t st) {
+#define A16_FWD_ONE(nt)                                                                            \
+  return off ? a16_fwd<nt, true, true>(qkv, out, lse, batch, seq, heads, 1, st, off, nullptr)      \
+             : a16_fwd<nt, false, true>(qkv, out, lse, batch, seq, heads, causal, st, nullptr, rows)
+  switch ((seq + 15) / 16) {
+    case 1: A16_FWD_ONE(1);
+    case 2: A16_FWD_ONE(2);
+    case 3: A16_FWD_ONE(3);
+    case 4: A16_FWD_ONE(4);
+    case 5: A16_FWD_ONE(5);
+    default: A16_FWD_ONE(6);
+  }
+#undef A16_FWD_ONE
+}
+
+int attention16_bwd_one(const float* qkv, const float* dout, const float* out, const float* lse, float* dqkv,
+                        const int32_t* rows, const int32_t* off, bool pin, int batch, int seq, int heads, int causal,
+                        hipStream_t st) {
+#define A16_BWD_ONE(nt)                                                                                                    \
+  if (!off) return a16_bwd<nt, false, false, true>(qkv, dout, out, lse, dqkv, nullptr, batch, seq, heads, causal, st, nullptr, rows); \
+  return pin ? a16_bwd<nt, true, true, true>(qkv, dout, out, lse, dqkv, nullptr, batch, seq, heads, 1, st, off, nullptr)   \
+             : a16_bwd<nt, true, false, true>(qkv, dout, out, lse, dqkv, nullptr, batch, seq, heads, 1, st, off, nullptr)
+  switch ((seq + 15) / 16) {
+    case 1: A16_BWD_ONE(1);
+    case 2: A16_BWD_ONE(2);
+    case 3: A16_BWD_ONE(3);
+    case 4: A16_BWD_ONE(4);
+    case 5: A16_BWD_ONE(5);
+    default: A16_BWD_ONE(6);
+  }
+#undef A16_BWD_ONE
+}
+
+}
diff --git a/jittor-clip-fewshot_amd/csrc/elem.hip b/jittor-clip-fewshot_amd/csrc/elem.hip
--- a/jittor-clip-fewshot_amd/csrc/elem.hip
+++ b/jittor-clip-fewshot_amd/csrc/elem.hip
@@ -502,15 +502,70 @@
   v[i] = vi;
 }
 
-__global__ __launch_bounds__(256) void matmul_small_kernel(const float* __restrict__ A, const float* __restrict__ B,
-                                                           float* __restrict__ C, int M, int N, int K, long sam, long sak,
-                                                           long sbk, long sbn, float alpha) {
+__global__ __launch_bounds__(256) void matmul_small_ref_kernel(const float* __restrict__ A, const float* __restrict__ B,
+                                                               float* __restrict__ C, int M, int N, int K, long sam, long sak,
+                                                               long sbk, long sbn, float alpha) {
   const size_t i = (size_t)blockIdx.x * 256 + threadIdx.x;
   if (i >= (size_t)M * N) return;
   const int m = (int)(i / N), n = (int)(i % N);
   float acc = 0.f;
   for (int k = 0; k < K; ++k) acc = fmaf(A[m * sam + k * sak], B[k * sbk + n * sbn], acc);
   C[i] = alpha * acc;
+}
+
+constexpr int MS_TILE = 32;
+__global__ __launch_bounds__(256) void matmul_small_kernel(const float* __restrict__ A, const float* __restrict__ B,
+                                                           float* __restrict__ C, int M, int N, int K, long sam, long sak,
+                                                           long sbk, long sbn, float alpha) {
+  __shared__ float sA[MS_TILE][MS_TILE + 1];
+  __shared__ float sB[MS_TILE][MS_TILE + 1];
+  const int tx = threadIdx.x & 31, ty = threadIdx.x >> 5;
+  const int m0 = blockIdx.y * MS_TILE, n0 = blockIdx.x * MS_TILE;
+  const bool a_kfast = sak <= sam, b_nfast = sbn <= sbk;
+  float ra[4], rb[4];
+  auto fetch = [&](int k0) {
+#pragma unroll
+    for (int j = 0; j < 4; ++j) {
+      const int s = ty + 8 * j;
+      const int am = m0 + (a_kfast ? s : tx), ak = k0 + (a_kfast ? tx : s);
+      const int bn = n0 + (b_nfast ? tx : s), bk = k0 + (b_nfast ? s : tx);
+      ra[j] = (am < M && ak < K) ? A[am * sam + ak * sak] : 0.f;
+      rb[j] = (bn < N && bk < K) ? B[bk * sbk + bn * sbn] : 0.f;
+    }
+  };
+  fetch(0);
+  float acc[4] = {0.f, 0.f, 0.f, 0.f};
+  for (int k0 = 0; k0 < K; k0 += MS_TILE) {
+    __syncthreads();
+#pragma unroll
+    for (int j = 0; j < 4; ++j) {
+      const int s = ty + 8 * j;
+      sA[a_kfast ? tx : s][a_kfast ? s : tx] = ra[j];
+      sB[b_nfast ? s : tx][b_nfast ? tx : s] = rb[j];
+    }
+    __syncthreads();
+    if (k0 + MS_TILE < K) fetch(k0 + MS_TILE);
+    if (k0 + MS_TILE <= K) {
+#pragma unroll
+      for (int k = 0; k < MS_TILE; ++k) {
+        const float bv = sB[k][tx];
+#pragma unroll
+        for (int i = 0; i < 4; ++i) acc[i] = fmaf(sA[k][ty + 8 * i], bv, acc[i]);
+      }
+    } else {
+      for (int k = 0; k < K - k0; ++k) {
+        const float bv = sB[k][tx];
+#pragma unroll
+        for (int i = 0; i < 4; ++i) acc[i] = fmaf(sA[k][ty + 8 * i], bv, acc[i]);
+      }
+    }
+  }
+  const int n = n0 + tx;
+#pragma unroll
+  for (int i = 0; i < 4; ++i) {
+    const int m = m0 + ty + 8 * i;
+    if (m < M && n < N) C[(size_t)m * N + n] = alpha * acc[i];
+  }
 }
 
 static inline unsigned grid_for(size_t total) {
@@ -611,9 +666,19 @@
 extern "C" int clipfs_matmul_small(const float* A, const float* B, float* C, int M, int N, int K, long sam, long sak,
                                    long sbk, long sbn, float alpha, void* stream) {
   CLIPFS_REQUIRE(A && B && C && M > 0 && N > 0 && K > 0, "matmul_small: bad args");
+  const unsigned gx = (unsigned)((N + MS_TILE - 1) / MS_TILE), gy = (unsigned)((M + MS_TILE - 1) / MS_TILE);
+  CLIPFS_REQUIRE(gy <= 65535u, "matmul_small: M %d too large", M);
+  hipLaunchKernelGGL(matmul_small_kernel, dim3(gx, gy), dim3(256), 0, (hipStream_t)stream, A, B, C, M, N, K, sam, sak, sbk,
+                     sbn, alpha);
+  return launch_status();
+}
+
+extern "C" int clipfs_matmul_small_ref(const float* A, const float* B, float* C, int M, int N, int K, long sam, long sak,
+                                       long sbk, long sbn, float alpha, void* stream) {
+  CLIPFS_REQUIRE(A && B && C && M > 0 && N > 0 && K > 0, "matmul_small_ref: bad args");
   const size_t total = (size_t)M * N;
-  hipLaunchKernelGGL(matmul_small_kernel, dim3((unsigned)((total + 255) / 256)), dim3(256), 0, (hipStream_t)stream, A, B, C,
-                     M, N, K, sam, sak, sbk, sbn, alpha);
+  hipLaunchKernelGGL(matmul_small_ref_kernel, dim3((unsigned)((total + 255) / 256)), dim3(256), 0, (hipStream_t)stream, A, B,
+                     C, M, N, K, sam, sak, sbk, sbn, alpha);
   return launch_status();
 }
 
diff --git a/jittor-clip-fewshot_amd/csrc/tower.hip b/jittor-clip-fewshot_amd/csrc/tower.hip
--- a/jittor-clip-fewshot_amd/csrc/tower.hip
+++ b/jittor-clip-fewshot_amd/csrc/tower.hip
@@ -219,6 +219,76 @@
   return clipfs_bias_grad(x, (size_t)cols, rows, cols, segw, o0, o1, o2, work, st);
 }
 
+static int gemm_ld(const TowerCtx& cx, const float* A, int lda, const float* B, int ldb, float* C, int ldc, int M, int N, int K,
+                   const float* bias, const float* res, const float* lt, const float* lb, int r, int nseg, int segw,
+                   float lscale, hipStream_t st) {
+  clipfs_gemm_args a = {};
+  a.struct_size = sizeof(a);
+  a.workspace = cx.ws;
+  a.workspace_floats = cx.ws_floats;
+  a.counters = cx.counters;
+  a.counters_ints = cx.counters_ints;
+  a.A = A; a.B = B; a.C = C; a.M = M; a.N = N; a.K = K;
+  a.lda = lda; a.ldb = ldb; a.ldc = ldc; a.alpha = 1.f;
+  a.bias = bias; a.residual = res; a.ldres = N;
+  a.lora_t = lt; a.lora_b = lb; a.lora_r = r; a.lora_nseg = nseg; a.lora_seg_width = segw; a.lora_scale = lscale;
+  return clipfs_gemm_nt(&a, st);
+}
+
+static TowerCtx unsplit_ctx(const TowerCtx& cx) {
+  TowerCtx c = cx;
+  c.ws = nullptr;
+  c.ws_floats = 0;
+  c.counters = nullptr;
+  c.counters_ints = 0;
+  return c;
+}
+
+struct RowSel {
+  const int32_t* rows;
+  const int32_t* map;
+  int seq;
+};
+static int gather_sel(const RowSel& s, const float* src, size_t ld, float* out, int n, int width, hipStream_t st) {
+  return s.map ? clipfs_gather_rows_map(src, ld, s.map, out, n, width, st)
+               : clipfs_gather_seq_rows(src, ld, s.rows, out, n, s.seq, width, st);
+}
+static int put_sel(const RowSel& s, const float* src, float* dst, size_t ld, int n, int width, hipStream_t st) {
+  return s.map ? clipfs_put_rows_map(src, s.map, dst, ld, n, width, st)
+               : clipfs_put_seq_rows(src, s.rows, dst, ld, n, s.seq, width, st);
+}
+
+static int qkv_fwd_one(const clipfs_tower* t, const clipfs_block& b, const TowerCtx& cx, const RowSel& sel, const float* h1,
+                       const float* t_qkv, float* qkv, int rows_all, int batch, float* tmp, hipStream_t st) {
+  const int d = t->width, r = t->lora_r;
+  const TowerCtx cxu = unsplit_ctx(cx);
+  CLIPFS_CHECK(gemm_ld(cxu, h1, d, b.w_qkv + (size_t)d * d, d, qkv + d, 3 * d, rows_all, 2 * d, d, b.b_qkv ? b.b_qkv + d : nullptr,
+                       nullptr, t_qkv ? t_qkv + r : nullptr, t_qkv ? b.lora_b_qkv + (size_t)d * r : nullptr, r, 3, d,
+                       t->lora_scale, st));
+  float* q_s = tmp;
+  float* h1_s = q_s + al4((size_t)batch * d);
+  float* tq_s = h1_s + al4((size_t)batch * d);
+  CLIPFS_CHECK(gather_sel(sel, h1, (size_t)d, h1_s, batch, d, st));
+  if (t_qkv) CLIPFS_CHECK(gather_sel(sel, t_qkv, (size_t)3 * r, tq_s, batch, 3 * r, st));
+  CLIPFS_CHECK(gemm_ld(cxu, h1_s, d, b.w_qkv, d, q_s, d, batch, d, d, b.b_qkv, nullptr, t_qkv ? tq_s : nullptr,
+                       t_qkv ? b.lora_b_qkv : nullptr, r, 3, d, t->lora_scale, st));
+  return put_sel(sel, q_s, qkv, (size_t)3 * d, batch, d, st);
+}
+
+static int qkv_dgrad_one(const clipfs_tower* t, const clipfs_block& b, const TowerCtx& cx, const RowSel& sel,
+                         const float* dqkv, float* dh, int rows_all, int batch, float* tmp, hipStream_t st) {
+  const int d = t->width;
+  const TowerCtx cxu = unsplit_ctx(cx);
+  CLIPFS_CHECK(gemm_ld(cxu, dqkv + d, 3 * d, b.w_qkv_t + d, 3 * d, dh, d, rows_all, d, 2 * d, nullptr, nullptr, nullptr, nullptr,
+                       0, 0, 0, 0.f, st));
+  float* dqkv_s = tmp;
+  float* dh_s = dqkv_s + al4((size_t)batch * 3 * d);
+  CLIPFS_CHECK(gather_sel(sel, dqkv, (size_t)3 * d, dqkv_s, batch, 3 * d, st));
+  CLIPFS_CHECK(gemm_ld(cxu, dqkv_s, 3 * d, b.w_qkv_t, 3 * d, dh_s, d, batch, d, 3 * d, nullptr, nullptr, nullptr, nullptr, 0, 0, 0,
+                       0.f, st));
+  return put_sel(sel, dh_s, dh, (size_t)d, batch, d, st);
+}
+
 }
 
 using namespace clipfs;
@@ -244,6 +314,14 @@
   const clipfs_block& b = t->blocks[t->layers - 1];
   const bool lora_o = b.lora_a_o && (b.lora_mask & 8u);
   return !(force_dense || lora_o || t->seq < 8);
+}
+
+static bool g_one_query = true;
+static bool one_query_ok(const clipfs_tower* t, int batch) {
+  static const bool env_off = getenv("CLIPFS_ONE_QUERY") && atoi(getenv("CLIPFS_ONE_QUERY")) == 0;
+  if (env_off || !g_one_query || !last_block_rows_ok(t)) return false;
+  if (t->weight_format != 0 || !clipfs_attention_one_ok(t->seq)) return false;
+  return clipfs_gemm_workspace_floats(batch * t->seq, 3 * t->width, t->width) == 0;
 }
 
 static int tower_fwd_impl(const clipfs_tower* t, float* x, const int32_t* rows, int batch, float* saved, float* scratch,
@@ -302,10 +380,17 @@
                                       keep, st));
     }
     const bool q16 = qkv_f16(t);
-    CLIPFS_CHECK(gemm(cx, h1, b.w_qkv, b.w_qkv_p, qkv, M, 3 * d, d, b.b_qkv, nullptr, 0, nullptr, nullptr, qkv_mask ? t_qkv : nullptr,
-                      b.lora_b_qkv, r, 3, d, t->lora_scale, st, CHAIN_NONE, h16, q16 ? (void*)qkv : nullptr));
+    const bool one_q = rows && l == t->layers - 1 && one_query_ok(t, batch);
+    if (one_q) {
+      const RowSel sel = {rows, nullptr, t->seq};
+      CLIPFS_CHECK(qkv_fwd_one(t, b, cx, sel, h1, qkv_mask ? t_qkv : nullptr, qkv, M, batch, scratch + SC.big, st));
+    } else
+      CLIPFS_CHECK(gemm(cx, h1, b.w_qkv, b.w_qkv_p, qkv, M, 3 * d, d, b.b_qkv, nullptr, 0, nullptr, nullptr, qkv_mask ? t_qkv : nullptr,
+                        b.lora_b_qkv, r, 3, d, t->lora_scale, st, CHAIN_NONE, h16, q16 ? (void*)qkv : nullptr));
     const void* att16 = nullptr;
-    if (f16_attention(t)) {
+    if (one_q) {
+      CLIPFS_CHECK(clipfs_attention_fwd_one(qkv, att, lse, rows, nullptr, batch, t->seq, t->heads, t->causal, st));
+    } else if (f16_attention(t)) {
       CLIPFS_CHECK(clipfs_attention_f16_fwd(qkv, q16, att, h16, lse, batch, t->seq, t->heads, t->causal, st));
       att16 = h16;
     } else
@@ -377,6 +462,18 @@
 
 extern "C" int clipfs_tower_rows_mode(const clipfs_tower* t) {
   return (t && t->blocks && t->layers > 0 && last_block_rows_ok(t)) ? 1 : 0;
+}
+
+extern "C" int clipfs_tower_one_query(int enable) {
+  const int was = g_one_query ? 1 : 0;
+  g_one_query = enable != 0;
+  return was;
+}
+
+extern "C" int clipfs_tower_one_query_mode(const clipfs_tower* t, int batch) {
+  if (!t || !t->blocks || t->struct_size != sizeof(clipfs_tower) || t->block_size != sizeof(clipfs_block)) return 0;
+  if (batch <= 0 || t->layers <= 0 || t->seq <= 0) return 0;
+  return one_query_ok(t, batch) ? 1 : 0;
 }
 
 static int lora_bwd_block(const clipfs_tower* t, bool dy16, const float* dy, const void* dy16p, const float* x,
@@ -526,7 +623,7 @@
 
 static int tower_bwd_packed_range(const clipfs_tower* t, float* dx, int batch, const PackPlan& P, const float* saved,
                                   float* scratch, int stop_at_input, hipStream_t st, int l_hi, bool attn_only_top,
-                                  bool saved_packed) {
+                                  bool saved_packed, const float* datt_rows = nullptr) {
   const int M = batch * t->seq, d = t->width, r = t->lora_r, R = P.R;
   const SavedLayout SL = saved_packed ? saved_layout_packed(t, (size_t)R, (size_t)batch) : saved_layout(t, (size_t)M);
   const int srows = saved_packed ? R : M;
@@ -583,7 +680,11 @@
                                     work, st, l));
       }
     }
-    if (saved_packed)
+    const bool one_q = datt_rows && attn_only_top && l == l_hi;
+    if (one_q)
+      CLIPFS_CHECK(clipfs_attention_bwd_one(sv + SL.qkv, datt_rows, sv + SL.att, sv + SL.lse, dqkv_p, nullptr, P.off,
+                                            saved_packed ? 1 : 0, batch, t->seq, t->heads, 1, st));
+    else if (saved_packed)
       CLIPFS_CHECK(clipfs_attention_bwd_packed_io(sv + SL.qkv, datt_p, sv + SL.att, sv + SL.lse, dqkv_p, P.off, batch, t->seq,
                                                   t->heads, st));
     else
@@ -592,7 +693,10 @@
     CLIPFS_CHECK(bias_sum(dqkv_p, R, 3 * d, d, b.g_b_q, b.g_b_k, b.g_b_v, bwork, st));
     const bool need_dx = !(l == lo && stop_at_input) || b.g_prompt;
     const bool need_dh = need_dx || b.g_ln1_b;
-    if (need_dh)
+    if (need_dh && one_q) {
+      const RowSel sel = {nullptr, P.eotp, t->seq};
+      CLIPFS_CHECK(qkv_dgrad_one(t, b, cx, sel, dqkv_p, dh_p, R, batch, scratch + SC.big, st));
+    } else if (need_dh)
       CLIPFS_CHECK(gemm(cx, dqkv_p, b.w_qkv_t, b.w_qkv_t_p, dh_p, R, d, 3 * d, nullptr, nullptr, 0, nullptr, nullptr, nullptr, nullptr,
                         0, 0, 0, 0.f, st));
     if (qkv_mask && (b.g_lora_a_qkv || need_dh)) {
@@ -650,7 +754,9 @@
   float* datt_s = dxm_s + (size_t)Ms * d;
   float* mean_s = datt_s + (size_t)Ms * d;
   float* rstd_s = mean_s + al4((size_t)Ms);
+  float* tmp_s = rstd_s + al4((size_t)Ms);
   float* bwork = scratch + SC.bwork;
+  const bool one_q = one_query_ok(t, batch);
   CLIPFS_CHECK(bias_sum(dxs, Ms, d, d, b.g_b_pr, nullptr, nullptr, bwork, st));
   const bool f16m = t->weight_format == 2;
   if (saved_packed) {
@@ -680,23 +786,32 @@
   if (P) {
     float* datt_p = scratch + SC.b1;
     const size_t Rd = (size_t)P->R * d;
-    hipError_t e = hipMemsetAsync(datt_p, 0, (al4(Rd) + Rd) * sizeof(float), st);
-    CLIPFS_REQUIRE(e == hipSuccess, "tower_bwd_packed: memset failed: %s", hipGetErrorString(e));
-    CLIPFS_CHECK(clipfs_put_rows_map(datt_s, P->eotp, datt_p, (size_t)d, Ms, d, st));
+    if (one_q) {
+      hipError_t e = hipMemsetAsync(datt_p + al4(Rd), 0, Rd * sizeof(float), st);
+      CLIPFS_REQUIRE(e == hipSuccess, "tower_bwd_packed: memset failed: %s", hipGetErrorString(e));
+    } else {
+      hipError_t e = hipMemsetAsync(datt_p, 0, (al4(Rd) + Rd) * sizeof(float), st);
+      CLIPFS_REQUIRE(e == hipSuccess, "tower_bwd_packed: memset failed: %s", hipGetErrorString(e));
+      CLIPFS_CHECK(clipfs_put_rows_map(datt_s, P->eotp, datt_p, (size_t)d, Ms, d, st));
+    }
     CLIPFS_CHECK(clipfs_put_rows_map(dxm_s, P->eotp, datt_p + al4(Rd), (size_t)d, Ms, d, st));
-    return tower_bwd_packed_range(t, dx, batch, *P, saved, scratch, stop_at_input, st, l, true, saved_packed);
+    return tower_bwd_packed_range(t, dx, batch, *P, saved, scratch, stop_at_input, st, l, true, saved_packed,
+                                  one_q ? datt_s : nullptr);
   }
   float* dh = scratch + SC.h;
   float* datt = scratch + SC.b1;
   float* dqkv = scratch + SC.b3;
   float* dt = scratch + SC.dt;
   float* work = scratch + SC.work;
-  CLIPFS_CHECK(clipfs_scatter_rows(datt_s, rows, datt, batch, seq, d, st));
+  if (!one_q) CLIPFS_CHECK(clipfs_scatter_rows(datt_s, rows, datt, batch, seq, d, st));
   const unsigned qkv_mask = b.lora_a_qkv ? (b.lora_mask & 7u) : 0u;
   const void* dqkv16_ready = nullptr;
   void* dqkv16 = (f16_attention(t) && cx.a16) ? (void*)((char*)cx.a16 + (size_t)M * d * 2) : nullptr;
   const bool dy16 = dqkv16 && (!qkv_mask || clipfs_lora_bwd_f16dy_ok(d, d, r, 3));
-  if (f16_attention(t)) {
+  if (one_q) {
+    CLIPFS_CHECK(clipfs_attention_bwd_one(sv + SL.qkv, datt_s, sv + SL.att, sv + SL.lse, dqkv, rows, nullptr, 0, batch, seq,
+                                          t->heads, t->causal, st));
+  } else if (f16_attention(t)) {
     CLIPFS_CHECK(clipfs_attention_f16_bwd(sv + SL.qkv, qkv_f16(t), datt, 0, sv + SL.att, sv + SL.lse, dy16 ? nullptr : dqkv, dqkv16,
                                           dh, batch, seq, t->heads, t->causal, st));
     dqkv16_ready = dqkv16;
@@ -706,7 +821,10 @@
   const uint32_t ds = t->dropout_stream0 + 4u * (uint32_t)l;
   const bool need_dx = !(l == t->grad_lo && stop_at_input) || b.g_prompt;
   const bool need_dh = need_dx || b.g_ln1_b;
-  if (need_dh)
+  if (need_dh && one_q) {
+    const RowSel sel = {rows, nullptr, seq};
+    CLIPFS_CHECK(qkv_dgrad_one(t, b, cx, sel, dqkv, dh, M, batch, tmp_s, st));
+  } else if (need_dh)
     CLIPFS_CHECK(gemm(cx, dqkv, b.w_qkv_t, b.w_qkv_t_p, dh, M, d, 3 * d, nullptr, nullptr, 0, nullptr, nullptr, nullptr, nullptr, 0, 0,
                       0, 0.f, st, CHAIN_NONE, dqkv16_ready));
   if (qkv_mask)
@@ -822,9 +940,16 @@
         CLIPFS_CHECK(clipfs_lora_down(h1, b.lora_a_qkv, t_qkv, R, d, r, 3, qkv_mask, t->lora_dropout, seed, ds, t->dropout_row0,
                                       keep, st));
     }
-    CLIPFS_CHECK(gemm(cxp, h1, b.w_qkv, b.w_qkv_p, qkv, R, 3 * d, d, b.b_qkv, nullptr, 0, nullptr, nullptr,
-                      qkv_mask ? t_qkv : nullptr, b.lora_b_qkv, r, 3, d, t->lora_scale, st));
-    CLIPFS_CHECK(clipfs_attention_fwd_packed(qkv, att, lse, P.off, batch, seq, t->heads, st));
+    const bool one_q = l == t->layers - 1 && one_query_ok(t, batch);
+    if (one_q) {
+      const RowSel sel = {nullptr, P.eotp, seq};
+      CLIPFS_CHECK(qkv_fwd_one(t, b, cxp, sel, h1, qkv_mask ? t_qkv : nullptr, qkv, R, batch, scratch + SC.big, st));
+      CLIPFS_CHECK(clipfs_attention_fwd_one(qkv, att, lse, nullptr, P.off, batch, seq, t->heads, 1, st));
+    } else {
+      CLIPFS_CHECK(gemm(cxp, h1, b.w_qkv, b.w_qkv_p, qkv, R, 3 * d, d, b.b_qkv, nullptr, 0, nullptr, nullptr,
+                        qkv_mask ? t_qkv : nullptr, b.lora_b_qkv, r, 3, d, t->lora_scale, st));
+      CLIPFS_CHECK(clipfs_attention_fwd_packed(qkv, att, lse, P.off, batch, seq, t->heads, st));
+    }
     if (l == t->layers - 1) {
       const int Ms = batch;
       float* att_s = scratch + SC.big;
```

Result: no change. 4902 images/s, median of 6 (+0.7%).
